# leejaeyong7/nerfacc

Measured on AMD Instinct MI355X. Metric: rays/sec (fwd+bwd) through 128^3 occ-grid, 1M-ray batch, higher is better.
Workload: dtype f32; 1 GPU; cfg2: 1048576 image rays/GPU, 128^3 shell10 occ grid (G=1), step 2*sqrt(3)/1024, sampling+rendering fwd+bwd; rays_per_gpu=1048576, resolution=128, grid=shell10, samples_after_compaction=32244949, parallelism=ray-sharded x1, field=synthetic analytic field, native callbacks (see bench.py NativeField/TorchField)

## Files before the change

### include/nerfacc_hip.h

```cpp
#ifndef NERFACC_HIP_H
#define NERFACC_HIP_H

#include <stdint.h>

#ifdef __cplusplus
extern "C" {
#endif

#define NFA_OK 0
#define NFA_EINVAL (-1)
#define NFA_EHIP (-2)

#define NFA_MAX_GRID_LEVELS 8

typedef void *nfa_stream_t;

const char *nfa_last_error(void);
#define NFA_VERSION 403
int nfa_version(void);
int nfa_set_tuning(const char *name, const char *value);
int nfa_device_arch(char *buf, int buflen);


int64_t nfa_cumsum_scratch_bytes(int64_t n);
// ... 78 lines not shown
                       uint8_t *mask, int32_t *alive, int64_t *count, int32_t count_samples, nfa_stream_t stream);
int nfa_bin_rays_levels(const float *rays_o, const float *rays_d, int64_t n_rays, const float *aabbs, int32_t n_grids,
                        const int32_t *res, float near_plane, int32_t *order, void *scratch,
                        uint64_t *coherence , nfa_stream_t stream);
int nfa_expand_runs(int64_t n_rays, float step_size, const int32_t *run_cnts, const uint64_t *runs,
                    int32_t max_runs, const int64_t *packed_info , float *t_starts,
                    float *t_ends, float *t_mids, int64_t *ray_indices, int64_t capacity, nfa_stream_t stream);
int nfa_fill_ray_indices(int64_t n_rays, const int64_t *packed_info , int64_t *ray_indices,
                         nfa_stream_t stream);
int nfa_traverse_cone_runs(const nfa_traverse_args *args, int32_t *run_cnts, uint64_t *runs, int32_t max_runs,
                           int32_t *overflow_count, const int32_t *ray_order ,
                           int64_t n_order, nfa_stream_t stream);
int nfa_traverse_cone_walk(const nfa_traverse_args *args, const uint32_t *bits, int32_t *run_cnts, uint64_t *runs,
                           int32_t max_runs, int32_t *overflow_count, uint32_t *arena, int32_t arena_capacity,
                           const int32_t *ray_order, int64_t n_order, nfa_stream_t stream);
int nfa_expand_cone_arena(const uint32_t *arena, int32_t n_entries, float step_size, float cone_angle,
                          const int64_t *packed_info , float *t_starts, float *t_ends, int64_t *ray_indices,
                          nfa_stream_t stream);
int nfa_expand_cone_runs(int64_t n_rays, float step_size, float cone_angle, const int32_t *run_cnts,
                         const uint64_t *runs, int32_t max_runs, const int64_t *packed_info, float *t_starts,
                         float *t_ends, int64_t *ray_indices, nfa_stream_t stream);
int nfa_expand_intervals(int64_t n_rays, float step_size, const int32_t *run_cnts, const uint64_t *runs,
                         int32_t max_runs, const int64_t *iv_packed_info , float *vals,
                         int64_t *ray_indices, uint8_t *is_left, uint8_t *is_right, nfa_stream_t stream);


int nfa_grid_cell_points(const int64_t *indices, const float *jitter , int64_t n, const int32_t *res,
                         const float *aabb , float *x , nfa_stream_t stream);
int nfa_grid_ema_update(float *occs, int64_t cell_base, const int64_t *indices, int64_t n, const float *occ,
                        float ema_decay, float *scratch , nfa_stream_t stream);
int64_t nfa_grid_rebinarize_scratch_bytes(void);
int nfa_grid_rebinarize(const float *occs, int32_t n_grids, const int32_t *res, float occ_thre, uint8_t *binaries,
                        uint32_t *walk_bits, void *scratch, nfa_stream_t stream);


void nfa_seg_plan(int64_t n_elems, int64_t n_rays, int64_t *tile_elems, int64_t *n_tiles);
int64_t nfa_seg_table_rows(int64_t n_tiles);
int nfa_seg_build_tiles(const int64_t *packed_info , int64_t n_rays, int64_t n_elems,
                        int64_t tile_elems, int64_t n_tiles, int64_t *tiles ,
                        int32_t *flags, nfa_stream_t stream);

int nfa_packed_scan(int kind, int reverse, const int64_t *packed_info, const int64_t *tiles, int64_t n_tiles,
                    int64_t n_rays, int64_t n_elems, const float *inputs, float *outputs,
                    nfa_stream_t stream);
int nfa_packed_scan_generic(int kind, int reverse, int normalize, const int64_t *packed_info,
                            int64_t n_rays, int64_t n_elems, const float *inputs, float *outputs,
                            nfa_stream_t stream);
int nfa_packed_prod_backward(int kind, const int64_t *packed_info, const int64_t *tiles, int64_t n_tiles,
                             int64_t n_rays, int64_t n_elems, const float *inputs,
                             const float *outputs, const float *grad_outputs, float *grad_inputs,
                             nfa_stream_t stream);

int nfa_render_from_density_fwd(const float *t_starts, const float *t_ends, const float *sigmas,
                                const float *prefix_trans , const int64_t *packed_info,
                                const int64_t *tiles, int64_t n_tiles, int64_t n_rays, int64_t n_elems,
                                float *weights, float *trans, float *alphas, nfa_stream_t stream);
int nfa_render_from_alpha_fwd(const float *alphas, const float *prefix_trans, const int64_t *packed_info,
                              const int64_t *tiles, int64_t n_tiles, int64_t n_rays, int64_t n_elems,
                              float *weights, float *trans, nfa_stream_t stream);
int nfa_render_from_density_bwd(const float *t_starts, const float *t_ends, const float *trans,
                                const float *alphas, const float *g_weights, const float *g_trans,
                                const float *g_alphas, const int64_t *packed_info, const int64_t *tiles, int64_t n_tiles,
                                int64_t n_rays, int64_t n_elems, float *grad_sigmas, float *grad_x,
                                nfa_stream_t stream);
int nfa_density_cdf_rows_fwd(const float *t_starts, const float *t_ends, const float *sigmas, const int64_t *packed_info,
                             const int64_t *tiles, int64_t n_tiles, int64_t n_rays, int64_t n_elems, int32_t row_len,
                             float *trans, float *alphas, float *cdfs , nfa_stream_t stream);
int nfa_density_cdf_rows_bwd(const float *t_starts, const float *t_ends, const float *trans, const float *alphas,
                             const float *g_cdfs , const int64_t *packed_info, const int64_t *tiles,
                             int64_t n_tiles, int64_t n_rays, int64_t n_elems, int32_t row_len, float *grad_sigmas,
                             nfa_stream_t stream);
int nfa_render_from_alpha_bwd(const float *alphas, const float *trans, const float *g_weights,
                              const float *g_trans, const int64_t *packed_info, const int64_t *tiles, int64_t n_tiles,
                              int64_t n_rays, int64_t n_elems, float *grad_alphas, nfa_stream_t stream);

int nfa_render_visibility(const float *t_starts, const float *t_ends, const float *sigmas_or_alphas,
                          const float *prefix_trans, float early_stop_eps, float alpha_thre,
                          const int64_t *packed_info, const int64_t *tiles, int64_t n_tiles, int64_t n_rays,
                          int64_t n_elems, uint8_t *vis, int64_t *vis_cnts, nfa_stream_t stream);
int nfa_compact_samples(const uint8_t *vis, const float *t_starts, const float *t_ends,
                        const int64_t *packed_info, const int64_t *tiles, int64_t n_tiles, const int64_t *out_starts,
                        int64_t n_rays, int64_t n_elems, int64_t *out_ray_indices,
                        float *out_t_starts, float *out_t_ends, int64_t capacity, nfa_stream_t stream);

int nfa_accumulate_along_rays(const float *weights, const float *values, int32_t D,
                              const int64_t *packed_info, const int64_t *tiles, int64_t n_tiles, int64_t n_rays,
                              int64_t n_elems, int accumulate, float *out, nfa_stream_t stream);
int nfa_accumulate_along_rays_atomic(const float *weights, const float *values, int32_t D,
                                     const int64_t *ray_indices, int64_t n_rays, int64_t n_elems,
                                     float *out, nfa_stream_t stream);
int nfa_accumulate_along_rays_bwd(const float *weights, const float *values, int32_t D,
                                  const float *g_out, const int64_t *packed_info, const int64_t *tiles, int64_t n_tiles,
                                  int64_t n_rays, int64_t n_elems, float *g_weights, float *g_values,
                                  nfa_stream_t stream);
int nfa_render_accumulate_fwd(const float *weights, const float *rgbs, const float *t_starts,
                              const float *t_ends, const int64_t *packed_info, const int64_t *tiles, int64_t n_tiles,
                              int64_t n_rays, int64_t n_elems, float *colors, float *opacities,
                              float *depths, nfa_stream_t stream);
int nfa_render_accumulate_bwd(const float *weights, const float *rgbs, const float *t_starts,
                              const float *t_ends, const float *g_colors, const float *g_opacities,
                              const float *g_depths, const int64_t *packed_info, const int64_t *tiles, int64_t n_tiles,
                              int64_t n_rays, int64_t n_elems, float *g_weights, float *g_rgbs,
                              nfa_stream_t stream);

int nfa_render_fused_fwd(const float *t_starts, const float *t_ends, const float *sigmas, const float *rgbs,
                         const int64_t *packed_info, const int64_t *tiles, int64_t n_tiles, int64_t n_rays,
                         int64_t n_elems, float *weights, float *trans, float *alphas, float *colors,
                         float *opacities, float *depths, nfa_stream_t stream);
int nfa_render_fused_bwd(const float *t_starts, const float *t_ends, const float *rgbs, const float *trans,
                         const float *alphas, const float *g_colors, const float *g_opacities,
                         const float *g_depths, const float *g_weights, const float *g_trans,
                         const float *g_alphas, const int64_t *packed_info, const int64_t *tiles, int64_t n_tiles,
                         int64_t n_rays, int64_t n_elems, float *grad_sigmas, float *grad_rgbs,
                         nfa_stream_t stream);

int nfa_distortion_fwd(const float *weights, const float *t_starts, const float *t_ends, const int64_t *packed_info,
                       const int64_t *tiles, int64_t n_tiles, int64_t n_rays, int64_t n_elems, float *loss, float *w_tot,
                       float *s_tot, nfa_stream_t stream);
int nfa_distortion_bwd(const float *weights, const float *t_starts, const float *t_ends, const float *w_tot,
                       const float *s_tot, const float *g_loss, const int64_t *packed_info, const int64_t *tiles,
                       int64_t n_tiles, int64_t n_rays, int64_t n_elems, float *grad_weights, float *grad_t_starts,
                       float *grad_t_ends, nfa_stream_t stream);

#define NFA_VISIBLE_SLOTS 1024
int nfa_render_step_accumulate(const float *t_starts, const float *t_ends, const float *sigmas, const float *rgbs,
                               const int64_t *packed_info, const int64_t *tiles, int64_t n_tiles, int64_t n_rays,
                               int64_t n_elems, float alpha_thre, float *colors, float *opacities, float *depths,
                               int64_t *n_visible, nfa_stream_t stream);


int nfa_importance_sampling(const float *in_vals, const float *cdfs, const int64_t *in_packed_info,
                            int64_t n_rays, int64_t n_edges_per_ray, int64_t n_samples,
                            int stratified, uint64_t seed, uint64_t offset,
                            float *out_intervals , float *out_samples ,
                            nfa_stream_t stream);
int nfa_importance_sampling_t(const float *in_vals, const float *cdfs, const int64_t *in_packed_info, int64_t n_rays,
                              int64_t n_edges_per_ray, int64_t n_samples, int stratified, uint64_t seed,
                              uint64_t offset, float *out_intervals, float *out_samples, int transform, float t_a,
                              float t_b, float *out_t_starts, float *out_t_ends, nfa_stream_t stream);
int nfa_importance_sampling_packed(const float *in_vals, const float *cdfs, const int64_t *in_packed_info, int64_t n_rays,
                                   int64_t n_edges_per_ray, const int64_t *sm_packed_info, const int64_t *iv_packed_info,
                                   int stratified, uint64_t seed, uint64_t offset, float *sm_vals, int64_t *sm_ray_indices,
                                   float *iv_vals, int64_t *iv_ray_indices, uint8_t *iv_is_left, uint8_t *iv_is_right,
                                   nfa_stream_t stream);
int nfa_searchsorted(const float *q_vals, const int64_t *q_packed_info, const int64_t *q_ray_indices,
                     int64_t q_n_rays, int64_t q_per_ray, int64_t q_total,
                     const float *k_vals, const int64_t *k_packed_info, int64_t k_per_ray,
                     int64_t *ids_left, int64_t *ids_right, nfa_stream_t stream);

int nfa_pdf_loss_fwd(const float *q_vals, const float *q_cdfs, const float *k_vals, const float *k_cdfs,
                     int64_t n_rays, int32_t n_query_edges, int32_t n_key_edges, float eps, float *loss,
                     uint32_t *key_ids, nfa_stream_t stream);
int nfa_pdf_loss_bwd(const float *q_cdfs, const float *k_cdfs, const uint32_t *key_ids, int64_t n_rays,
                     int32_t n_query_edges, int32_t n_key_edges, float eps, const float *g_loss, float *g_k_cdfs,
                     float *g_q_cdfs, nfa_stream_t stream);
int64_t nfa_pdf_loss_partials(int64_t n_rays, int32_t n_query_edges, int32_t n_key_edges);
int nfa_pdf_loss_sum_fwd(const float *q_vals, const float *q_cdfs, const float *k_vals, const float *k_cdfs,
                         int64_t n_rays, int32_t n_query_edges, int32_t n_key_edges, float eps, float *partials,
                         uint32_t *key_ids, nfa_stream_t stream);
int nfa_pdf_loss_mean_bwd(const float *q_cdfs, const float *k_cdfs, const uint32_t *key_ids, int64_t n_rays,
                          int32_t n_query_edges, int32_t n_key_edges, float eps, const float *g_mean, float *g_k_cdfs,
                          float *g_q_cdfs, nfa_stream_t stream);


int nfa_opencv_lens_undistortion(const float *uv, const float *params, int64_t n_points, int32_t n_params,
                                 int64_t param_stride, float eps, int32_t iters, float *uv_out, nfa_stream_t stream);
int nfa_opencv_lens_undistortion_fisheye(const float *uv, const float *params, int64_t n_points, int32_t n_params,
                                         int64_t param_stride, float eps, int32_t iters, float *uv_out,
                                         nfa_stream_t stream);


int nfa_hashgrid_fwd(const float *x, const float *params, int64_t n_points, int32_t n_levels, int32_t n_features,
                     int32_t log2_hashmap_size, const float *scales_host, const int32_t *resolutions_host,
                     const int32_t *sizes_host, int64_t n_params, float *y, nfa_stream_t stream);
int nfa_hashgrid_bwd(const float *x, const float *params, const float *grad_y, int64_t n_points, int32_t n_levels,
                     int32_t n_features, int32_t log2_hashmap_size, const float *scales_host,
                     const int32_t *resolutions_host, const int32_t *sizes_host, int64_t n_params, float *grad_params,
                     float *grad_x, nfa_stream_t stream);
int nfa_sh_fwd(const float *dirs, int64_t n_points, int32_t degree, float *out, nfa_stream_t stream);
int nfa_sh_bwd(const float *dirs, const float *grad_out, int64_t n_points, int32_t degree, float *grad_dirs,
               nfa_stream_t stream);


int nfa_sample_positions_fwd(const float *rays_o, const float *rays_d, const float *t_starts, const float *t_ends,
                             const int64_t *ray_indices, int64_t n_rays, int64_t n_elems, int64_t samples_per_ray,
                             const float *aabb_host, const float *aabb, int32_t contraction, int32_t dirs_mode,
                             float *positions, float *dirs, uint8_t *selector, nfa_stream_t stream);
int nfa_sample_positions_bwd(const float *rays_o, const float *rays_d, const float *t_starts, const float *t_ends,
                             const int64_t *ray_indices, const float *g_positions, const float *g_dirs,
                             const int64_t *packed_info, const int64_t *tiles, int64_t n_tiles, int64_t n_rays,
                             int64_t n_elems, int64_t samples_per_ray, const float *aabb_host, const float *aabb,
                             int32_t contraction, int32_t dirs_mode, float *grad_rays_o, float *grad_rays_d,
                             float *grad_t_starts, float *grad_t_ends, float *grad_p, nfa_stream_t stream);

#ifdef __cplusplus
}
#endif
// ... 2 lines not shown
```

### nerfacc_amd/_backend.py

```python
from __future__ import annotations

import ctypes as C
import os
import threading
from typing import Optional

import torch

from . import _build

_lock = threading.Lock()
_lib: Optional[C.CDLL] = None

_vp, _i64, _i32, _f32, _u64, _int = C.c_void_p, C.c_int64, C.c_int32, C.c_float, C.c_uint64, C.c_int


class TraverseArgs(C.Structure):
    _fields_ = [
        ("n_rays", _i64), ("rays_o", _vp), ("rays_d", _vp), ("rays_mask", _vp),
        ("n_grids", _i32), ("res", _i32 * 3), ("binaries", _vp), ("aabbs", _vp),
        ("hits", _vp), ("t_sorted", _vp), ("t_indices", _vp),
        ("near_planes", _vp), ("far_planes", _vp),
        ("step_size", _f32), ("cone_angle", _f32), ("traverse_steps_limit", _i32), ("mode", _i32),
        ("iv_vals", _vp), ("iv_ray_indices", _vp), ("iv_is_left", _vp), ("iv_is_right", _vp),
        ("iv_starts", _vp), ("iv_cnts", _vp),
        ("sm_vals", _vp), ("sm_ray_indices", _vp), ("sm_is_valid", _vp),
        ("sm_t_starts", _vp), ("sm_t_ends", _vp), ("sm_starts", _vp), ("sm_cnts", _vp),
        ("terminate_planes", _vp),
        ("ray_filter", _vp), ("ray_filter_min", _i32),
        ("bricks", _vp), ("coarse", _vp),
        ("steps_limit_dev", _vp), ("n_listed_dev", _vp), ("run_if_nonzero", _vp),
    ]


_SIGS = {
    "nfa_exclusive_cumsum_i64": [_vp, _i64, _vp, _vp, _vp, _vp],
    "nfa_exclusive_cumsum_pairs_i64": [_vp, _i64, _vp, _vp, _vp, _vp],
    "nfa_exclusive_cumsum_pairs_stats_i64": [_vp, _i64, _vp, _vp, _vp, _vp],
    "nfa_pack_info": [_vp, _i64, _i64, _vp, _vp, _vp, _vp],
    "nfa_pdf_loss_fwd": [_vp, _vp, _vp, _vp, _i64, _i32, _i32, _f32, _vp, _vp, _vp],
    "nfa_pdf_loss_bwd": [_vp, _vp, _vp, _i64, _i32, _i32, _f32, _vp, _vp, _vp, _vp],
    "nfa_pdf_loss_partials": [_i64, _i32, _i32],
    "nfa_pdf_loss_sum_fwd": [_vp, _vp, _vp, _vp, _i64, _i32, _i32, _f32, _vp, _vp, _vp],
    "nfa_pdf_loss_mean_bwd": [_vp, _vp, _vp, _i64, _i32, _i32, _f32, _vp, _vp, _vp, _vp],
    "nfa_pack_bits": [_vp, _i64, _vp, _vp],
    "nfa_unpack_rows": [_vp, _vp, _vp, _i64, _i64, _i64, _i64, _vp, _i32, _vp, _vp],
    "nfa_pack_rows": [_vp, _vp, _vp, _i64, _i64, _i64, _i64, _vp, _vp],
    "nfa_mask_row_counts": [_vp, _i64, _i64, _vp, _vp],
    "nfa_ray_aabb_intersect": [_vp, _vp, _i64, _vp, _i32, _f32, _f32, _f32, _vp, _vp, _vp, _vp],
    "nfa_ray_events": [_vp, _vp, _i64, _vp, _i32, _vp, _vp, _vp, _vp],
    "nfa_traverse_grids": [C.POINTER(TraverseArgs), _vp],
    "nfa_bricks_words": [_i32, C.POINTER(_i32)],
    "nfa_pack_bricks": [_vp, _i32, C.POINTER(_i32), _vp, _vp, _vp],
    "nfa_walk_bits_words": [_i32, C.POINTER(_i32)],
    "nfa_pack_walk_bits": [_vp, _i32, C.POINTER(_i32), _vp, _vp],
    "nfa_traverse_runs": [C.POINTER(TraverseArgs), _vp, _vp, _vp, _i32, _vp, _f32, _vp, _i64, _vp],
    "nfa_bin_rays": [_vp, _vp, _i64, _vp, _vp, _vp, _vp],
    "nfa_grid_cell_points": [_vp, _vp, _i64, C.POINTER(_i32), _vp, _vp, _vp],
    "nfa_grid_ema_update": [_vp, _i64, _vp, _i64, _vp, _f32, _vp, _vp],
    "nfa_grid_rebinarize_scratch_bytes": [],
    "nfa_grid_rebinarize": [_vp, _i32, C.POINTER(_i32), _f32, _vp, _vp, _vp, _vp],
    "nfa_expand_runs": [_i64, _f32, _vp, _vp, _i32, _vp, _vp, _vp, _vp, _vp, _i64, _vp],
    "nfa_fill_ray_indices": [_i64, _vp, _vp, _vp],
    "nfa_traverse_cone_runs": [C.POINTER(TraverseArgs), _vp, _vp, _i32, _vp, _vp, _i64, _vp],
    "nfa_alive_rays": [_vp, _vp, _i64, _f32, _i64, _vp, _vp, _vp, _vp],
    "nfa_testmode_begin": [_vp, _vp, _i64, _i32, _i32, _vp, _vp, _vp, _i32, _vp],
    "nfa_testmode_alive": [_vp, _vp, _vp, _f32, _i64, _vp, _vp, _vp, _i32, _vp],
    "nfa_traverse_cone_walk": [C.POINTER(TraverseArgs), _vp, _vp, _vp, _i32, _vp, _vp, _i32, _vp, _i64, _vp],
    "nfa_expand_cone_arena": [_vp, _i32, _f32, _f32, _vp, _vp, _vp, _vp, _vp],
    "nfa_bin_rays_levels": [_vp, _vp, _i64, _vp, _i32, C.POINTER(_i32), _f32, _vp, _vp, _vp, _vp],
    "nfa_expand_cone_runs": [_i64, _f32, _f32, _vp, _vp, _i32, _vp, _vp, _vp, _vp, _vp],
    "nfa_expand_intervals": [_i64, _f32, _vp, _vp, _i32, _vp, _vp, _vp, _vp, _vp, _vp],
    "nfa_seg_plan": [_i64, _i64, C.POINTER(_i64), C.POINTER(_i64)],
    "nfa_seg_table_rows": [_i64],
    "nfa_seg_build_tiles": [_vp, _i64, _i64, _i64, _i64, _vp, _vp, _vp],
    "nfa_packed_scan": [_int, _int, _vp, _vp, _i64, _i64, _i64, _vp, _vp, _vp],
    "nfa_packed_scan_generic": [_int, _int, _int, _vp, _i64, _i64, _vp, _vp, _vp],
    "nfa_packed_prod_backward": [_int, _vp, _vp, _i64, _i64, _i64, _vp, _vp, _vp, _vp, _vp],
    "nfa_render_from_density_fwd": [_vp, _vp, _vp, _vp, _vp, _vp, _i64, _i64, _i64, _vp, _vp, _vp, _vp],
    "nfa_render_from_alpha_fwd": [_vp, _vp, _vp, _vp, _i64, _i64, _i64, _vp, _vp, _vp],
    "nfa_render_from_density_bwd": [_vp, _vp, _vp, _vp, _vp, _vp, _vp, _vp, _vp, _i64, _i64, _i64, _vp, _vp, _vp],
    "nfa_density_cdf_rows_fwd": [_vp, _vp, _vp, _vp, _vp, _i64, _i64, _i64, _i32, _vp, _vp, _vp, _vp],
    "nfa_density_cdf_rows_bwd": [_vp, _vp, _vp, _vp, _vp, _vp, _vp, _i64, _i64, _i64, _i32, _vp, _vp],
    "nfa_render_from_alpha_bwd": [_vp, _vp, _vp, _vp, _vp, _vp, _i64, _i64, _i64, _vp, _vp],
    "nfa_render_visibility": [_vp, _vp, _vp, _vp, _f32, _f32, _vp, _vp, _i64, _i64, _i64, _vp, _vp, _vp],
    "nfa_compact_samples": [_vp, _vp, _vp, _vp, _vp, _i64, _vp, _i64, _i64, _vp, _vp, _vp, _i64, _vp],
    "nfa_accumulate_along_rays": [_vp, _vp, _i32, _vp, _vp, _i64, _i64, _i64, _int, _vp, _vp],
    "nfa_accumulate_along_rays_atomic": [_vp, _vp, _i32, _vp, _i64, _i64, _vp, _vp],
    "nfa_accumulate_along_rays_bwd": [_vp, _vp, _i32, _vp, _vp, _vp, _i64, _i64, _i64, _vp, _vp, _vp],
    "nfa_render_accumulate_fwd": [_vp, _vp, _vp, _vp, _vp, _vp, _i64, _i64, _i64, _vp, _vp, _vp, _vp],
    "nfa_render_accumulate_bwd": [_vp, _vp, _vp, _vp, _vp, _vp, _vp, _vp, _vp, _i64, _i64, _i64, _vp, _vp, _vp],
    "nfa_render_fused_fwd": [_vp, _vp, _vp, _vp, _vp, _vp, _i64, _i64, _i64, _vp, _vp, _vp, _vp, _vp, _vp, _vp],
    "nfa_render_fused_bwd": [_vp] * 13 + [_i64, _i64, _i64, _vp, _vp, _vp],
    "nfa_render_step_accumulate": [_vp, _vp, _vp, _vp, _vp, _vp, _i64, _i64, _i64, _f32, _vp, _vp, _vp, _vp, _vp],
    "nfa_distortion_fwd": [_vp, _vp, _vp, _vp, _vp, _i64, _i64, _i64, _vp, _vp, _vp, _vp],
    "nfa_distortion_bwd": [_vp] * 8 + [_i64, _i64, _i64, _vp, _vp, _vp, _vp],
    "nfa_importance_sampling": [_vp, _vp, _vp, _i64, _i64, _i64, _int, _u64, _u64, _vp, _vp, _vp],
    "nfa_importance_sampling_t": [_vp, _vp, _vp, _i64, _i64, _i64, _int, _u64, _u64, _vp, _vp, _int, _f32, _f32, _vp, _vp, _vp],
    "nfa_importance_sampling_packed": [_vp, _vp, _vp, _i64, _i64, _vp, _vp, _int, _u64, _u64, _vp, _vp, _vp, _vp, _vp, _vp, _vp],
    "nfa_searchsorted": [_vp, _vp, _vp, _i64, _i64, _i64, _vp, _vp, _i64, _vp, _vp, _vp],
    "nfa_opencv_lens_undistortion": [_vp, _vp, _i64, _i32, _i64, _f32, _i32, _vp, _vp],
    "nfa_opencv_lens_undistortion_fisheye": [_vp, _vp, _i64, _i32, _i64, _f32, _i32, _vp, _vp],
    "nfa_hashgrid_fwd": [_vp, _vp, _i64, _i32, _i32, _i32, _vp, _vp, _vp, _i64, _vp, _vp],
    "nfa_hashgrid_bwd": [_vp, _vp, _vp, _i64, _i32, _i32, _i32, _vp, _vp, _vp, _i64, _vp, _vp, _vp],
    "nfa_sh_fwd": [_vp, _i64, _i32, _vp, _vp],
    "nfa_sh_bwd": [_vp, _vp, _i64, _i32, _vp, _vp],
    "nfa_sample_positions_fwd": [_vp, _vp, _vp, _vp, _vp, _i64, _i64, _i64, _vp, _vp, _i32, _i32, _vp, _vp, _vp, _vp],
    "nfa_sample_positions_bwd": [_vp] * 9 + [_i64, _i64, _i64, _i64, _vp, _vp, _i32, _i32, _vp, _vp, _vp, _vp, _vp, _vp],
    "nfa_cumsum_scratch_bytes": [_i64],
    "nfa_last_error": [],
    "nfa_version": [],
    "nfa_set_tuning": [C.c_char_p, C.c_char_p],
    "nfa_device_arch": [C.c_char_p, _int],
}
_RESTYPES = {"nfa_grid_rebinarize_scratch_bytes": _i64, "nfa_bricks_words": _i64, "nfa_walk_bits_words": _i64, "nfa_pdf_loss_partials": _i64, "nfa_cumsum_scratch_bytes": _i64, "nfa_seg_table_rows": _i64, "nfa_seg_plan": None, "nfa_last_error": C.c_char_p}

EXPORTED_SYMBOLS = tuple(_SIGS)


def library_path() -> str:
    return _build.LIB_PATH


def load() -> C.CDLL:
    global _lib
    if _lib is not None:
        return _lib
    with _lock:
        if _lib is not None:
            return _lib
        path = _build.LIB_PATH
        if _build.is_stale() and _build.hipcc() is not None:
            path = _build.build()
        if not os.path.exists(path):
            raise RuntimeError(
                "nerfacc_amd: libnerfacc_hip.so is missing and hipcc is not available to build it. "
                "There is no CPU fallback for the native ops.")
        lib = C.CDLL(path)
        for name, argtypes in _SIGS.items():
            fn = getattr(lib, name)
            fn.argtypes = argtypes
            fn.restype = _RESTYPES[name] if name in _RESTYPES else _int
        if lib.nfa_version() != ABI_VERSION:
            raise RuntimeError(f"nerfacc_amd: {path} was built from include/nerfacc_hip.h version {lib.nfa_version()}, these "
                               f"bindings are written for {ABI_VERSION}: rebuild the library (nerfacc_amd._build.build(force=True))")
        _lib = lib
    return _lib


ABI_VERSION = 403


def set_tuning(name: str, value: Optional[str]) -> None:
    call("nfa_set_tuning", name.encode(), None if value is None else str(value).encode())


class NativeError(RuntimeError):
    """Counterpart of the RuntimeError TORCH_CHECK raises in the reference."""


def call(name: str, *args) -> None:
    lib = load()
    rc = getattr(lib, name)(*args)
    if rc != 0:
        msg = lib.nfa_last_error()
        raise NativeError(f"{name}: {msg.decode() if msg else rc}")


def call_group(name: str, fn) -> None:
    fn()


def ptr(t: Optional[torch.Tensor]):
    return None if t is None else t.data_ptr()


_RAW_STREAM = getattr(torch._C, "_cuda_getCurrentRawStream", None)
_CUR_DEVICE = getattr(torch._C, "_cuda_getDevice", None)


def stream() -> int:
    if _RAW_STREAM is not None and _CUR_DEVICE is not None:
        return _RAW_STREAM(_CUR_DEVICE())
    return torch.cuda.current_stream().cuda_stream


def require_device(*tensors: Optional[torch.Tensor]) -> torch.device:
    dev = None
    for t in tensors:
        if t is None:
            continue
        if not t.is_cuda:
            raise NotImplementedError(
                "nerfacc_amd: this op runs only on a ROCm device (the reference has no CPU "
                "implementation of its native ops either); got a tensor on " + str(t.device))
        if dev is None:
            dev = t.device
        elif t.device != dev:
            raise RuntimeError(f"nerfacc_amd: tensors on different devices ({dev} vs {t.device})")
    if dev is None:
        raise RuntimeError("nerfacc_amd: no tensor argument")
    return dev


def seg_plan(n_elems: int, n_rays: int = 0):
    t, n = _i64(0), _i64(0)
    load().nfa_seg_plan(n_elems, n_rays, C.byref(t), C.byref(n))
    return int(t.value), int(n.value)


def cumsum_scratch(n: int, device) -> torch.Tensor:
    nbytes = ((max(n, 1) + 2047) // 2048 + 1) * 8
    return torch.empty(nbytes // 8, dtype=torch.int64, device=device)
```

### nerfacc_amd/_segments.py

```python
from __future__ import annotations

from dataclasses import dataclass
from typing import Optional

import torch
from torch import Tensor

from . import _backend as B


@dataclass
class SegInfo:
    packed_info: Tensor
    n_rays: int
    n_elems: int
    tiles: Optional[Tensor]
    contiguous: bool
    sorted_indices: bool = True
    n_tiles: int = 0
    trusted: bool = False


_ATTR = "_nfa_seg"
_ATTR_RI = "_nfa_seg_from_ray_indices"


def _build_tiles(packed_info: Tensor, n_elems: int, trusted: bool) -> SegInfo:
    dev = B.require_device(packed_info)
    n_rays = packed_info.shape[0]
    with torch.cuda.device(dev):
        tile_elems, n_tiles = B.seg_plan(n_elems, n_rays)
        tiles = torch.empty((int(B.load().nfa_seg_table_rows(n_tiles)), 2), dtype=torch.int64, device=dev)
        flag = None if trusted else torch.empty(1, dtype=torch.int32, device=dev)
        B.call("nfa_seg_build_tiles", B.ptr(packed_info), n_rays, n_elems, tile_elems, n_tiles, B.ptr(tiles), B.ptr(flag),
               B.stream())
        ok = True if trusted else (int(flag.item()) == 0)
    return SegInfo(packed_info, n_rays, n_elems, tiles if ok else None, ok, n_tiles=n_tiles, trusted=trusted)


def seginfo_from_packed(packed_info: Tensor, n_elems: int, trusted: bool = False) -> SegInfo:
    assert packed_info.dim() == 2 and packed_info.shape[-1] == 2, "packed_info must be 2-D with shape (B, 2)."
    cached = getattr(packed_info, _ATTR, None)
    if cached is not None and cached[0] == packed_info._version and cached[1] == n_elems:
        return cached[2]
    pi = packed_info
    if pi.dtype != torch.int64 or not pi.is_contiguous():
        pi = pi.to(torch.int64).contiguous()
    info = _build_tiles(pi, n_elems, trusted)
    try:
        setattr(packed_info, _ATTR, (packed_info._version, n_elems, info))
    except Exception:
        pass
    return info


def tag_trusted(packed_info: Tensor, n_elems: int) -> SegInfo:
    return seginfo_from_packed(packed_info, n_elems, trusted=True)


def pack_info_native(ray_indices: Tensor, n_rays: int):
    dev = B.require_device(ray_indices)
    ri = ray_indices if (ray_indices.dtype == torch.int64 and ray_indices.is_contiguous()) else \
        ray_indices.to(torch.int64).contiguous()
    with torch.cuda.device(dev):
        packed = torch.empty((n_rays, 2), dtype=torch.int64, device=dev)
        flag = torch.empty(1, dtype=torch.int32, device=dev)
        scratch = B.cumsum_scratch(n_rays, dev)
        B.call("nfa_pack_info", B.ptr(ri), ri.numel(), n_rays, B.ptr(packed), B.ptr(flag), B.ptr(scratch), B.stream())
    return packed, flag


def seginfo_from_ray_indices(ray_indices: Tensor, n_rays: int) -> SegInfo:
    assert ray_indices.dim() == 1, "ray_indices must be a 1D tensor with shape (n_samples)."
    assert n_rays is not None, "n_rays must be provided"
    cached = getattr(ray_indices, _ATTR_RI, None)
    if cached is not None and cached[0] == ray_indices._version and cached[1] == n_rays:
        return cached[2]
    packed, flag = pack_info_native(ray_indices, n_rays)
    info = _build_tiles(packed, ray_indices.numel(), trusted=True)
    info.sorted_indices = int(flag.item()) == 0
    try:
        setattr(ray_indices, _ATTR_RI, (ray_indices._version, n_rays, info))
    except Exception:
        pass
    return info


def tag_ray_indices(ray_indices: Tensor, n_rays: int, info: SegInfo) -> None:
    setattr(ray_indices, _ATTR_RI, (ray_indices._version, n_rays, info))


def resolve(n_elems: int, packed_info: Optional[Tensor], ray_indices: Optional[Tensor],
            n_rays: Optional[int]) -> Optional[SegInfo]:
    if packed_info is not None:
        return seginfo_from_packed(packed_info, n_elems)
    if ray_indices is not None:
        if n_rays is None:
            n_rays = int(ray_indices.max().item()) + 1 if ray_indices.numel() else 0
        return seginfo_from_ray_indices(ray_indices, n_rays)
    return None


_UNIFORM: "dict[tuple, SegInfo]" = {}


def uniform_seginfo(n_rows: int, row_len: int, device: torch.device) -> SegInfo:
    key = (int(n_rows), int(row_len), device.type, device.index)
    info = _UNIFORM.get(key)
    if info is None:
        starts = torch.arange(n_rows, dtype=torch.int64, device=device) * row_len
        packed = torch.stack([starts, torch.full_like(starts, row_len)], dim=-1)
        info = _build_tiles(packed, n_rows * row_len, trusted=True)
        setattr(packed, _ATTR, (packed._version, n_rows * row_len, info))
        if len(_UNIFORM) >= 6:
            _UNIFORM.pop(next(iter(_UNIFORM)))
        _UNIFORM[key] = info
    return info


def batched_native(*tensors: Optional[Tensor]) -> Optional[SegInfo]:
    ref = None
    for t in tensors:
        if t is None:
            continue
        if not t.is_cuda or t.dtype != torch.float32 or t.dim() < 1:
            return None
        if ref is None:
            ref = t
        elif t.shape != ref.shape:
            return None
    if ref is None or ref.numel() == 0:
        return None
    return uniform_seginfo(ref.numel() // ref.shape[-1], ref.shape[-1], ref.device)
```

### nerfacc_amd/csrc/segscan.hip

```cpp
#include <stdlib.h>

#include "common.hip.h"
#include "samples.h"

namespace nfa {

constexpr int SE = 4;
constexpr int SQ = SE / 4;
constexpr int SEG_CHUNK = 64 * SE;
#ifndef NFA_SEG_TILE_ROWS
#define NFA_SEG_TILE_ROWS 256
#endif
constexpr int64_t SEG_TILE_ROWS = NFA_SEG_TILE_ROWS;
#ifndef NFA_VIS_EXP_FREE
#define NFA_VIS_EXP_FREE 1
#endif
#ifndef NFA_SEG_WAVES_PER_BLOCK
#define NFA_SEG_WAVES_PER_BLOCK 4
#endif
constexpr int SEG_WAVES_PER_BLOCK = NFA_SEG_WAVES_PER_BLOCK;

__global__ __launch_bounds__(256) void seg_build_tiles_kernel(const int64_t *__restrict__ packed_info, int64_t n_rays,
                                                              int64_t n_elems, int64_t tile_elems, int64_t n_tiles,
                                                              longlong2 *__restrict__ tiles, int32_t *__restrict__ flags)
{
    for (int64_t r = (int64_t)blockIdx.x * blockDim.x + threadIdx.x; r <= n_rays;
         r += (int64_t)blockDim.x * gridDim.x) {
        int64_t b_lo, b_hi, e_first;
        bool bad = false;
        if (r < n_rays) {
            const int64_t s = packed_info[2 * r], n = packed_info[2 * r + 1];
            int64_t s_prev = -1;
            if (r > 0) {
                const int64_t ps = packed_info[2 * r - 2], pn = packed_info[2 * r - 1];
                s_prev = ps;
                bad |= (ps + pn != s);
            }
            bad |= (n < 0) || (s < 0) || (s + n > n_elems);
            if (bad) { if (flags) atomicOr(flags, 1); continue; }
            b_lo = (s_prev < 0) ? 0 : s_prev / tile_elems + (r - 1) / SEG_TILE_ROWS + 1;
            b_hi = s / tile_elems + r / SEG_TILE_ROWS;
            e_first = s;
        } else {
            const int64_t s_prev = n_rays > 0 ? packed_info[2 * n_rays - 2] : -1;
            const int64_t n_prev = n_rays > 0 ? packed_info[2 * n_rays - 1] : 0;
            b_lo = (s_prev < 0) ? 0 : s_prev / tile_elems + (n_rays - 1) / SEG_TILE_ROWS + 1;
            b_hi = n_tiles;
            e_first = (s_prev < 0) ? 0 : s_prev + n_prev;
            if (s_prev > n_elems) { if (flags) atomicOr(flags, 1); continue; }
        }
        for (int64_t b = b_lo; b <= b_hi && b <= n_tiles; ++b) tiles[b] = make_longlong2(r, e_first);
    }
}

__host__ __device__ inline int64_t seg_table_rows(int64_t n_tiles) { return n_tiles + 1; }

struct F4 { float v[SE]; };

struct Pos {
    int64_t c;
    int32_t off;
    int32_t safe;
    bool valid[SE];
    bool any, all;
    int32_t d_lo, d_hi;
    bool qany[SQ], qall[SQ];
    __device__ __forceinline__ int64_t p0() const { return c + off; }
};

template <bool VEC>
__device__ __forceinline__ void ld4(const float *__restrict__ p, const Pos &q, F4 &out)
{
    const float *b = p + q.c;
    if (VEC) {
#pragma unroll
        for (int h = 0; h < SQ; ++h) {
            const nfa_v4f v = *reinterpret_cast<const nfa_v4f *>(b + (q.qany[h] ? q.off + 4 * h : q.safe));
            out.v[4 * h] = v.x; out.v[4 * h + 1] = v.y; out.v[4 * h + 2] = v.z; out.v[4 * h + 3] = v.w;
        }
    } else {
#pragma unroll
        for (int j = 0; j < SE; ++j) out.v[j] = b[q.valid[j] ? q.off + j : q.safe];
    }
}
__device__ __forceinline__ float sel(const F4 &r, int j, const bool valid[SE], float fill) { return valid[j] ? r.v[j] : fill; }

#define NFA_ELEMENTWISE_PATH() asm volatile("; element-wise path" ::: "memory")
template <bool VEC>
__device__ __forceinline__ void store4(float *__restrict__ p, const Pos &q, const float v[SE])
{
    float *b = p + q.c;
#pragma unroll
    for (int h = 0; h < SQ; ++h) {
        if (VEC && q.qall[h]) {
            store_f4(b + q.off + 4 * h, v[4 * h], v[4 * h + 1], v[4 * h + 2], v[4 * h + 3]);
        } else {
            NFA_ELEMENTWISE_PATH();
#pragma unroll
            for (int j = 4 * h; j < 4 * h + 4; ++j)
                if (q.valid[j]) b[q.off + j] = v[j];
        }
    }
}

struct StepHeads {
    int32_t lh[SE];
    uint32_t acc;
    bool open_prefix;
    bool carry_on_lane_end;
    int32_t carry_lane;
    int32_t ph;
    int32_t rid[SE], prev_rid[SE];
    bool is_head[SE];
};

template <int S>
__device__ __forceinline__ void heads_step(int32_t &ah, uint32_t &acc)
{
    const int32_t uh = dpp_step<S>(-1, ah);
    if (ah < 0) { acc |= 1u << S; ah = uh; }
}

template <int DIR>
__device__ __forceinline__ void resolve_heads(const int32_t hj[SE], const bool valid[SE], int32_t carry_rid, StepHeads &hd)
{
#pragma unroll
    for (int k = 0; k < SE; ++k) {
        const int j = DIR > 0 ? k : SE - 1 - k;
        const int32_t h = valid[j] ? hj[j] : -1;
        hd.is_head[k] = h >= 0;
        hd.lh[k] = (k == 0 || h >= 0) ? h : hd.lh[k - 1 < 0 ? 0 : k - 1];
    }
    int32_t ah = hd.lh[SE - 1];
    uint32_t acc = 0;
    heads_step<0>(ah, acc); heads_step<1>(ah, acc); heads_step<2>(ah, acc);
    heads_step<3>(ah, acc); heads_step<4>(ah, acc); heads_step<5>(ah, acc);
    const int lane = lane_id(), r = lane & 15;
    const uint32_t has_src = (r >= 1 ? 1u : 0u) | (r >= 2 ? 2u : 0u) | (r >= 4 ? 4u : 0u) | (r >= 8 ? 8u : 0u) |
                             ((lane & 16) ? 16u : 0u) | (lane >= 32 ? 32u : 0u);
    hd.acc = acc & has_src;
    int32_t ph = dpp_prev_lane(-1, ah);
    hd.open_prefix = ph < 0;
    if (ph < 0) ph = carry_rid;
    hd.ph = ph;
    int32_t pr = ph;
#pragma unroll
    for (int k = 0; k < SE; ++k) {
        hd.prev_rid[k] = pr;
        hd.rid[k] = hd.lh[k] >= 0 ? hd.lh[k] : ph;
        pr = hd.rid[k];
    }
}

template <int S, int N, class FI, class FC>
__device__ __forceinline__ void values_step(const StepHeads &hd, float av[N], FI identity, FC comb)
{
    const bool take = (hd.acc >> S) & 1u;
#pragma unroll
    for (int ch = 0; ch < N; ++ch) {
        const float uv = dpp_step<S>(identity(ch), av[ch]);
        if (take) av[ch] = comb(ch, uv, av[ch]);
    }
}

template <int N, class FI, class FC>
__device__ __forceinline__ void scan_values(const StepHeads &hd, const float x[SE][N], float carry[N], float incl[SE][N],
                                            float prev[SE][N], FI identity, FC comb)
{
    float li[SE][N];
#pragma unroll
    for (int k = 0; k < SE; ++k)
#pragma unroll
        for (int ch = 0; ch < N; ++ch)
            li[k][ch] = (k == 0 || hd.is_head[k]) ? x[k][ch] : comb(ch, li[k - 1 < 0 ? 0 : k - 1][ch], x[k][ch]);
    float av[N];
#pragma unroll
    for (int ch = 0; ch < N; ++ch) av[ch] = li[SE - 1][ch];
    values_step<0, N>(hd, av, identity, comb); values_step<1, N>(hd, av, identity, comb);
    values_step<2, N>(hd, av, identity, comb); values_step<3, N>(hd, av, identity, comb);
    values_step<4, N>(hd, av, identity, comb); values_step<5, N>(hd, av, identity, comb);
    float pv[N];
#pragma unroll
    for (int ch = 0; ch < N; ++ch) {
        pv[ch] = dpp_prev_lane(identity(ch), av[ch]);
        if (hd.open_prefix) pv[ch] = comb(ch, carry[ch], pv[ch]);
    }
#pragma unroll
// ... 462 lines not shown
#pragma unroll
                for (int j = 0; j < 4; ++j)
                    if (pq.valid[4 * h + j]) g4[j] = b[pq.off + 4 * h + j + crid[4 * h + j]];
            }
#pragma unroll
            for (int j = 0; j < 4; ++j) {
                const float GT = -g4[j];
                q[4 * h + j] = GW[4 * h + j] * (T[4 * h + j] * A[4 * h + j]) + GT * T[4 * h + j];
            }
        }
    }
    __device__ __forceinline__ void fetch(const Pos &q, Raw &r) const
    {
        ld4<VEC>(ts, q, r.a);
        ld4<VEC>(te, q, r.b);
        ld4<VEC>(tr, q, r.T);
        if (!CDF) ld4<VEC>(al, q, r.A);
        if (gw) ld4<VEC>(gw, q, r.gw);
        if (gt) ld4<VEC>(gt, q, r.gt);
        if (ga) ld4<VEC>(ga, q, r.ga);
    }
    __device__ __forceinline__ void load(const Raw &r, const Pos &pos)
    {
        const bool *valid = pos.valid;
#pragma unroll
        for (int j = 0; j < SE; ++j) {
            T[j] = sel(r.T, j, valid, 0.0f); A[j] = CDF ? 0.0f : sel(r.A, j, valid, 0.0f);
            GW[j] = (gw && valid[j]) ? r.gw.v[j] : 0.0f;
            const float GT = (gt && valid[j]) ? r.gt.v[j] : 0.0f;
            GA[j] = (ga && valid[j]) ? r.ga.v[j] : 0.0f;
            dlt[j] = r.b.v[j] - r.a.v[j];
            q[j] = GW[j] * (T[j] * A[j]) + GT * T[j];
        }
    }
    __device__ __forceinline__ float x(int j, int) const { return q[j]; }
    __device__ __forceinline__ void emit(int j, int64_t, bool, bool is_head, int, int, const float *, const float prev[1])
    {
        const float E = is_head ? 0.0f : prev[0];
        const float om = 1.0f - A[j];
        const float B = GW[j] * T[j] * om + GA[j] * om - E;
        rx[j] = B; rs[j] = dlt[j] * B;
    }
    __device__ __forceinline__ void store(const Pos &q)
    {
        (void)q.p0();
        if (gsig) store4<VEC>(gsig, q, rs);
        if (gx) store4<VEC>(gx, q, rx);
    }
};

template <bool VEC>
struct AlphaBwdOp : OpBase {
    struct Raw { F4 T, A, gw, gt; };
    const float *al, *tr, *gw, *gt;
    float *galpha;
    float T[SE], A[SE], GW[SE], q[SE], res[SE];
    __device__ __forceinline__ void fetch(const Pos &q, Raw &r) const
    {
        ld4<VEC>(tr, q, r.T);
        ld4<VEC>(al, q, r.A);
        if (gw) ld4<VEC>(gw, q, r.gw);
        if (gt) ld4<VEC>(gt, q, r.gt);
    }
    __device__ __forceinline__ void load(const Raw &r, const Pos &pos)
    {
        const bool *valid = pos.valid;
#pragma unroll
        for (int j = 0; j < SE; ++j) {
            T[j] = sel(r.T, j, valid, 0.0f); A[j] = sel(r.A, j, valid, 0.0f);
            GW[j] = (gw && valid[j]) ? r.gw.v[j] : 0.0f;
            const float GT = (gt && valid[j]) ? r.gt.v[j] : 0.0f;
            q[j] = (GW[j] * A[j] + GT) * T[j];
        }
    }
    __device__ __forceinline__ float x(int j, int) const { return q[j]; }
    __device__ __forceinline__ void emit(int j, int64_t, bool, bool is_head, int, int, const float *, const float prev[1])
    {
        const float E = is_head ? 0.0f : prev[0];
        res[j] = GW[j] * T[j] - E / fmaxf(1.0f - A[j], 1e-10f);
    }
    __device__ __forceinline__ void store(const Pos &q) { store4<VEC>(galpha, q, res); }
};

template <bool DENSITY, bool VEC, bool COUNT>
struct VisibilityOp : OpBase {
    static constexpr int NCHB = COUNT ? 1 : 0;
    struct Raw { F4 s, pf, a, b; };
    const float *ts, *te, *val, *prefix;
    float eps, thre;
    float s_lo, s_hi;
    uint8_t *vis;
    int64_t *cnts;
    float x0[SE], a4[SE], pf[SE];
    uint8_t m[SE];
    __device__ __forceinline__ float identity(int) const { return DENSITY ? 0.0f : 1.0f; }
    __device__ __forceinline__ float comb(int, float a, float b) const { return DENSITY ? a + b : a * b; }
    __device__ __forceinline__ void fetch(const Pos &q, Raw &r) const
    {
        ld4<VEC>(val, q, r.s);
        if (prefix) ld4<VEC>(prefix, q, r.pf);
        if (DENSITY) {
            ld4<VEC>(ts, q, r.a);
            ld4<VEC>(te, q, r.b);
        }
    }
    __device__ __forceinline__ void load(const Raw &r, const Pos &pos)
    {
        const bool *valid = pos.valid;
#pragma unroll
        for (int j = 0; j < SE; ++j) {
            pf[j] = prefix ? r.pf.v[j] : 1.0f;
            const float sv = sel(r.s, j, valid, 0.0f);
            if (DENSITY) { x0[j] = valid[j] ? sv * (r.b.v[j] - r.a.v[j]) : 0.0f; a4[j] = (thre > 0.0f) ? 1.0f - expf(-x0[j]) : 1.0f; }
            else { a4[j] = sv; x0[j] = 1.0f - sv; }
        }
    }
    __device__ __forceinline__ float x(int j, int) const { return x0[j]; }
    __device__ __forceinline__ void emit(int j, int64_t, bool valid, bool is_head, int, int, const float *, const float prev[1])
    {
        bool v;
        if (DENSITY && NFA_VIS_EXP_FREE && !prefix) {
            const float S = is_head ? 0.0f : prev[0];
            v = S <= s_lo;
            const bool band = S > s_lo && S < s_hi;
            if (__ballot(band) != 0ull) {
                asm volatile("; transmittance near the threshold" ::: "memory");
                if (band) v = expf(-S) >= eps;
            }
        } else {
            float T = DENSITY ? expf(-(is_head ? 0.0f : prev[0])) : (is_head ? 1.0f : prev[0]);
            if (prefix) T *= pf[j];
            v = T >= eps;
        }
        if (thre > 0.0f) v = v && (a4[j] >= thre);
        m[j] = (valid && v) ? 1 : 0;
    }
    __device__ __forceinline__ float xb(int j, int) const { return (float)m[j]; }
    __device__ __forceinline__ void ray_done_b(int rid, int, float tot) const { cnts[rid] = (int64_t)tot; }
    __device__ __forceinline__ void store(const Pos &q)
    {
        uint8_t *b = vis + q.c;
#pragma unroll
        for (int h = 0; h < SQ; ++h) {
            if (VEC && q.qall[h]) {
                *reinterpret_cast<uchar4 *>(b + q.off + 4 * h) = make_uchar4(m[4 * h], m[4 * h + 1], m[4 * h + 2], m[4 * h + 3]);
            } else {
                NFA_ELEMENTWISE_PATH();
#pragma unroll
                for (int j = 4 * h; j < 4 * h + 4; ++j)
                    if (q.valid[j]) b[q.off + j] = m[j];
            }
        }
    }
    __device__ __forceinline__ void empty_ray(int rid) const
    {
        if (COUNT) cnts[rid] = 0;
    }
};

struct U4 { uint32_t w[SQ]; };
__device__ __forceinline__ void load_mask4(const uint8_t *vis, bool vec, const Pos &q, U4 &m)
{
    const uint8_t *b = vis + q.c;
#pragma unroll
    for (int h = 0; h < SQ; ++h) {
        if (vec) {
            const int32_t o = q.safe + (q.qany[h] ? 1 : 0) * (q.off + 4 * h - q.safe);
            m.w[h] = *reinterpret_cast<const uint32_t *>(b + o);
        } else {
            uint32_t w = 0;
#pragma unroll
            for (int j = 0; j < 4; ++j) w |= (uint32_t)b[q.valid[4 * h + j] ? q.off + 4 * h + j : q.safe] << (8 * j);
            m.w[h] = w;
        }
    }
}
__device__ __forceinline__ float mask_sel(const U4 &m, int j, const bool valid[SE])
{
    return (valid[j] && ((m.w[j / 4] >> (8 * (j % 4))) & 0xFFu)) ? 1.0f : 0.0f;
}

template <bool VEC>
struct CompactOp : OpBase {
    static constexpr int RAY_CAP = 192;
    static constexpr int RAY_LDS_FLOATS = 3 * SEG_CHUNK + 2 * RAY_CAP;
    struct Raw { U4 m; F4 a, b; };
    const uint8_t *vis;
    int vis_vec;
    const float *ts, *te;
    const int64_t *out_starts;
    int64_t *o_ri;
    float *o_ts, *o_te;
    int64_t cap = (int64_t)1 << 62;
    float *stage = nullptr;
    const int64_t *s_start = nullptr;
    int32_t g_lo = 0, g_n = 0;
    float m[SE], a[SE], b[SE];
    int64_t dst[SE];
    int32_t er[SE];
    float rank[SE];
    __device__ __forceinline__ void tile_begin(int32_t r_lo, int32_t r_hi, float *lds)
    {
        stage = lds;
        int64_t *st = reinterpret_cast<int64_t *>(lds + 3 * SEG_CHUNK);
        s_start = st; g_lo = r_lo; g_n = min(r_hi - r_lo, RAY_CAP);
        __builtin_amdgcn_wave_barrier();
        for (int32_t i = lane_id(); i < g_n; i += 64) st[i] = out_starts[(int64_t)r_lo + i];
        __builtin_amdgcn_wave_barrier();
    }
    __device__ __forceinline__ void fetch(const Pos &q, Raw &r) const
    {
        load_mask4(vis, vis_vec != 0, q, r.m);
        ld4<VEC>(ts, q, r.a);
        ld4<VEC>(te, q, r.b);
    }
    __device__ __forceinline__ void load(const Raw &r, const Pos &pos)
    {
        const bool *valid = pos.valid;
#pragma unroll
        for (int j = 0; j < SE; ++j) { m[j] = mask_sel(r.m, j, valid); a[j] = r.a.v[j]; b[j] = r.b.v[j]; }
    }
    __device__ __forceinline__ float x(int j, int) const { return m[j]; }
    __device__ __forceinline__ void emit(int j, int64_t, bool, bool is_head, int rid, int, const float *, const float prev[1])
    {
        er[j] = rid;
        rank[j] = is_head ? 0.0f : prev[0];
    }
    __device__ __forceinline__ void store(const Pos &)
    {
        struct __attribute__((packed, aligned(4))) Q4 { float x, y, z, w; };
        struct __attribute__((packed, aligned(8))) L2 { int64_t x, y; };
        bool keep[SE];
        bool any = false;
        int n_mine = 0;
#pragma unroll
        for (int j = 0; j < SE; ++j) { keep[j] = m[j] != 0.0f; any = any || keep[j]; n_mine += keep[j] ? 1 : 0; }
        const unsigned long long lanes = __ballot(any);
        if (lanes == 0ull) return;
        bool far = false;
#pragma unroll
        for (int j = 0; j < SE; ++j) {
            const uint32_t slot = (uint32_t)(er[j] - g_lo);
            const bool staged = slot < (uint32_t)g_n;
            dst[j] = s_start[staged ? slot : 0u];
            far = far || (keep[j] && !staged);
        }
        if (__ballot(far) != 0ull) {
            asm volatile("; output offsets beyond the staged rays" ::: "memory");
#pragma unroll
            for (int j = 0; j < SE; ++j)
                if (keep[j] && (uint32_t)(er[j] - g_lo) >= (uint32_t)g_n) dst[j] = out_starts[er[j]];
        }
#pragma unroll
        for (int j = 0; j < SE; ++j) dst[j] = keep[j] ? dst[j] + (int64_t)rank[j] : 0;
        const int lane = lane_id();
        const int first = __builtin_ctzll(lanes), last = 63 - __builtin_clzll(lanes);
        int64_t my_first = dst[SE - 1], my_last = dst[0];
#pragma unroll
        for (int j = SE - 2; j >= 0; --j) if (keep[j]) my_first = dst[j];
#pragma unroll
        for (int j = 1; j < SE; ++j) if (keep[j]) my_last = dst[j];
        const int64_t base = uniform64(__shfl(my_first, first, 64));
        const int64_t span = uniform64(__shfl(my_last, last, 64)) - base + 1;
        int cnt = n_mine;
#pragma unroll
        for (int off = 32; off >= 1; off >>= 1) cnt += __shfl_xor(cnt, off, 64);
        if (span == (int64_t)cnt && span <= SEG_CHUNK) {
            float *s_ts = stage, *s_te = stage + SEG_CHUNK;
            int32_t *s_ri = reinterpret_cast<int32_t *>(stage + 2 * SEG_CHUNK);
            __builtin_amdgcn_wave_barrier();
#pragma unroll
            for (int j = 0; j < SE; ++j)
                if (keep[j]) {
                    const uint32_t o = (uint32_t)(dst[j] - base);
                    if (o < (uint32_t)SEG_CHUNK) { s_ts[o] = a[j]; s_te[o] = b[j]; s_ri[o] = er[j]; }
                }
            __builtin_amdgcn_wave_barrier();
            const int n = (int)max((int64_t)0, min(span, cap - base));
            float *g_ts = o_ts + base, *g_te = o_te + base;
            int64_t *g_ri = o_ri + base;
            for (int o = 4 * lane; o < n; o += 256) {
                if (o + 3 < n) {
                    const Q4 vt = {s_ts[o], s_ts[o + 1], s_ts[o + 2], s_ts[o + 3]};
                    const Q4 ve = {s_te[o], s_te[o + 1], s_te[o + 2], s_te[o + 3]};
                    *reinterpret_cast<Q4 *>(g_ts + o) = vt;
                    *reinterpret_cast<Q4 *>(g_te + o) = ve;
                    const L2 r0 = {(int64_t)s_ri[o], (int64_t)s_ri[o + 1]}, r1 = {(int64_t)s_ri[o + 2], (int64_t)s_ri[o + 3]};
                    *reinterpret_cast<L2 *>(g_ri + o) = r0;
                    *reinterpret_cast<L2 *>(g_ri + o + 2) = r1;
                } else {
                    for (int i = o; i < n; ++i) { g_ts[i] = s_ts[i]; g_te[i] = s_te[i]; g_ri[i] = (int64_t)s_ri[i]; }
                }
            }
            __builtin_amdgcn_wave_barrier();
        } else {
#pragma unroll
            for (int j = 0; j < SE; ++j)
                if (keep[j] && dst[j] < cap) { o_ri[dst[j]] = er[j]; o_ts[dst[j]] = a[j]; o_te[dst[j]] = b[j]; }
        }
    }
};

template <int C, bool VEC>
// ... 161 lines not shown
    const float *w, *rgb, *ts, *te;
    float *colors, *opac, *depth;
    float xv[SE][5];
    __device__ __forceinline__ void fetch(const Pos &q, Raw &r) const
    {
        ld4<VEC>(w, q, r.w);
        ld4<VEC>(ts, q, r.a);
        ld4<VEC>(te, q, r.b);
        load_rgb12(rgb, VEC, q, r.c);
    }
    __device__ __forceinline__ void load(const Raw &r, const Pos &pos)
    {
        const bool *valid = pos.valid;
        float c[3 * SE];
        fix_rgb12(rgb, VEC, pos, r.c, c);
#pragma unroll
        for (int j = 0; j < SE; ++j) {
            const float ww = sel(r.w, j, valid, 0.0f);
            xv[j][0] = ww * c[3 * j]; xv[j][1] = ww * c[3 * j + 1]; xv[j][2] = ww * c[3 * j + 2];
            xv[j][3] = ww;
            xv[j][4] = ww * ((r.a.v[j] + r.b.v[j]) / 2.0f);
        }
    }
    __device__ __forceinline__ float x(int j, int ch) const { return xv[j][ch]; }
    __device__ __forceinline__ void put(int rid, const float *t) const
    {
        colors[3 * (int64_t)rid] = t[0]; colors[3 * (int64_t)rid + 1] = t[1]; colors[3 * (int64_t)rid + 2] = t[2];
        opac[rid] = t[3]; depth[rid] = t[4];
    }
    __device__ __forceinline__ void emit(int, int64_t, bool, bool, int, int, const float *, const float *) const {}
    __device__ __forceinline__ void store(const Pos &) const {}
    __device__ __forceinline__ void ray_done(int rid, const float t[5]) const { put(rid, t); }
    __device__ __forceinline__ void empty_ray(int rid) const
    {
        const float z[5] = {0, 0, 0, 0, 0};
        put(rid, z);
    }
};

template <bool VEC>
struct RenderAccumBwdOp : OpBase {
    struct Raw { F4 w, a, b; float c[3 * SE]; };
    const float *w, *rgb, *ts, *te, *gc, *go, *gd;
    float *gw, *grgb;
    float ww[SE], mid[SE], res[SE], c[3 * SE], gr[3 * SE];
    __device__ __forceinline__ void fetch(const Pos &q, Raw &r) const
    {
        ld4<VEC>(w, q, r.w);
        ld4<VEC>(ts, q, r.a);
        ld4<VEC>(te, q, r.b);
        load_rgb12(rgb, VEC, q, r.c);
    }
    __device__ __forceinline__ void load(const Raw &r, const Pos &pos)
    {
        const bool *valid = pos.valid;
        (void)valid;
#pragma unroll
        for (int j = 0; j < SE; ++j) { ww[j] = r.w.v[j]; mid[j] = (r.a.v[j] + r.b.v[j]) / 2.0f; }
        fix_rgb12(rgb, VEC, pos, r.c, c);
    }
    __device__ __forceinline__ float x(int, int) const { return 0.0f; }
    __device__ __forceinline__ void emit(int j, int64_t, bool valid, bool, int rid, int, const float *, const float *)
    {
        float g = 0.0f;
        gr[3 * j] = gr[3 * j + 1] = gr[3 * j + 2] = 0.0f;
        if (valid) {
            if (gc) {
                const float g0 = gc[3 * (int64_t)rid], g1 = gc[3 * (int64_t)rid + 1], g2 = gc[3 * (int64_t)rid + 2];
                g += g0 * c[3 * j] + g1 * c[3 * j + 1] + g2 * c[3 * j + 2];
                gr[3 * j] = g0 * ww[j]; gr[3 * j + 1] = g1 * ww[j]; gr[3 * j + 2] = g2 * ww[j];
            }
            if (go) g += go[rid];
            if (gd) g += gd[rid] * mid[j];
        }
        res[j] = g;
    }
    __device__ __forceinline__ void store(const Pos &q)
    {
        if (gw) store4<VEC>(gw, q, res);
        if (grgb) store_rgb12(grgb, VEC, q, gr);
    }
};

template <bool VEC>
struct RenderFusedFwdOp : OpBase {
    static constexpr int NCHB = 5;
    struct Raw { F4 a, b, s; float c[3 * SE]; };
    const float *ts, *te, *sig, *rgb;
    float *w, *tr, *al, *colors, *opac, *depth;
    float xs[SE], mid[SE], rw[SE], rt[SE], ra[SE], c[3 * SE];
    __device__ __forceinline__ void fetch(const Pos &q, Raw &r) const
    {
        ld4<VEC>(ts, q, r.a);
        ld4<VEC>(te, q, r.b);
        ld4<VEC>(sig, q, r.s);
        load_rgb12(rgb, VEC, q, r.c);
    }
    __device__ __forceinline__ void load(const Raw &r, const Pos &pos)
    {
        const bool *valid = pos.valid;
        fix_rgb12(rgb, VEC, pos, r.c, c);
#pragma unroll
        for (int j = 0; j < SE; ++j) {
            xs[j] = valid[j] ? r.s.v[j] * (r.b.v[j] - r.a.v[j]) : 0.0f;
            mid[j] = (r.a.v[j] + r.b.v[j]) / 2.0f;
        }
    }
    __device__ __forceinline__ float x(int j, int) const { return xs[j]; }
    __device__ __forceinline__ void emit(int j, int64_t, bool, bool is_head, int, int, const float *, const float prev[1])
    {
        const float S = is_head ? 0.0f : prev[0];
        const float T = expf(-S);
        const float a = 1.0f - expf(-xs[j]);
        rt[j] = T; ra[j] = a; rw[j] = T * a;
    }
    __device__ __forceinline__ float xb(int j, int ch) const
    {
        return ch < 3 ? rw[j] * c[3 * j + ch] : (ch == 3 ? rw[j] : rw[j] * mid[j]);
    }
    __device__ __forceinline__ void put(int rid, const float *t) const
    {
        colors[3 * (int64_t)rid] = t[0]; colors[3 * (int64_t)rid + 1] = t[1]; colors[3 * (int64_t)rid + 2] = t[2];
        opac[rid] = t[3]; depth[rid] = t[4];
    }
    __device__ __forceinline__ void ray_done_b(int rid, int ch, float t) const
    {
        if (ch < 3) colors[3 * (int64_t)rid + ch] = t;
        else if (ch == 3) opac[rid] = t;
        else depth[rid] = t;
    }
    __device__ __forceinline__ void empty_ray(int rid) const
    {
        const float z[5] = {0, 0, 0, 0, 0};
        put(rid, z);
    }
    __device__ __forceinline__ void store(const Pos &q)
    {
        if (w) store4<VEC>(w, q, rw);
        if (tr) store4<VEC>(tr, q, rt);
        if (al) store4<VEC>(al, q, ra);
    }
};

template <bool VEC>
struct RenderStepOp : OpBase {
    static constexpr int NCHB = 5;
    static constexpr bool NEEDS_RID = true;
    struct Raw { F4 a, b, s; float c[3 * SE]; };
    const float *ts, *te, *sig, *rgb;
    float thre;
    float *colors, *opac, *depth;
    unsigned long long *n_visible;
    float xs[SE], mid[SE], pf[SE], rw[SE], c[3 * SE];
    bool keep[SE];
    __device__ __forceinline__ void fetch(const Pos &q, Raw &r) const
    {
        ld4<VEC>(ts, q, r.a);
        ld4<VEC>(te, q, r.b);
        ld4<VEC>(sig, q, r.s);
        load_rgb12(rgb, VEC, q, r.c);
    }
    __device__ __forceinline__ void load(const Raw &r, const Pos &pos)
    {
        const bool *valid = pos.valid;
        fix_rgb12(rgb, VEC, pos, r.c, c);
#pragma unroll
        for (int j = 0; j < SE; ++j) {
            xs[j] = valid[j] ? r.s.v[j] * (r.b.v[j] - r.a.v[j]) : 0.0f;
            mid[j] = (r.a.v[j] + r.b.v[j]) / 2.0f;
        }
    }
    __device__ __forceinline__ void pre(int j, int64_t, bool valid, int rid) { pf[j] = valid ? 1.0f - opac[rid] : 1.0f; }
    __device__ __forceinline__ void store_pre(const Pos &) const {}
    __device__ __forceinline__ float x(int j, int) const { return xs[j]; }
    __device__ __forceinline__ void emit(int j, int64_t, bool valid, bool is_head, int, int, const float *, const float prev[1])
    {
        const float S = is_head ? 0.0f : prev[0];
        const float T = expf(-S) * pf[j];
        const float a = 1.0f - expf(-xs[j]);
        keep[j] = valid && !(thre > 0.0f && !(a >= thre));
        rw[j] = keep[j] ? T * a : 0.0f;
    }
    __device__ __forceinline__ float xb(int j, int ch) const
    {
        return ch < 3 ? rw[j] * c[3 * j + ch] : (ch == 3 ? rw[j] : rw[j] * mid[j]);
    }
    __device__ __forceinline__ void ray_done_b(int rid, int ch, float t) const
    {
        if (ch < 3) colors[3 * (int64_t)rid + ch] += t;
        else if (ch == 3) opac[rid] += t;
        else depth[rid] += t;
    }
    __device__ __forceinline__ void store(const Pos &) const
    {
        if (n_visible) {
            int c = 0;
#pragma unroll
            for (int j = 0; j < SE; ++j) c += __builtin_popcountll(__ballot(keep[j]));
            if (c > 0 && lane_id() == 0)
                atomicAdd(n_visible + ((blockIdx.x * SEG_WAVES_PER_BLOCK + (threadIdx.x >> 6)) & (NFA_VISIBLE_SLOTS - 1)), (unsigned long long)c);
        }
    }
};

template <bool VEC, bool EXTRA >
struct RenderFusedBwdOp : OpBase {
    static constexpr bool NEEDS_RID = true;
    static constexpr int RAY_CAP = 192;
    static constexpr int RAY_LDS_FLOATS = 8 * RAY_CAP;
    static constexpr bool PIPE = true;
    struct Raw { F4 a, b, T, A, gw, gt, ga; float c[3 * SE]; };
    const float *ts, *te, *rgb, *tr, *al, *gc, *go, *gd, *gw, *gt, *ga;
    float *gsig, *grgb;
    const float *g_lds = nullptr;
    int32_t g_lo = 0, g_n = 0;
    __device__ __forceinline__ void tile_begin(int32_t r_lo, int32_t r_hi, float *lds)
    {
        g_lds = lds; g_n = min(r_hi - r_lo, RAY_CAP); g_lo = r_hi - g_n;
        __builtin_amdgcn_wave_barrier();
        for (int32_t i = lane_id(); i < g_n; i += 64) {
            const int64_t r = (int64_t)g_lo + i;
            float4 v = make_float4(0.f, 0.f, 0.f, 0.f);
            if (gc) { v.x = gc[3 * r]; v.y = gc[3 * r + 1]; v.z = gc[3 * r + 2]; }
            if (go) v.w = go[r];
            *reinterpret_cast<float4 *>(lds + 8 * i) = v;
            lds[8 * i + 4] = gd ? gd[r] : 0.0f;
        }
        __builtin_amdgcn_wave_barrier();
    }
    float T[SE], A[SE], GW[SE], GT[SE], GA[SE], dlt[SE], mid[SE], q[SE], rs[SE], c[3 * SE], gr[3 * SE];
    __device__ __forceinline__ void fetch(const Pos &q, Raw &r) const
    {
        ld4<VEC>(ts, q, r.a);
        ld4<VEC>(te, q, r.b);
        ld4<VEC>(tr, q, r.T);
        ld4<VEC>(al, q, r.A);
        if (EXTRA) {
            if (gw) ld4<VEC>(gw, q, r.gw);
            if (gt) ld4<VEC>(gt, q, r.gt);
            if (ga) ld4<VEC>(ga, q, r.ga);
        }
        load_rgb12(rgb, VEC, q, r.c);
    }
    __device__ __forceinline__ void load(const Raw &r, const Pos &pos)
    {
        const bool *valid = pos.valid;
        fix_rgb12(rgb, VEC, pos, r.c, c);
#pragma unroll
        for (int j = 0; j < SE; ++j) {
            T[j] = sel(r.T, j, valid, 0.0f); A[j] = sel(r.A, j, valid, 0.0f);
            GW[j] = (EXTRA && gw && valid[j]) ? r.gw.v[j] : 0.0f;
            GT[j] = (EXTRA && gt && valid[j]) ? r.gt.v[j] : 0.0f;
            GA[j] = (EXTRA && ga && valid[j]) ? r.ga.v[j] : 0.0f;
            dlt[j] = r.b.v[j] - r.a.v[j];
            mid[j] = (r.a.v[j] + r.b.v[j]) / 2.0f;
        }
    }
    __device__ __forceinline__ void pre(int j, int64_t, bool valid, int rid)
    {
        float g = 0.0f;
        gr[3 * j] = gr[3 * j + 1] = gr[3 * j + 2] = 0.0f;
        const float wj = T[j] * A[j];
        if (valid) {
            const uint32_t slot = (uint32_t)(rid - g_lo);
            float g0, g1, g2, g3, g4;
            if (slot < (uint32_t)g_n) {
                const float4 v = *reinterpret_cast<const float4 *>(g_lds + 8 * slot);
                g0 = v.x; g1 = v.y; g2 = v.z; g3 = v.w; g4 = g_lds[8 * slot + 4];
            } else {
                g0 = gc ? gc[3 * (int64_t)rid] : 0.0f; g1 = gc ? gc[3 * (int64_t)rid + 1] : 0.0f; g2 = gc ? gc[3 * (int64_t)rid + 2] : 0.0f;
                g3 = go ? go[rid] : 0.0f; g4 = gd ? gd[rid] : 0.0f;
            }
            if (gc) {
                g += g0 * c[3 * j] + g1 * c[3 * j + 1] + g2 * c[3 * j + 2];
                gr[3 * j] = g0 * wj; gr[3 * j + 1] = g1 * wj; gr[3 * j + 2] = g2 * wj;
            }
            if (go) g += g3;
            if (gd) g += g4 * mid[j];
        }
        GW[j] = g + GW[j];
        q[j] = GW[j] * wj + GT[j] * T[j];
    }
    __device__ __forceinline__ void store_pre(const Pos &pq)
    {
        if (grgb) store_rgb12(grgb, VEC, pq, gr);
    }
    __device__ __forceinline__ float x(int j, int) const { return q[j]; }
    __device__ __forceinline__ void emit(int j, int64_t, bool, bool is_head, int, int, const float *, const float prev[1])
    {
        const float E = is_head ? 0.0f : prev[0];
        const float om = 1.0f - A[j];
        const float Bv = GW[j] * T[j] * om + GA[j] * om - E;
        rs[j] = dlt[j] * Bv;
    }
    __device__ __forceinline__ void store(const Pos &pq)
    {
        if (gsig) store4<VEC>(gsig, pq, rs);
    }
};

constexpr int DIST_RAY_CAP = SEG_TILE_ROWS < 256 ? (int)SEG_TILE_ROWS : 256;
__device__ __forceinline__ float dist_mid(float a, float b) { return (a + b) / 2.0f; }
__device__ __forceinline__ float dist_first_mid(const int64_t *packed_info, const float *ts, const float *te, int64_t r)
{
    const longlong2 pr = *reinterpret_cast<const longlong2 *>(packed_info + 2 * r);
    return pr.y > 0 ? dist_mid(ts[pr.x], te[pr.x]) : 0.0f;
}

template <bool VEC>
struct DistortionFwdOp : OpBase {
    static constexpr int NCH = 2;
    static constexpr int NCHB = 1;
    static constexpr bool NEEDS_RID = true;
    static constexpr bool TOTALS = true;
    static constexpr int RAY_LDS_FLOATS = DIST_RAY_CAP;
    struct Raw { F4 a, b, w; };
    const int64_t *pinfo;
    const float *ts, *te, *w;
    float *loss, *wtot, *stot;
    const float *m_lds = nullptr;
    int32_t g_lo = 0, g_n = 0;
    float ww[SE], mid[SE], sw[SE], d[SE], term[SE];
    __device__ __forceinline__ void tile_begin(int32_t r_lo, int32_t r_hi, float *lds)
    {
        m_lds = lds; g_lo = r_lo; g_n = min(r_hi - r_lo, DIST_RAY_CAP);
        __builtin_amdgcn_wave_barrier();
        for (int32_t i = lane_id(); i < g_n; i += 64) lds[i] = dist_first_mid(pinfo, ts, te, (int64_t)g_lo + i);
        __builtin_amdgcn_wave_barrier();
    }
    __device__ __forceinline__ void fetch(const Pos &q, Raw &r) const
    {
        ld4<VEC>(ts, q, r.a);
        ld4<VEC>(te, q, r.b);
        ld4<VEC>(w, q, r.w);
    }
    __device__ __forceinline__ void load(const Raw &r, const Pos &pos)
    {
        const bool *valid = pos.valid;
// ... 157 lines not shown
    }
    __device__ __forceinline__ void put(int rid, const float *t) const
    {
        if (go) { go[3 * (int64_t)rid] = t[0]; go[3 * (int64_t)rid + 1] = t[1]; go[3 * (int64_t)rid + 2] = t[2]; }
        if (gd) { gd[3 * (int64_t)rid] = t[3]; gd[3 * (int64_t)rid + 1] = t[4]; gd[3 * (int64_t)rid + 2] = t[5]; }
    }
    __device__ __forceinline__ void ray_done(int rid, const float t[6]) const { put(rid, t); }
    __device__ __forceinline__ void empty_ray(int rid) const
    {
        const float z[6] = {0, 0, 0, 0, 0, 0};
        put(rid, z);
    }
};

template <bool EXCL, bool PROD>
__global__ __launch_bounds__(256) void generic_scan_kernel(const int64_t *__restrict__ packed_info, int64_t n_rays,
                                                           const float *__restrict__ in, float *__restrict__ out,
                                                           int reverse, int normalize)
{
    const int lane = lane_id();
    const float init = PROD ? 1.0f : 0.0f;
    for (int64_t r = ((int64_t)blockIdx.x * blockDim.x + threadIdx.x) >> 6; r < n_rays;
         r += ((int64_t)blockDim.x * gridDim.x) >> 6) {
        const int64_t s = packed_info[2 * r], n = packed_info[2 * r + 1];
        if (n <= 0) continue;
        float den = 1.0f;
        if (normalize) {
            float tot = init;
            for (int64_t k = lane; k < n; k += 64) tot = PROD ? tot * in[s + k] : tot + in[s + k];
#pragma unroll
            for (int off = 32; off >= 1; off >>= 1) {
                const float u = __shfl_xor(tot, off, 64);
                tot = PROD ? tot * u : tot + u;
            }
            den = fmaxf(tot, 1e-10f);
        }
        float carry = init;
        for (int64_t c = 0; c < n; c += 64) {
            const int64_t k = c + lane;
            const int64_t pos = reverse ? s + n - 1 - k : s + k;
            float v = k < n ? in[pos] : init;
#pragma unroll
            for (int off = 1; off < 64; off <<= 1) {
                const float u = __shfl_up(v, off, 64);
                if (lane >= off) v = PROD ? u * v : u + v;
            }
            v = PROD ? carry * v : carry + v;
            float prevv = __shfl_up(v, 1, 64);
            if (lane == 0) prevv = carry;
            if (k < n) {
                float o = EXCL ? prevv : v;
                if (normalize && !(EXCL && k == 0)) o /= den;
                out[pos] = o;
            }
            carry = __shfl(v, 63, 64);
        }
    }
}

__global__ __launch_bounds__(256) void accumulate_atomic_kernel(const float *__restrict__ w, const float *__restrict__ vals,
                                                                int32_t D, const int64_t *__restrict__ ri, int64_t n_rays,
                                                                int64_t n, float *__restrict__ out)
{
    for (int64_t i = (int64_t)blockIdx.x * blockDim.x + threadIdx.x; i < n * D; i += (int64_t)blockDim.x * gridDim.x) {
        const int64_t e = i / D;
        const int32_t ch = (int32_t)(i - e * D);
        const int64_t r = ri[e];
        if (r < 0 || r >= n_rays) continue;
        const float v = vals ? w[e] * vals[i] : w[e];
        atomicAdd(out + r * D + ch, v);
    }
}

}

using namespace nfa;

#define SEG_COMMON_CHECKS(name)                                                                         \
    NFA_REQUIRE(n_rays >= 0 && n_elems >= 0, name ": negative size");                                   \
    NFA_REQUIRE(n_rays < ((int64_t)1 << 31) - 64, name ": too many rays");                              \
    if (n_elems == 0 && n_rays == 0) return NFA_OK;                                                      \
    NFA_REQUIRE(packed_info && tiles && n_tiles >= 1, name ": packed_info/tiles is null")

extern "C" {

void nfa_seg_plan(int64_t n_elems, int64_t n_rays, int64_t *tile_elems, int64_t *n_tiles)
{
    const int64_t t_env = tuning_env("NFA_SEG_TILE") ? atoll(tuning_env("NFA_SEG_TILE")) : 0;
    const int64_t t = t_env > 0 ? t_env : 1024;
    *tile_elems = t;
    *n_tiles = n_elems / t + (n_rays > 0 ? n_rays : 0) / SEG_TILE_ROWS + 1;
}

int64_t nfa_seg_table_rows(int64_t n_tiles) { return seg_table_rows(n_tiles); }

int nfa_seg_build_tiles(const int64_t *packed_info, int64_t n_rays, int64_t n_elems, int64_t tile_elems, int64_t n_tiles,
                        int64_t *tiles, int32_t *flags, nfa_stream_t stream)
{
    NFA_REQUIRE(n_rays >= 0 && n_elems >= 0 && tiles, "seg_build_tiles: bad arguments");
    NFA_REQUIRE(n_rays == 0 || packed_info, "seg_build_tiles: packed_info is null");
    NFA_REQUIRE(n_rays < ((int64_t)1 << 31) - 64, "seg_build_tiles: too many rays");
    NFA_REQUIRE(tile_elems >= 64 && tile_elems % 4 == 0 && n_tiles == n_elems / tile_elems + n_rays / SEG_TILE_ROWS + 1,
                "seg_build_tiles: tile_elems must be a multiple of 4 (>= 64) and n_tiles what nfa_seg_plan returns for (n_elems, n_rays)");
    hipStream_t s = as_stream(stream);
    if (flags && hipMemsetAsync(flags, 0, sizeof(int32_t), s) != hipSuccess) { set_error("seg_build_tiles: memset failed"); return NFA_EHIP; }
    hipLaunchKernelGGL(seg_build_tiles_kernel, dim3(grid_1d(n_rays + 1, 256)), dim3(256), 0, s, packed_info, n_rays,
                       n_elems, tile_elems, n_tiles, reinterpret_cast<longlong2 *>(tiles), flags);
    NFA_CHECK_LAUNCH("seg_build_tiles");
    return NFA_OK;
}

int nfa_packed_scan(int kind, int reverse, const int64_t *packed_info, const int64_t *tiles, int64_t n_tiles, int64_t n_rays,
                    int64_t n_elems, const float *inputs, float *outputs, nfa_stream_t stream)
{
    SEG_COMMON_CHECKS("packed_scan");
    NFA_REQUIRE(kind >= 0 && kind <= 3, "packed_scan: kind must be 0..3");
    if (n_elems == 0) return NFA_OK;
    NFA_REQUIRE(inputs && outputs, "packed_scan: null data pointer");
    hipStream_t s = as_stream(stream);
    const bool vec = all_aligned16(inputs, outputs);
    dispatch_bool(kind & 1, [&](auto EX) {
        dispatch_bool(kind >= 2, [&](auto PR) {
            dispatch_bool(vec, [&](auto V) {
                ScanOp<EX, PR, V> op;
                op.in = inputs; op.out = outputs;
                dispatch_bool(reverse != 0, [&](auto REV) { launch_seg<REV ? -1 : 1>(op, packed_info, tiles, n_rays, n_tiles, s); });
            });
        });
    });
    NFA_CHECK_LAUNCH("packed_scan");
    return NFA_OK;
}

int nfa_packed_scan_generic(int kind, int reverse, int normalize, const int64_t *packed_info, int64_t n_rays,
                            int64_t n_elems, const float *inputs, float *outputs, nfa_stream_t stream)
{
    NFA_REQUIRE(kind >= 0 && kind <= 3 && n_rays >= 0 && n_elems >= 0, "packed_scan_generic: bad arguments");
    if (n_elems == 0 || n_rays == 0) return NFA_OK;
    NFA_REQUIRE(packed_info && inputs && outputs, "packed_scan_generic: null pointer");
    hipStream_t s = as_stream(stream);
    const unsigned grid = grid_1d(n_rays * 64, 256, 1 << 16);
    switch (kind) {
        case 0: hipLaunchKernelGGL((generic_scan_kernel<false, false>), dim3(grid), dim3(256), 0, s, packed_info, n_rays, inputs, outputs, reverse, normalize); break;
        case 1: hipLaunchKernelGGL((generic_scan_kernel<true, false>), dim3(grid), dim3(256), 0, s, packed_info, n_rays, inputs, outputs, reverse, normalize); break;
        case 2: hipLaunchKernelGGL((generic_scan_kernel<false, true>), dim3(grid), dim3(256), 0, s, packed_info, n_rays, inputs, outputs, reverse, normalize); break;
        default: hipLaunchKernelGGL((generic_scan_kernel<true, true>), dim3(grid), dim3(256), 0, s, packed_info, n_rays, inputs, outputs, reverse, normalize); break;
    }
    NFA_CHECK_LAUNCH("packed_scan_generic");
    return NFA_OK;
}

int nfa_packed_prod_backward(int kind, const int64_t *packed_info, const int64_t *tiles, int64_t n_tiles, int64_t n_rays,
                             int64_t n_elems, const float *inputs, const float *outputs, const float *grad_outputs,
                             float *grad_inputs, nfa_stream_t stream)
{
    SEG_COMMON_CHECKS("packed_prod_backward");
    NFA_REQUIRE(kind == 2 || kind == 3, "packed_prod_backward: kind must be 2 or 3");
    if (n_elems == 0) return NFA_OK;
    NFA_REQUIRE(inputs && outputs && grad_outputs && grad_inputs, "packed_prod_backward: null data pointer");
    hipStream_t s = as_stream(stream);
    const bool vec = all_aligned16(inputs, outputs, grad_outputs, grad_inputs);
    dispatch_bool(kind == 3, [&](auto EX) {
        dispatch_bool(vec, [&](auto V) {
            ProdBwdOp<EX, V> op;
            op.in = inputs; op.outv = outputs; op.g = grad_outputs; op.gin = grad_inputs;
            launch_seg<-1>(op, packed_info, tiles, n_rays, n_tiles, s);
// ... 51 lines not shown
    NFA_REQUIRE(t_starts && t_ends && trans && alphas && (grad_sigmas || grad_x), "render_from_density_bwd: null pointer");
    hipStream_t s = as_stream(stream);
    const bool vec = all_aligned16(t_starts, t_ends, trans, alphas, g_weights, g_trans, g_alphas, grad_sigmas, grad_x);
    dispatch_bool(vec, [&](auto V) {
        DensityBwdOp<V> op;
        op.ts = t_starts; op.te = t_ends; op.tr = trans; op.al = alphas;
        op.gw = g_weights; op.gt = g_trans; op.ga = g_alphas; op.gsig = grad_sigmas; op.gx = grad_x;
        launch_seg<-1>(op, packed_info, tiles, n_rays, n_tiles, s);
    });
    NFA_CHECK_LAUNCH("render_from_density_bwd");
    return NFA_OK;
}

int nfa_density_cdf_rows_fwd(const float *t_starts, const float *t_ends, const float *sigmas, const int64_t *packed_info,
                             const int64_t *tiles, int64_t n_tiles, int64_t n_rays, int64_t n_elems, int32_t row_len,
                             float *trans, float *alphas, float *cdfs, nfa_stream_t stream)
{
    SEG_COMMON_CHECKS("density_cdf_rows_fwd");
    if (n_elems == 0) return NFA_OK;
    NFA_REQUIRE(t_starts && t_ends && sigmas && cdfs, "density_cdf_rows_fwd: null pointer");
    NFA_REQUIRE(row_len >= 1 && n_rays * (int64_t)row_len == n_elems, "density_cdf_rows_fwd: n_elems must be n_rays * row_len");
    hipStream_t s = as_stream(stream);
    const bool vec = all_aligned16(t_starts, t_ends, sigmas, trans, alphas);
    dispatch_bool(vec, [&](auto V) {
        DensityFwdOp<V> op;
        op.ts = t_starts; op.te = t_ends; op.sig = sigmas; op.prefix = nullptr;
        op.w = nullptr; op.tr = trans; op.al = alphas; op.cdf = cdfs; op.row_len = row_len;
        launch_seg<1>(op, packed_info, tiles, n_rays, n_tiles, s);
    });
    NFA_CHECK_LAUNCH("density_cdf_rows_fwd");
    return NFA_OK;
}

int nfa_density_cdf_rows_bwd(const float *t_starts, const float *t_ends, const float *trans, const float *alphas,
                             const float *g_cdfs, const int64_t *packed_info, const int64_t *tiles, int64_t n_tiles,
                             int64_t n_rays, int64_t n_elems, int32_t row_len, float *grad_sigmas, nfa_stream_t stream)
{
    SEG_COMMON_CHECKS("density_cdf_rows_bwd");
    if (n_elems == 0) return NFA_OK;
    NFA_REQUIRE(t_starts && t_ends && trans && g_cdfs && grad_sigmas, "density_cdf_rows_bwd: null pointer");
    (void)alphas;
    NFA_REQUIRE(row_len >= 1 && n_rays * (int64_t)row_len == n_elems, "density_cdf_rows_bwd: n_elems must be n_rays * row_len");
    hipStream_t s = as_stream(stream);
    const bool vec = all_aligned16(t_starts, t_ends, trans, alphas, grad_sigmas);
    dispatch_bool(vec, [&](auto V) {
        DensityBwdOp<V, true> op;
        op.ts = t_starts; op.te = t_ends; op.tr = trans; op.al = alphas;
        op.gw = nullptr; op.gt = nullptr; op.ga = nullptr; op.gcdf = g_cdfs; op.gsig = grad_sigmas; op.gx = nullptr;
        launch_seg<-1>(op, packed_info, tiles, n_rays, n_tiles, s);
    });
    NFA_CHECK_LAUNCH("density_cdf_rows_bwd");
    return NFA_OK;
}

int nfa_render_from_alpha_bwd(const float *alphas, const float *trans, const float *g_weights, const float *g_trans,
                              const int64_t *packed_info, const int64_t *tiles, int64_t n_tiles, int64_t n_rays, int64_t n_elems,
                              float *grad_alphas, nfa_stream_t stream)
{
    SEG_COMMON_CHECKS("render_from_alpha_bwd");
    if (n_elems == 0) return NFA_OK;
    NFA_REQUIRE(alphas && trans && grad_alphas, "render_from_alpha_bwd: null pointer");
    hipStream_t s = as_stream(stream);
    const bool vec = all_aligned16(alphas, trans, g_weights, g_trans, grad_alphas);
    dispatch_bool(vec, [&](auto V) {
        AlphaBwdOp<V> op;
        op.al = alphas; op.tr = trans; op.gw = g_weights; op.gt = g_trans; op.galpha = grad_alphas;
        launch_seg<-1>(op, packed_info, tiles, n_rays, n_tiles, s);
    });
    NFA_CHECK_LAUNCH("render_from_alpha_bwd");
    return NFA_OK;
}

int nfa_render_visibility(const float *t_starts, const float *t_ends, const float *sigmas_or_alphas,
                          const float *prefix_trans, float early_stop_eps, float alpha_thre,
                          const int64_t *packed_info, const int64_t *tiles, int64_t n_tiles, int64_t n_rays, int64_t n_elems,
                          uint8_t *vis, int64_t *vis_cnts, nfa_stream_t stream)
{
    SEG_COMMON_CHECKS("render_visibility");
    hipStream_t s = as_stream(stream);
    if (n_elems > 0) {
        NFA_REQUIRE(sigmas_or_alphas && vis, "render_visibility: null pointer");
        const bool density = t_starts != nullptr;
        NFA_REQUIRE(!density || t_ends, "render_visibility: t_ends is null");
        float s_lo, s_hi;
        if (early_stop_eps > 0.0f) {
            const double L = -log((double)early_stop_eps);
            const double w = 2e-5 * (L > 1.0 ? L : 1.0);
            s_lo = (float)(L - w); s_hi = (float)(L + w);
        } else {
            s_lo = INFINITY; s_hi = INFINITY;
        }
        const bool vec = all_aligned16(t_starts, t_ends, sigmas_or_alphas, prefix_trans) &&
                         (reinterpret_cast<uintptr_t>(vis) & 3) == 0;
        dispatch_bool(density, [&](auto DN) {
            dispatch_bool(vec, [&](auto V) {
                dispatch_bool(vis_cnts != nullptr, [&](auto CN) {
                    VisibilityOp<DN, V, CN> op;
                    op.ts = t_starts; op.te = t_ends; op.val = sigmas_or_alphas; op.prefix = prefix_trans;
                    op.eps = early_stop_eps; op.thre = alpha_thre; op.vis = vis; op.cnts = vis_cnts; op.s_lo = s_lo; op.s_hi = s_hi;
                    launch_seg<1>(op, packed_info, tiles, n_rays, n_tiles, s);
                });
            });
        });
    } else if (vis_cnts && n_rays > 0) {
        if (hipMemsetAsync(vis_cnts, 0, sizeof(int64_t) * n_rays, s) != hipSuccess) { set_error("render_visibility: memset failed"); return NFA_EHIP; }
    }
    NFA_CHECK_LAUNCH("render_visibility");
    return NFA_OK;
}

int nfa_compact_samples(const uint8_t *vis, const float *t_starts, const float *t_ends, const int64_t *packed_info,
                        const int64_t *tiles, int64_t n_tiles, const int64_t *out_starts, int64_t n_rays, int64_t n_elems,
                        int64_t *out_ray_indices, float *out_t_starts, float *out_t_ends, int64_t capacity, nfa_stream_t stream)
{
    SEG_COMMON_CHECKS("compact_samples");
    if (n_elems == 0) return NFA_OK;
    NFA_REQUIRE(vis && t_starts && t_ends && out_starts, "compact_samples: null input");
    NFA_REQUIRE(capacity >= 0, "compact_samples: negative capacity");
    hipStream_t s = as_stream(stream);
    const bool vec = all_aligned16(t_starts, t_ends);
    dispatch_bool(vec, [&](auto V) {
        CompactOp<V> op;
        op.vis = vis; op.vis_vec = (reinterpret_cast<uintptr_t>(vis) & 3) == 0; op.ts = t_starts; op.te = t_ends;
        op.out_starts = out_starts; op.o_ri = out_ray_indices; op.o_ts = out_t_starts; op.o_te = out_t_ends; op.cap = capacity;
        launch_seg<1>(op, packed_info, tiles, n_rays, n_tiles, s);
    });
    NFA_CHECK_LAUNCH("compact_samples");
    return NFA_OK;
}

int nfa_accumulate_along_rays(const float *weights, const float *values, int32_t D, const int64_t *packed_info,
                              const int64_t *tiles, int64_t n_tiles, int64_t n_rays, int64_t n_elems, int accumulate, float *out,
                              nfa_stream_t stream)
{
    SEG_COMMON_CHECKS("accumulate_along_rays");
    NFA_REQUIRE(D >= 1 && (values || D == 1), "accumulate_along_rays: bad D");
    if (n_rays == 0) return NFA_OK;
    NFA_REQUIRE(out && (n_elems == 0 || weights), "accumulate_along_rays: null pointer");
    hipStream_t s = as_stream(stream);
    const bool vec = all_aligned16(weights);
    for (int32_t d0 = 0; d0 < D;) {
        const int32_t c = (D - d0 >= 4) ? 4 : (D - d0);
        dispatch_channels(c, [&](auto C) {
            dispatch_bool(vec, [&](auto V) {
                AccumOp<C, V> op;
                op.w = weights; op.vals = values; op.D = D; op.d0 = d0; op.out = out; op.accumulate = accumulate;
                launch_seg<1>(op, packed_info, tiles, n_rays, n_tiles, s);
            });
        });
        d0 += c;
    }
    NFA_CHECK_LAUNCH("accumulate_along_rays");
    return NFA_OK;
}

int nfa_accumulate_along_rays_atomic(const float *weights, const float *values, int32_t D, const int64_t *ray_indices,
                                     int64_t n_rays, int64_t n_elems, float *out, nfa_stream_t stream)
{
    NFA_REQUIRE(D >= 1 && (values || D == 1) && n_rays >= 0 && n_elems >= 0, "accumulate_along_rays_atomic: bad arguments");
    if (n_elems == 0 || n_rays == 0) return NFA_OK;
    NFA_REQUIRE(weights && ray_indices && out, "accumulate_along_rays_atomic: null pointer");
    hipLaunchKernelGGL(accumulate_atomic_kernel, dim3(grid_1d(n_elems * D, 256)), dim3(256), 0, as_stream(stream), weights,
                       values, D, ray_indices, n_rays, n_elems, out);
    NFA_CHECK_LAUNCH("accumulate_along_rays_atomic");
    return NFA_OK;
}

int nfa_accumulate_along_rays_bwd(const float *weights, const float *values, int32_t D, const float *g_out,
                                  const int64_t *packed_info, const int64_t *tiles, int64_t n_tiles, int64_t n_rays, int64_t n_elems,
                                  float *g_weights, float *g_values, nfa_stream_t stream)
{
    SEG_COMMON_CHECKS("accumulate_along_rays_bwd");
    NFA_REQUIRE(D >= 1 && (values || D == 1), "accumulate_along_rays_bwd: bad D");
    if (n_elems == 0) return NFA_OK;
    NFA_REQUIRE(weights && g_out && (g_weights || g_values), "accumulate_along_rays_bwd: null pointer");
    hipStream_t s = as_stream(stream);
    const bool vec = all_aligned16(weights, g_weights);
    for (int32_t d0 = 0; d0 < D;) {
        const int32_t c = (D - d0 >= 4) ? 4 : (D - d0);
        dispatch_channels(c, [&](auto C) {
            dispatch_bool(vec, [&](auto V) {
                AccumBwdOp<C, V> op;
                op.w = weights; op.vals = values; op.gout = g_out; op.D = D; op.d0 = d0;
                op.first = (d0 == 0); op.gw = g_weights; op.gv = g_values;
                launch_seg<1>(op, packed_info, tiles, n_rays, n_tiles, s);
            });
        });
        d0 += c;
    }
    NFA_CHECK_LAUNCH("accumulate_along_rays_bwd");
    return NFA_OK;
}

int nfa_render_accumulate_fwd(const float *weights, const float *rgbs, const float *t_starts, const float *t_ends,
                              const int64_t *packed_info, const int64_t *tiles, int64_t n_tiles, int64_t n_rays, int64_t n_elems,
                              float *colors, float *opacities, float *depths, nfa_stream_t stream)
{
    SEG_COMMON_CHECKS("render_accumulate_fwd");
    if (n_rays == 0) return NFA_OK;
    NFA_REQUIRE(colors && opacities && depths && (n_elems == 0 || (weights && rgbs && t_starts && t_ends)),
                "render_accumulate_fwd: null pointer");
    hipStream_t s = as_stream(stream);
    const bool vec = all_aligned16(weights, rgbs, t_starts, t_ends);
    dispatch_bool(vec, [&](auto V) {
        RenderAccumOp<V> op;
        op.w = weights; op.rgb = rgbs; op.ts = t_starts; op.te = t_ends;
        op.colors = colors; op.opac = opacities; op.depth = depths;
        launch_seg<1>(op, packed_info, tiles, n_rays, n_tiles, s);
    });
    NFA_CHECK_LAUNCH("render_accumulate_fwd");
    return NFA_OK;
}

int nfa_render_accumulate_bwd(const float *weights, const float *rgbs, const float *t_starts, const float *t_ends,
                              const float *g_colors, const float *g_opacities, const float *g_depths,
                              const int64_t *packed_info, const int64_t *tiles, int64_t n_tiles, int64_t n_rays, int64_t n_elems,
                              float *g_weights, float *g_rgbs, nfa_stream_t stream)
{
    SEG_COMMON_CHECKS("render_accumulate_bwd");
    if (n_elems == 0) return NFA_OK;
    NFA_REQUIRE(weights && rgbs && t_starts && t_ends && (g_weights || g_rgbs), "render_accumulate_bwd: null pointer");
    hipStream_t s = as_stream(stream);
    const bool vec = all_aligned16(weights, rgbs, t_starts, t_ends, g_weights, g_rgbs);
    dispatch_bool(vec, [&](auto V) {
        RenderAccumBwdOp<V> op;
        op.w = weights; op.rgb = rgbs; op.ts = t_starts; op.te = t_ends;
        op.gc = g_colors; op.go = g_opacities; op.gd = g_depths; op.gw = g_weights; op.grgb = g_rgbs;
        launch_seg<1>(op, packed_info, tiles, n_rays, n_tiles, s);
    });
    NFA_CHECK_LAUNCH("render_accumulate_bwd");
    return NFA_OK;
}

int nfa_render_fused_fwd(const float *t_starts, const float *t_ends, const float *sigmas, const float *rgbs,
                         const int64_t *packed_info, const int64_t *tiles, int64_t n_tiles, int64_t n_rays, int64_t n_elems,
                         float *weights, float *trans, float *alphas, float *colors, float *opacities, float *depths,
                         nfa_stream_t stream)
{
    SEG_COMMON_CHECKS("render_fused_fwd");
    if (n_rays == 0) return NFA_OK;
    NFA_REQUIRE(colors && opacities && depths && (n_elems == 0 || (t_starts && t_ends && sigmas && rgbs)),
                "render_fused_fwd: null pointer");
    hipStream_t s = as_stream(stream);
    const bool vec = all_aligned16(t_starts, t_ends, sigmas, rgbs, weights, trans, alphas);
    dispatch_bool(vec, [&](auto V) {
        RenderFusedFwdOp<V> op;
        op.ts = t_starts; op.te = t_ends; op.sig = sigmas; op.rgb = rgbs; op.w = weights; op.tr = trans; op.al = alphas;
        op.colors = colors; op.opac = opacities; op.depth = depths;
        launch_seg<1>(op, packed_info, tiles, n_rays, n_tiles, s);
    });
    NFA_CHECK_LAUNCH("render_fused_fwd");
    return NFA_OK;
}

int nfa_render_fused_bwd(const float *t_starts, const float *t_ends, const float *rgbs, const float *trans, const float *alphas,
                         const float *g_colors, const float *g_opacities, const float *g_depths, const float *g_weights,
                         const float *g_trans, const float *g_alphas, const int64_t *packed_info, const int64_t *tiles,
                         int64_t n_tiles, int64_t n_rays, int64_t n_elems, float *grad_sigmas, float *grad_rgbs,
                         nfa_stream_t stream)
{
    SEG_COMMON_CHECKS("render_fused_bwd");
    if (n_elems == 0) return NFA_OK;
    NFA_REQUIRE(t_starts && t_ends && rgbs && trans && alphas && (grad_sigmas || grad_rgbs), "render_fused_bwd: null pointer");
    hipStream_t s = as_stream(stream);
    const bool vec = all_aligned16(t_starts, t_ends, rgbs, trans, alphas, g_weights, g_trans, g_alphas, grad_sigmas, grad_rgbs);
    const bool extra = g_weights || g_trans || g_alphas;
    dispatch_bool(vec, [&](auto V) {
        dispatch_bool(extra, [&](auto X) {
            RenderFusedBwdOp<V, X> op;
            op.ts = t_starts; op.te = t_ends; op.rgb = rgbs; op.tr = trans; op.al = alphas;
            op.gc = g_colors; op.go = g_opacities; op.gd = g_depths; op.gw = g_weights; op.gt = g_trans; op.ga = g_alphas;
            op.gsig = grad_sigmas; op.grgb = grad_rgbs;
            launch_seg<-1>(op, packed_info, tiles, n_rays, n_tiles, s);
        });
    });
    NFA_CHECK_LAUNCH("render_fused_bwd");
    return NFA_OK;
}

int nfa_distortion_fwd(const float *weights, const float *t_starts, const float *t_ends, const int64_t *packed_info,
                       const int64_t *tiles, int64_t n_tiles, int64_t n_rays, int64_t n_elems, float *loss, float *w_tot,
                       float *s_tot, nfa_stream_t stream)
{
    SEG_COMMON_CHECKS("distortion_fwd");
    if (n_rays == 0) return NFA_OK;
    NFA_REQUIRE(loss && w_tot && s_tot && (n_elems == 0 || (weights && t_starts && t_ends)), "distortion_fwd: null pointer");
    hipStream_t s = as_stream(stream);
    const bool vec = all_aligned16(weights, t_starts, t_ends);
    dispatch_bool(vec, [&](auto V) {
        DistortionFwdOp<V> op;
        op.pinfo = packed_info; op.ts = t_starts; op.te = t_ends; op.w = weights;
        op.loss = loss; op.wtot = w_tot; op.stot = s_tot;
        launch_seg<1>(op, packed_info, tiles, n_rays, n_tiles, s);
    });
    NFA_CHECK_LAUNCH("distortion_fwd");
    return NFA_OK;
}

int nfa_distortion_bwd(const float *weights, const float *t_starts, const float *t_ends, const float *w_tot, const float *s_tot,
                       const float *g_loss, const int64_t *packed_info, const int64_t *tiles, int64_t n_tiles, int64_t n_rays,
                       int64_t n_elems, float *grad_weights, float *grad_t_starts, float *grad_t_ends, nfa_stream_t stream)
{
    SEG_COMMON_CHECKS("distortion_bwd");
    if (n_elems == 0) return NFA_OK;
    NFA_REQUIRE(weights && t_starts && t_ends && w_tot && s_tot && g_loss && (grad_weights || grad_t_starts || grad_t_ends),
                "distortion_bwd: null pointer");
    hipStream_t s = as_stream(stream);
    const bool vec = all_aligned16(weights, t_starts, t_ends, grad_weights, grad_t_starts, grad_t_ends);
    dispatch_bool(vec, [&](auto V) {
        DistortionBwdOp<V> op;
        op.pinfo = packed_info; op.ts = t_starts; op.te = t_ends; op.w = weights;
        op.wtot = w_tot; op.stot = s_tot; op.gl = g_loss;
        op.gw = grad_weights; op.gts = grad_t_starts; op.gte = grad_t_ends;
        launch_seg<-1>(op, packed_info, tiles, n_rays, n_tiles, s);
    });
    NFA_CHECK_LAUNCH("distortion_bwd");
    return NFA_OK;
}

int nfa_render_step_accumulate(const float *t_starts, const float *t_ends, const float *sigmas, const float *rgbs,
                               const int64_t *packed_info, const int64_t *tiles, int64_t n_tiles, int64_t n_rays,
                               int64_t n_elems, float alpha_thre, float *colors, float *opacities, float *depths,
                               int64_t *n_visible, nfa_stream_t stream)
{
    SEG_COMMON_CHECKS("render_step_accumulate");
    if (n_elems == 0) return NFA_OK;
    NFA_REQUIRE(t_starts && t_ends && sigmas && rgbs && colors && opacities && depths, "render_step_accumulate: null pointer");
    hipStream_t s = as_stream(stream);
    const bool vec = all_aligned16(t_starts, t_ends, sigmas, rgbs);
    dispatch_bool(vec, [&](auto V) {
        RenderStepOp<V> op;
        op.ts = t_starts; op.te = t_ends; op.sig = sigmas; op.rgb = rgbs; op.thre = alpha_thre;
        op.colors = colors; op.opac = opacities; op.depth = depths;
        op.n_visible = reinterpret_cast<unsigned long long *>(n_visible);
        launch_seg<1>(op, packed_info, tiles, n_rays, n_tiles, s);
    });
    NFA_CHECK_LAUNCH("render_step_accumulate");
    return NFA_OK;
}

int nfa_sample_positions_bwd(const float *rays_o, const float *rays_d, const float *t_starts, const float *t_ends,
                             const int64_t *ray_indices, const float *g_positions, const float *g_dirs,
                             const int64_t *packed_info, const int64_t *tiles, int64_t n_tiles, int64_t n_rays, int64_t n_elems,
                             int64_t samples_per_ray, const float *aabb_host, const float *aabb, int32_t contraction,
                             int32_t dirs_mode, float *grad_rays_o, float *grad_rays_d, float *grad_t_starts,
                             float *grad_t_ends, float *grad_p, nfa_stream_t stream)
{
    NFA_REQUIRE(n_rays >= 0 && n_elems >= 0 && samples_per_ray >= 0, "sample_positions_bwd: negative size");
    NFA_REQUIRE(n_rays < ((int64_t)1 << 31) - 64, "sample_positions_bwd: too many rays");
    NFA_REQUIRE(contraction >= 0 && contraction <= 2 && dirs_mode >= 0 && dirs_mode <= 2,
                "sample_positions_bwd: contraction and dirs_mode must be 0, 1 or 2");
    const bool has_box = aabb_host || aabb;
    NFA_REQUIRE(has_box || contraction == 0, "sample_positions_bwd: contraction needs an aabb");
    NFA_REQUIRE(!(aabb_host && aabb), "sample_positions_bwd: aabb given twice");
    const bool per_ray = grad_rays_o || grad_rays_d;
    if (n_elems == 0 && (n_rays == 0 || !per_ray)) return NFA_OK;
    NFA_REQUIRE(rays_o && rays_d && t_starts && t_ends, "sample_positions_bwd: null pointer");
    NFA_REQUIRE(!g_dirs || dirs_mode != 0, "sample_positions_bwd: g_dirs needs dirs_mode");
    SampleBox box;
// ... 31 lines not shown
```

### nerfacc_amd/estimators/occ_grid.py

```python
from __future__ import annotations

import ctypes as C
from typing import Callable, List, Optional, Tuple, Union

import torch
from torch import Tensor

from .. import _backend as B
from .._segments import SegInfo, tag_ray_indices, tag_trusted
from ..grid import _enlarge_aabb, _exclusive_cumsum, _traverse_samples
from ..volrend import _visibility_native
from .base import AbstractEstimator


class TraversalHandle:

    def __init__(self, tensors, event, key):
        self._tensors, self._event, self.key = tensors, event, key

    def consume(self, stream):
        assert self._tensors is not None, "a TraversalHandle can be consumed once"
        stream.wait_event(self._event)
        tensors, self._tensors = self._tensors, None
        for t in tensors:
            t.record_stream(stream)
        seg = getattr(tensors[3], "_nfa_seg", None)
        if seg is not None and seg[2].tiles is not None:
            seg[2].tiles.record_stream(stream)
        return tensors


class OccGridEstimator(AbstractEstimator):

    DIM: int = 3

    def __init__(self, roi_aabb: Union[List[int], Tensor], resolution: Union[int, List[int], Tensor] = 128,
                 levels: int = 1, **kwargs) -> None:
        super().__init__()
        if "contraction_type" in kwargs:
            raise ValueError("`contraction_type` is not supported anymore for nerfacc >= 0.4.0.")
        if isinstance(resolution, int):
            resolution = [resolution] * self.DIM
        if isinstance(resolution, (list, tuple)):
            resolution = torch.tensor(resolution, dtype=torch.int32)
        assert isinstance(resolution, Tensor), f"Invalid type: {resolution}!"
        assert resolution.shape[0] == self.DIM, f"Invalid shape: {resolution}!"
        if isinstance(roi_aabb, (list, tuple)):
            roi_aabb = torch.tensor(roi_aabb, dtype=torch.float32)
        assert isinstance(roi_aabb, Tensor), f"Invalid type: {roi_aabb}!"
        assert roi_aabb.shape[0] == self.DIM * 2, f"Invalid shape: {roi_aabb}!"

        self.levels = levels
        self.cells_per_lvl = int(resolution.prod().item())
        aabbs = torch.stack([_enlarge_aabb(roi_aabb, 2 ** i) for i in range(levels)], dim=0)
        self.register_buffer("resolution", resolution)
        self.register_buffer("aabbs", aabbs)
        self.register_buffer("occs", torch.zeros(levels * self.cells_per_lvl))
        self.register_buffer("binaries", torch.zeros([levels] + resolution.tolist(), dtype=torch.bool))
        self.register_buffer("grid_coords", _meshgrid3d(resolution).reshape(self.cells_per_lvl, self.DIM),
                             persistent=False)
        self.register_buffer("grid_indices", torch.arange(self.cells_per_lvl), persistent=False)
        self._occs_mean_cache = None
        self._prefetch_stream = None
        self._walk_stats = {}

    def _planes(self, rays_o: Tensor, near_plane: float, far_plane: float):
        key = (rays_o.shape[0], float(near_plane), float(far_plane), rays_o.device, rays_o.dtype)
        cached = getattr(self, "_planes_cache", None)
        if cached is None or cached[0] != key:
            cached = (key, torch.full_like(rays_o[..., 0], fill_value=near_plane),
                      torch.full_like(rays_o[..., 0], fill_value=far_plane))
            self._planes_cache = cached
        return cached[1], cached[2]

    bin_rays: Optional[bool] = None

    def _occs_mean(self) -> float:
        key = (id(self.occs), self.occs.data_ptr(), self.occs._version)
        if self._occs_mean_cache is None or self._occs_mean_cache[0] != key:
            self._occs_mean_cache = (key, float(self.occs.mean().item()))
        return self._occs_mean_cache[1]

    def _traverse(self, rays_o, rays_d, near_plane, far_plane, t_min, t_max, render_step_size, stratified, cone_angle,
                  speculate=True):
        near_planes, far_planes = self._planes(rays_o, near_plane, far_plane)
        if t_min is not None:
            near_planes = torch.clamp(near_planes, min=t_min)
        if t_max is not None:
            far_planes = torch.clamp(far_planes, max=t_max)
        if stratified:
            near_planes = near_planes + torch.rand_like(near_planes) * render_step_size
        use_bins = self.bin_rays
        if use_bins is None and not cone_angle > 0.0:
            use_bins = self._walk_stats.get("max_over_mean", 1.0) > 5.0 and rays_o.shape[0] >= 65536
        return _traverse_samples(rays_o, rays_d, self.binaries, self.aabbs, near_planes, far_planes, render_step_size,
                                 cone_angle, near_hint=near_plane, bin_rays=None if use_bins is None else bool(use_bins),
                                 stats_sink=self._walk_stats, speculate=speculate)

    def _traversal_key(self, rays_o, rays_d, near_plane, far_plane, t_min, t_max, render_step_size, stratified, cone_angle):
        def tid(t):
            return None if t is None else (t.data_ptr(), tuple(t.shape), t._version)
        return (tid(rays_o), tid(rays_d), tid(t_min), tid(t_max), float(near_plane), float(far_plane),
                float(render_step_size), bool(stratified), float(cone_angle), tid(self.binaries), id(self.binaries))

    @torch.no_grad()
    def prefetch_traversal(
        self,
        rays_o: Tensor,
        rays_d: Tensor,
        near_plane: float = 0.0,
        far_plane: float = 1e10,
        t_min: Optional[Tensor] = None,
        t_max: Optional[Tensor] = None,
        render_step_size: float = 1e-3,
        stratified: bool = False,
        cone_angle: float = 0.0,
        wait_for_inputs: bool = True,
    ) -> "TraversalHandle":
        if self._prefetch_stream is None:
            try:
                self._prefetch_stream = torch.cuda.Stream(device=rays_o.device, priority=-1)
            except Exception:
                self._prefetch_stream = torch.cuda.Stream(device=rays_o.device)
        side = self._prefetch_stream
        if wait_for_inputs:
            side.wait_stream(torch.cuda.current_stream(rays_o.device))
        with torch.cuda.stream(side):
            out = self._traverse(rays_o, rays_d, near_plane, far_plane, t_min, t_max, render_step_size, stratified,
                                 cone_angle, speculate=False)
            event = torch.cuda.Event()
            event.record(side)
        key = self._traversal_key(rays_o, rays_d, near_plane, far_plane, t_min, t_max, render_step_size, stratified, cone_angle)
        return TraversalHandle(out, event, key)

    @torch.no_grad()
    def sampling(
        self,
        rays_o: Tensor,
        rays_d: Tensor,
        sigma_fn: Optional[Callable] = None,
        alpha_fn: Optional[Callable] = None,
        near_plane: float = 0.0,
        far_plane: float = 1e10,
        t_min: Optional[Tensor] = None,
        t_max: Optional[Tensor] = None,
        render_step_size: float = 1e-3,
        early_stop_eps: float = 1e-4,
        alpha_thre: float = 0.0,
        stratified: bool = False,
        cone_angle: float = 0.0,
        traversal: Optional["TraversalHandle"] = None,
    ) -> Tuple[Tensor, Tensor, Tensor]:
        if traversal is not None:
            key = self._traversal_key(rays_o, rays_d, near_plane, far_plane, t_min, t_max, render_step_size, stratified, cone_angle)
            if traversal.key != key:
                raise ValueError("nerfacc_amd: the prefetched traversal was made for other rays / planes / step / grid "
                                 "(or the ray / plane tensors were modified in place since)")
            ray_indices, t_starts, t_ends, packed_info = traversal.consume(torch.cuda.current_stream(rays_o.device))
        else:
            ray_indices, t_starts, t_ends, packed_info = self._traverse(
                rays_o, rays_d, near_plane, far_plane, t_min, t_max, render_step_size, stratified, cone_angle)

        if (alpha_thre > 0.0 or early_stop_eps > 0.0) and (sigma_fn is not None or alpha_fn is not None):
            alpha_thre = min(alpha_thre, self._occs_mean())
            seg: SegInfo = tag_trusted(packed_info, t_starts.numel())
            if sigma_fn is not None:
                if t_starts.shape[0] != 0:
                    sigmas = sigma_fn(t_starts, t_ends, ray_indices)
                else:
                    sigmas = torch.empty((0,), device=t_starts.device)
                assert sigmas.shape == t_starts.shape, "sigmas must have shape of (N,)! Got {}".format(sigmas.shape)
                vis, cnts = _visibility_native(seg, t_starts, t_ends, sigmas, None, early_stop_eps, alpha_thre, True)
            else:
                if t_starts.shape[0] != 0:
                    alphas = alpha_fn(t_starts, t_ends, ray_indices)
                else:
                    alphas = torch.empty((0,), device=t_starts.device)
                assert alphas.shape == t_starts.shape, "alphas must have shape of (N,)! Got {}".format(alphas.shape)
                vis, cnts = _visibility_native(seg, None, None, alphas, None, early_stop_eps, alpha_thre, True)
            compacted = _compact(seg, vis, cnts, t_starts, t_ends)
            if compacted is not None:
                ray_indices, t_starts, t_ends = compacted
        return ray_indices, t_starts, t_ends

    @torch.no_grad()
    def update_every_n_steps(self, step: int, occ_eval_fn: Callable, occ_thre: float = 1e-2,
                             ema_decay: float = 0.95, warmup_steps: int = 256, n: int = 16) -> None:
        if not self.training:
            raise RuntimeError(
                "You should only call this function only during training. "
                "Please call _update() directly if you want to update the field during inference.")
        if step % n == 0:
            self._update(step=step, occ_eval_fn=occ_eval_fn, occ_thre=occ_thre, ema_decay=ema_decay,
                         warmup_steps=warmup_steps)

    @torch.no_grad()
    def mark_invisible_cells(self, K: Tensor, c2w: Tensor, width: int, height: int, near_plane: float = 0.0,
                             chunk: int = 32 ** 3) -> None:
        assert K.dim() == 3 and K.shape[1:] == (3, 3)
        assert c2w.dim() == 3 and (c2w.shape[1:] == (3, 4) or c2w.shape[1:] == (4, 4))
        assert K.shape[0] == c2w.shape[0] or K.shape[0] == 1
        n_cams = c2w.shape[0]
        rot = c2w[:, :3, :3].transpose(2, 1)
        trans = -rot @ c2w[:, :3, 3:]
        for lvl, indices in enumerate(self._get_all_cells()):
            coords = self.grid_coords[indices]
            lo, hi = self.aabbs[lvl, :3], self.aabbs[lvl, 3:]
            for i in range(0, len(indices), chunk):
                ids = indices[i:i + chunk]
                world = (lo + coords[i:i + chunk] / (self.resolution - 1) * (hi - lo)).T
                uvd = K @ (rot @ world + trans)
                depth = uvd[:, 2]
                uv = uvd[:, :2] / uvd[:, 2:]
                in_image = (depth >= 0) & (uv[:, 0] >= 0) & (uv[:, 0] < width) & (uv[:, 1] >= 0) & (uv[:, 1] < height)
                seen = ((depth >= near_plane) & in_image).sum(0) / n_cams > 0
                too_near = ((depth < near_plane) & in_image).any(0)
                self.occs[lvl * self.cells_per_lvl + ids] = torch.where(seen & ~too_near, 0.0, -1.0)

    @torch.no_grad()
    def _get_all_cells(self) -> List[Tensor]:
        out = []
        for lvl in range(self.levels):
            keep = self.occs[lvl * self.cells_per_lvl + self.grid_indices] >= 0.0
            out.append(self.grid_indices[keep])
        return out

    @torch.no_grad()
    def _sample_uniform_and_occupied_cells(self, n: int) -> List[Tensor]:
        if self.occs.is_cuda and self.levels * self.cells_per_lvl <= self.ONE_READ_MAX_CELLS:
            return self._sample_cells_one_read(n)
        dev, L, cells = self.occs.device, self.levels, self.cells_per_lvl
        out = []
        for lvl in range(L):
            uni = torch.randint(cells, (n,), device=dev)
            uni = uni[self.occs[lvl * cells + uni] >= 0.0]
            occ = torch.nonzero(self.binaries[lvl].flatten())[:, 0]
            if n < len(occ):
                occ = occ[torch.randint(len(occ), (n,), device=dev)]
            out.append(torch.cat([uni, occ], dim=0))
        return out

    ONE_READ_MAX_CELLS = 1 << 27

    @torch.no_grad()
    def _sample_cells_one_read(self, n: int) -> List[Tensor]:
        dev, L, cells = self.occs.device, self.levels, self.cells_per_lvl
        uni = torch.randint(cells, (L, n), device=dev)
        uni_ok = self.occs.view(L, cells).gather(1, uni) >= 0.0
        uni_pos = torch.cumsum(uni_ok, dim=1, dtype=torch.int32)
        occ_flag = self.binaries.view(L, cells)
        occ_pos = torch.cumsum(occ_flag, dim=1, dtype=torch.int32)
        sizes = torch.stack([uni_pos[:, -1], occ_pos[:, -1]], dim=1).tolist()
        out = []
        cell_ids = torch.arange(cells, device=dev)
        for lvl, (n_uni, n_occ) in enumerate(sizes):
# ... 38 lines not shown
            for lvl, indices in enumerate(lvl_indices):
                jitter = torch.rand((indices.shape[0], self.DIM), dtype=torch.float32, device=indices.device)
                x = self._cell_points(lvl, indices, jitter)
                occ = occ_eval_fn(x).squeeze(-1)
                self._ema_update(lvl, indices, occ, ema_decay)
        self._rebinarize(occ_thre)

    def _cell_points(self, lvl: int, indices: Tensor, jitter: Tensor) -> Tensor:
        if not indices.is_cuda:
            unit = (self.grid_coords[indices] + jitter) / self.resolution
            return self.aabbs[lvl, :3] + unit * (self.aabbs[lvl, 3:] - self.aabbs[lvl, :3])
        n = indices.shape[0]
        x = torch.empty((n, self.DIM), dtype=torch.float32, device=indices.device)
        res = (C.c_int32 * 3)(*[int(v) for v in self.binaries.shape[1:]])
        with torch.cuda.device(indices.device):
            B.call("nfa_grid_cell_points", B.ptr(indices.contiguous()), B.ptr(jitter.contiguous()), n, res,
                   self.aabbs.data_ptr() + 24 * lvl, B.ptr(x), B.stream())
        return x

    def _ema_update(self, lvl: int, indices: Tensor, occ: Tensor, ema_decay: float) -> None:
        if not self.occs.is_cuda:
            cell_ids = lvl * self.cells_per_lvl + indices
            self.occs[cell_ids] = torch.maximum(self.occs[cell_ids] * ema_decay, occ)
            return
        n = indices.shape[0]
        occ = occ.to(torch.float32).contiguous()
        assert occ.shape == (n,), "occ_eval_fn must return one value per position"
        scratch = torch.empty(n, dtype=torch.float32, device=self.occs.device)
        with torch.cuda.device(self.occs.device):
            B.call("nfa_grid_ema_update", B.ptr(self.occs), lvl * self.cells_per_lvl, B.ptr(indices.contiguous()), n, B.ptr(occ),
                   float(ema_decay), B.ptr(scratch), B.stream())
        self._occs_mean_cache = None

    def _rebinarize(self, occ_thre: float) -> None:
        if not self.occs.is_cuda:
            thre = torch.clamp(self.occs[self.occs >= 0].mean(), max=occ_thre)
            self.binaries = (self.occs > thre).view(self.binaries.shape)
            return
        from ..grid import _walk_supported
        dev = self.occs.device
        shape = tuple(self.binaries.shape)
        if not _walk_supported(self.binaries):
            thre = torch.clamp(self.occs[self.occs >= 0].mean(), max=occ_thre)
            self.binaries = (self.occs > thre).view(self.binaries.shape)
            return
        res = (C.c_int32 * 3)(*shape[1:])
        binaries = torch.empty(shape, dtype=torch.bool, device=dev)
        bits = torch.empty(int(B.load().nfa_walk_bits_words(shape[0], res)), dtype=torch.int32, device=dev)
        scratch = torch.empty(int(B.load().nfa_grid_rebinarize_scratch_bytes()) // 8 + 1, dtype=torch.float64, device=dev)
        with torch.cuda.device(dev):
            B.call("nfa_grid_rebinarize", B.ptr(self.occs), shape[0], res, float(occ_thre), B.ptr(binaries), B.ptr(bits),
                   B.ptr(scratch), B.stream())
        binaries._nfa_walk_bits = (binaries._version, bits)
        self.binaries = binaries
        self._occs_mean_cache = None


_PINNED_READ = __import__("os").environ.get("NERFACC_AMD_PINNED_READ", "1") != "0"
_PINNED_TOTALS: dict = {}


def _pinned_total(dev) -> Tensor:
    buf = _PINNED_TOTALS.get(dev.index)
    if buf is None:
        buf = _PINNED_TOTALS[dev.index] = torch.empty(1, dtype=torch.int64, pin_memory=True)
    return buf


_KEPT_FRACTION: dict = {}
_SPECULATE_COMPACTION = __import__("os").environ.get("NERFACC_AMD_SPECULATE_COMPACTION", "1") != "0"


def _compact(seg: SegInfo, vis: Tensor, cnts: Tensor, t_starts: Tensor, t_ends: Tensor):
    dev = t_starts.device
    n = t_starts.numel()
    key = (seg.n_rays, dev.index)
    with torch.cuda.device(dev):
        total = torch.empty(1, dtype=torch.int64, device=dev)
        out_starts = _exclusive_cumsum(cnts, total)
        frac = _KEPT_FRACTION.get(key, 1.0) if _SPECULATE_COMPACTION else 1.0
        host = _pinned_total(dev)
        ri = ts = te = None
        cap = 0

        def run(ri, ts, te, capacity):
            B.call("nfa_compact_samples", B.ptr(vis), B.ptr(t_starts), B.ptr(t_ends), B.ptr(seg.packed_info),
                   B.ptr(seg.tiles), seg.n_tiles, B.ptr(out_starts), seg.n_rays, n, B.ptr(ri), B.ptr(ts), B.ptr(te), capacity, B.stream())

        if frac < 1.0 and n > 0:
            cap = min(n, ((int(n * min(1.0, frac * 1.03)) + 8192) // 4096) * 4096)
            main = torch.cuda.current_stream()
            ready = torch.cuda.Event(); ready.record(main)
            from ..grid import _side_stream
            side = _side_stream(dev)
            with torch.cuda.stream(side):
                side.wait_event(ready)
                host.copy_(total, non_blocking=True)
                done = torch.cuda.Event(); done.record(side)
            ri = torch.empty(cap, dtype=torch.int64, device=dev)
            ts = torch.empty(cap, dtype=torch.float32, device=dev)
            te = torch.empty(cap, dtype=torch.float32, device=dev)
            run(ri, ts, te, cap)
            done.synchronize()
            m = int(host[0])
        elif _PINNED_READ:
            host.copy_(total, non_blocking=True)
            done = torch.cuda.Event(); done.record()
            done.synchronize()
            m = int(host[0])
        else:
            m = int(total.item())
        if n > 0:
            _KEPT_FRACTION[key] = m / n
        if m == n:
            return None
        if cap > 0 and m <= cap:
            ri, ts, te = ri[:m], ts[:m], te[:m]
        else:
            ri = torch.empty(m, dtype=torch.int64, device=dev)
            ts = torch.empty(m, dtype=torch.float32, device=dev)
            te = torch.empty(m, dtype=torch.float32, device=dev)
            if m > 0:
                run(ri, ts, te, m)
        packed = torch.stack([out_starts, cnts], dim=-1)
    info = tag_trusted(packed, m)
    tag_ray_indices(ri, seg.n_rays, info)
    return ri, ts, te


def _meshgrid3d(res: Tensor, device: Union[torch.device, str] = "cpu") -> Tensor:
    assert len(res) == 3
    axes = [torch.arange(int(r), dtype=torch.long) for r in res.tolist()]
    return torch.stack(torch.meshgrid(axes, indexing="ij"), dim=-1).to(device)
```

### nerfacc_amd/grid.py

```python
from __future__ import annotations

import ctypes as C
import os
from typing import Optional, Tuple

import torch
from torch import Tensor

from . import _backend as B
from ._segments import tag_ray_indices, tag_trusted
from .data_specs import RayIntervals, RaySamples


@torch.no_grad()
def ray_aabb_intersect(
    rays_o: Tensor,
    rays_d: Tensor,
    aabbs: Tensor,
    near_plane: float = -float("inf"),
    far_plane: float = float("inf"),
    miss_value: float = float("inf"),
) -> Tuple[Tensor, Tensor, Tensor]:
    assert rays_o.ndim == 2 and rays_o.shape[-1] == 3
    assert rays_d.ndim == 2 and rays_d.shape[-1] == 3
    assert aabbs.ndim == 2 and aabbs.shape[-1] == 6
    dev = B.require_device(rays_o, rays_d, aabbs)
    rays_o, rays_d, aabbs = rays_o.float().contiguous(), rays_d.float().contiguous(), aabbs.float().contiguous()
    n, m = rays_o.shape[0], aabbs.shape[0]
    t_mins = torch.empty((n, m), dtype=torch.float32, device=dev)
    t_maxs = torch.empty((n, m), dtype=torch.float32, device=dev)
    hits = torch.empty((n, m), dtype=torch.bool, device=dev)
    with torch.cuda.device(dev):
        B.call("nfa_ray_aabb_intersect", B.ptr(rays_o), B.ptr(rays_d), n, B.ptr(aabbs), m, float(near_plane),
               float(far_plane), float(miss_value), B.ptr(t_mins), B.ptr(t_maxs), B.ptr(hits), B.stream())
    return t_mins, t_maxs, hits


def _traverse_args(rays_o, rays_d, rays_mask, binaries, aabbs, t_sorted, t_indices, hits, near_planes, far_planes,
                   step_size, cone_angle, limit, mode) -> B.TraverseArgs:
    a = B.TraverseArgs()
    a.n_rays = rays_o.shape[0]
    a.rays_o, a.rays_d, a.rays_mask = B.ptr(rays_o), B.ptr(rays_d), B.ptr(rays_mask)
    a.n_grids = binaries.shape[0]
    a.res[0], a.res[1], a.res[2] = binaries.shape[1], binaries.shape[2], binaries.shape[3]
    a.binaries, a.aabbs = B.ptr(binaries), B.ptr(aabbs)
    a.hits, a.t_sorted, a.t_indices = B.ptr(hits), B.ptr(t_sorted), B.ptr(t_indices)
    a.near_planes, a.far_planes = B.ptr(near_planes), B.ptr(far_planes)
    a.step_size, a.cone_angle = float(step_size), float(cone_angle)
    a.traverse_steps_limit, a.mode = int(limit), int(mode)
    bricks, coarse = _get_bricks(binaries)
    a._keepalive = (bricks, coarse)
    a.bricks, a.coarse = B.ptr(bricks), B.ptr(coarse)
    return a


def _launch(a: B.TraverseArgs) -> None:
    B.call("nfa_traverse_grids", C.byref(a), B.stream())


def _exclusive_cumsum(cnts: Tensor, total_out: Tensor):
    starts = torch.empty_like(cnts)
    scratch = B.cumsum_scratch(cnts.numel(), cnts.device)
    B.call("nfa_exclusive_cumsum_i64", B.ptr(cnts), cnts.numel(), B.ptr(starts), B.ptr(total_out), B.ptr(scratch),
           B.stream())
    return starts


def _cumsum_packed(cnts: Tensor, total_out: Tensor, stats: bool = False) -> Tensor:
    packed = torch.empty((cnts.numel(), 2), dtype=torch.int64, device=cnts.device)
    scratch = B.cumsum_scratch(cnts.numel(), cnts.device)
    B.call("nfa_exclusive_cumsum_pairs_stats_i64" if stats else "nfa_exclusive_cumsum_pairs_i64", B.ptr(cnts), cnts.numel(),
           B.ptr(packed), B.ptr(total_out), B.ptr(scratch), B.stream())
    return packed


MAX_EVENT_LEVELS = 8


def ray_events(rays_o: Tensor, rays_d: Tensor, aabbs: Tensor):
    G = aabbs.shape[0]
    if G > MAX_EVENT_LEVELS or not rays_o.is_cuda:
        t_mins, t_maxs, hits = ray_aabb_intersect(rays_o, rays_d, aabbs)
        t_sorted, t_indices = torch.sort(torch.cat([t_mins, t_maxs], dim=-1), dim=-1)
        return t_sorted, t_indices, hits
    dev = B.require_device(rays_o, rays_d, aabbs)
    rays_o, rays_d, aabbs = rays_o.float().contiguous(), rays_d.float().contiguous(), aabbs.float().contiguous()
    n = rays_o.shape[0]
    t_sorted = torch.empty((n, 2 * G), dtype=torch.float32, device=dev)
    t_indices = torch.empty((n, 2 * G), dtype=torch.int64, device=dev)
    hits = torch.empty((n, G), dtype=torch.bool, device=dev)
    with torch.cuda.device(dev):
        B.call("nfa_ray_events", B.ptr(rays_o), B.ptr(rays_d), n, B.ptr(aabbs), G, B.ptr(t_sorted), B.ptr(t_indices),
               B.ptr(hits), B.stream())
# ... 320 lines not shown
            _launch(a)
        packed_info = _cumsum_packed(sm_cnts, meta[0:3], stats=True)
        cap = _SPEC_CAPACITY.get(spec_key, 0) if (SPECULATE and speculate and use_runs) else 0
        t_starts = t_ends = ray_indices = None
        if cap > 0:
            host = _pinned_meta(dev)
            main = torch.cuda.current_stream()
            ready = torch.cuda.Event(); ready.record(main)
            side = _side_stream(dev)
            with torch.cuda.stream(side):
                side.wait_event(ready)
                host[:6].copy_(meta, non_blocking=True)
                done = torch.cuda.Event(); done.record(side)
            t_starts = torch.empty(cap, dtype=torch.float32, device=dev)
            t_ends = torch.empty(cap, dtype=torch.float32, device=dev)
            ray_indices = torch.empty(cap, dtype=torch.int64, device=dev)
            B.call("nfa_expand_runs", n_rays, float(step_size), B.ptr(run_cnts), B.ptr(runs), MAX_RUNS,
                   B.ptr(packed_info), B.ptr(t_starts), B.ptr(t_ends), None, B.ptr(ray_indices), cap, B.stream())
            done.synchronize()
            n_sm, s_max, s_sum, n_overflow, c_max, c_sum = (int(v) for v in host[:6].tolist())
        else:
            n_sm, s_max, s_sum, n_overflow, c_max, c_sum = (int(v) for v in meta.tolist())
        n_overflow, off_lattice = n_overflow & 0xFFFFFFFF, n_overflow >> 32
        n_arena = 0
        if use_cone_runs and arena is not None:
            n_arena, off_lattice = min(off_lattice, arena_cap), 0
        if off_lattice and use_runs and near_hint is not None:
            return _traverse_samples(rays_o, rays_d, binaries, aabbs, near_planes, far_planes, step_size, cone_angle,
                                     rays_mask=rays_mask, traverse_steps_limit=traverse_steps_limit, t_sorted=t_sorted,
                                     t_indices=t_indices, hits=hits, return_terminate=return_terminate, near_hint=None,
                                     bin_rays=bin_rays, stats_sink=stats_sink, speculate=speculate, n_alive=n_alive,
                                     alive_list=alive_list)
        if stats_sink is not None and c_sum > 0:
            stats_sink["cells_max_over_mean"] = 64.0 * c_max / c_sum
        if SPECULATE and use_runs:
            _SPEC_CAPACITY[spec_key] = ((int(n_sm * 1.03) + 4096) // 4096) * 4096
        if stats_sink is not None and s_sum > 0:
            stats_sink["max_over_mean"] = 64.0 * s_max / s_sum
        expanded = cap > 0 and n_sm <= cap
        if expanded:
            t_starts, t_ends, ray_indices = t_starts[:n_sm], t_ends[:n_sm], ray_indices[:n_sm]
        else:
            t_starts = torch.empty(n_sm, dtype=torch.float32, device=dev)
            t_ends = torch.empty(n_sm, dtype=torch.float32, device=dev)
            ray_indices = torch.empty(n_sm, dtype=torch.int64, device=dev)
        if n_sm > 0:
            main = torch.cuda.current_stream()
            joined = None
            if (use_runs or use_cone_runs) and n_overflow > 0:
                sm_starts = packed_info[:, 0].contiguous()
                side = _side_stream(dev)
                side.wait_stream(main)
                with torch.cuda.stream(side):
                    a.mode = 1
                    a.terminate_planes = None
                    a.sm_starts = B.ptr(sm_starts)
                    a.sm_t_starts, a.sm_t_ends, a.sm_ray_indices = B.ptr(t_starts), B.ptr(t_ends), B.ptr(ray_indices)
                    a.ray_filter, a.ray_filter_min = B.ptr(run_cnts), MAX_RUNS
                    _launch(a)
                    joined = torch.cuda.Event()
                    joined.record(side)
            if use_runs and not expanded:
                B.call("nfa_expand_runs", n_rays, float(step_size), B.ptr(run_cnts), B.ptr(runs), MAX_RUNS,
                       B.ptr(packed_info), B.ptr(t_starts), B.ptr(t_ends), None, B.ptr(ray_indices), n_sm, B.stream())
            elif use_cone_runs:
                B.call("nfa_expand_cone_runs", n_rays, float(step_size), float(cone_angle), B.ptr(run_cnts), B.ptr(runs),
                       MAX_RUNS, B.ptr(packed_info), B.ptr(t_starts), B.ptr(t_ends), B.ptr(ray_indices), B.stream())
                if n_arena > 0:
                    B.call("nfa_expand_cone_arena", B.ptr(arena), n_arena, float(step_size), float(cone_angle), B.ptr(packed_info),
                           B.ptr(t_starts), B.ptr(t_ends), B.ptr(ray_indices), B.stream())
            if joined is not None:
                main.wait_event(joined)
            if not (use_runs or use_cone_runs):
                a.mode = 1
                a.terminate_planes = None
                sm_starts = packed_info[:, 0].contiguous()
                a.sm_starts = B.ptr(sm_starts)
                a.sm_t_starts, a.sm_t_ends = B.ptr(t_starts), B.ptr(t_ends)
                a.sm_ray_indices = None
                _launch(a)
                B.call("nfa_fill_ray_indices", n_rays, B.ptr(packed_info), B.ptr(ray_indices), B.stream())
    info = tag_trusted(packed_info, n_sm)
    tag_ray_indices(ray_indices, n_rays, info)
    out = (ray_indices, t_starts, t_ends, packed_info)
    return (*out, terminate) if return_terminate else out


def _enlarge_aabb(aabb: Tensor, factor: float) -> Tensor:
    center = (aabb[:3] + aabb[3:]) / 2
    extent = (aabb[3:] - aabb[:3]) / 2
    return torch.cat([center - extent * factor, center + extent * factor])


def _query(x: Tensor, data: Tensor, base_aabb: Tensor) -> Tuple[Tensor, Tensor]:
    lo, hi = base_aabb[:3], base_aabb[3:]
    u = (x - lo) / (hi - lo)
    r = (u - 0.5).abs().amax(dim=-1).clamp_min(0.1)
    mip = (torch.frexp(r)[1].long() + 1).clamp_min(0)
    inside = mip < data.shape[0]
    uu = (u - 0.5) / (2 ** mip)[:, None] + 0.5
    res = torch.tensor(data.shape[1:], device=x.device)
    ix = torch.minimum((uu * res).long(), res - 1)
    lvl = mip.clamp_max(data.shape[0] - 1)
    return data[lvl, ix[:, 0], ix[:, 1], ix[:, 2]] * inside, inside
```

### nerfacc_amd/volrend.py

```python
from __future__ import annotations

from typing import Callable, Dict, Optional, Tuple

import torch
from torch import Tensor
from torch.autograd.function import once_differentiable

from . import _backend as B
from ._segments import SegInfo, batched_native, resolve, seginfo_from_ray_indices
from .scan import exclusive_prod, exclusive_sum


FUSE_RENDERING = True


def _f32c(t: Optional[Tensor]) -> Optional[Tensor]:
    if t is None:
        return None
    if t.dtype != torch.float32:
        raise TypeError("nerfacc_amd: packed rendering ops support float32 only")
    return t.contiguous()


class _RenderFromDensity(torch.autograd.Function):

    @staticmethod
    def forward(ctx, t_starts, t_ends, sigmas, prefix_trans, seg: SegInfo, want_weights: bool):
        ctx.set_materialize_grads(False)
        ts, te, sg, pf = _f32c(t_starts), _f32c(t_ends), _f32c(sigmas), _f32c(prefix_trans)
        dev = B.require_device(ts, te, sg, pf)
        n = sg.numel()
        weights = torch.empty_like(sg) if want_weights else None
        trans, alphas = torch.empty_like(sg), torch.empty_like(sg)
        if n:
            with torch.cuda.device(dev):
                B.call("nfa_render_from_density_fwd", B.ptr(ts), B.ptr(te), B.ptr(sg), B.ptr(pf),
                       B.ptr(seg.packed_info), B.ptr(seg.tiles), seg.n_tiles, seg.n_rays, n, B.ptr(weights), B.ptr(trans),
                       B.ptr(alphas), B.stream())
        ctx.seg = seg
        ctx.want_weights = want_weights
        ctx.save_for_backward(ts, te, sg, trans, alphas)
        if not want_weights:
            weights = trans.new_empty(0)
            ctx.mark_non_differentiable(weights)
        return weights, trans, alphas

    @staticmethod
    @once_differentiable
    def backward(ctx, g_w, g_t, g_a):
        ts, te, sg, trans, alphas = ctx.saved_tensors
        seg = ctx.seg
        n = sg.numel()
        need_ts, need_te, need_sg = ctx.needs_input_grad[0], ctx.needs_input_grad[1], ctx.needs_input_grad[2]
        if ctx.needs_input_grad[3]:
            raise NotImplementedError("nerfacc_amd: gradient w.r.t. prefix_trans is not implemented")
        g_w = None if (g_w is None or not ctx.want_weights) else _f32c(g_w)
        g_t = None if g_t is None else _f32c(g_t)
        g_a = None if g_a is None else _f32c(g_a)
        need_x = need_ts or need_te
        g_sig = torch.empty_like(sg) if need_sg else None
        g_x = torch.empty_like(sg) if need_x else None
        if n and (need_sg or need_x):
            with torch.cuda.device(sg.device):
                B.call("nfa_render_from_density_bwd", B.ptr(ts), B.ptr(te), B.ptr(trans), B.ptr(alphas), B.ptr(g_w),
                       B.ptr(g_t), B.ptr(g_a), B.ptr(seg.packed_info), B.ptr(seg.tiles), seg.n_tiles, seg.n_rays, n,
                       B.ptr(g_sig), B.ptr(g_x), B.stream())
        g_ts = (-(g_x * sg)) if need_ts else None
        g_te = (g_x * sg) if need_te else None
        return g_ts, g_te, g_sig, None, None, None


class _RenderFromAlpha(torch.autograd.Function):

    @staticmethod
    def forward(ctx, alphas, prefix_trans, seg: SegInfo, want_weights: bool):
        ctx.set_materialize_grads(False)
        al, pf = _f32c(alphas), _f32c(prefix_trans)
        dev = B.require_device(al, pf)
        n = al.numel()
        weights = torch.empty_like(al) if want_weights else None
        trans = torch.empty_like(al)
        if n:
            with torch.cuda.device(dev):
                B.call("nfa_render_from_alpha_fwd", B.ptr(al), B.ptr(pf), B.ptr(seg.packed_info), B.ptr(seg.tiles), seg.n_tiles,
                       seg.n_rays, n, B.ptr(weights), B.ptr(trans), B.stream())
        ctx.seg, ctx.want_weights = seg, want_weights
        ctx.save_for_backward(al, trans)
        if not want_weights:
            weights = trans.new_empty(0)
            ctx.mark_non_differentiable(weights)
        return weights, trans

# ... 9 lines not shown
        g_w = None if (g_w is None or not ctx.want_weights) else _f32c(g_w)
        g_t = None if g_t is None else _f32c(g_t)
        g_al = torch.empty_like(al)
        if al.numel():
            with torch.cuda.device(al.device):
                B.call("nfa_render_from_alpha_bwd", B.ptr(al), B.ptr(trans), B.ptr(g_w), B.ptr(g_t),
                       B.ptr(seg.packed_info), B.ptr(seg.tiles), seg.n_tiles, seg.n_rays, al.numel(), B.ptr(g_al), B.stream())
        return g_al, None, None, None


class _Accumulate(torch.autograd.Function):

    @staticmethod
    def forward(ctx, weights, values, seg: SegInfo):
        ctx.set_materialize_grads(False)
        w, v = _f32c(weights), _f32c(values)
        dev = B.require_device(w, v)
        D = 1 if v is None else v.shape[-1]
        out = torch.empty((seg.n_rays, D), dtype=torch.float32, device=dev)
        if seg.n_rays and D:
            with torch.cuda.device(dev):
                B.call("nfa_accumulate_along_rays", B.ptr(w), B.ptr(v), D, B.ptr(seg.packed_info), B.ptr(seg.tiles), seg.n_tiles,
                       seg.n_rays, w.numel(), 0, B.ptr(out), B.stream())
        ctx.seg, ctx.D, ctx.has_values = seg, D, v is not None
        ctx.save_for_backward(w, v if v is not None else w.new_empty(0))
        return out

    @staticmethod
    @once_differentiable
    def backward(ctx, g_out):
        w, v = ctx.saved_tensors
        v = v if ctx.has_values else None
        seg = ctx.seg
        g_out = _f32c(g_out)
        need_w, need_v = ctx.needs_input_grad[0], ctx.needs_input_grad[1] and v is not None
        g_w = torch.empty_like(w) if need_w else None
        g_v = torch.empty_like(v) if need_v else None
        if w.numel() and (need_w or need_v):
            with torch.cuda.device(w.device):
                B.call("nfa_accumulate_along_rays_bwd", B.ptr(w), B.ptr(v), ctx.D, B.ptr(g_out),
                       B.ptr(seg.packed_info), B.ptr(seg.tiles), seg.n_tiles, seg.n_rays, w.numel(), B.ptr(g_w), B.ptr(g_v),
                       B.stream())
        return g_w, g_v, None


class _RenderAccumulate(torch.autograd.Function):

    @staticmethod
    def forward(ctx, weights, rgbs, t_starts, t_ends, seg: SegInfo):
        ctx.set_materialize_grads(False)
        w, c, ts, te = _f32c(weights), _f32c(rgbs), _f32c(t_starts), _f32c(t_ends)
        dev = B.require_device(w, c, ts, te)
        R = seg.n_rays
        colors = torch.empty((R, 3), dtype=torch.float32, device=dev)
        opac = torch.empty((R, 1), dtype=torch.float32, device=dev)
        depth = torch.empty((R, 1), dtype=torch.float32, device=dev)
        if R:
            with torch.cuda.device(dev):
                B.call("nfa_render_accumulate_fwd", B.ptr(w), B.ptr(c), B.ptr(ts), B.ptr(te), B.ptr(seg.packed_info),
                       B.ptr(seg.tiles), seg.n_tiles, R, w.numel(), B.ptr(colors), B.ptr(opac), B.ptr(depth), B.stream())
        ctx.seg = seg
        ctx.save_for_backward(w, c, ts, te)
        return colors, opac, depth

    @staticmethod
    @once_differentiable
    def backward(ctx, g_c, g_o, g_d):
        w, c, ts, te = ctx.saved_tensors
        seg = ctx.seg
        need_w, need_c = ctx.needs_input_grad[0], ctx.needs_input_grad[1]
        g_w = torch.empty_like(w) if need_w else None
        g_rgb = torch.empty_like(c) if need_c else None
        if w.numel() and (need_w or need_c):
            with torch.cuda.device(w.device):
                B.call("nfa_render_accumulate_bwd", B.ptr(w), B.ptr(c), B.ptr(ts), B.ptr(te), B.ptr(_f32c(g_c)),
                       B.ptr(_f32c(g_o)), B.ptr(_f32c(g_d)), B.ptr(seg.packed_info), B.ptr(seg.tiles), seg.n_tiles, seg.n_rays,
                       w.numel(), B.ptr(g_w), B.ptr(g_rgb), B.stream())
        return g_w, g_rgb, None, None, None


class _RenderFused(torch.autograd.Function):

    @staticmethod
    def forward(ctx, t_starts, t_ends, sigmas, rgbs, seg: SegInfo):
        ctx.set_materialize_grads(False)
        ts, te, sg, c = _f32c(t_starts), _f32c(t_ends), _f32c(sigmas), _f32c(rgbs)
        dev = B.require_device(ts, te, sg, c)
        R, n = seg.n_rays, sg.numel()
        weights, trans, alphas = torch.empty_like(sg), torch.empty_like(sg), torch.empty_like(sg)
        colors = torch.empty((R, 3), dtype=torch.float32, device=dev)
        opac = torch.empty((R, 1), dtype=torch.float32, device=dev)
        depth = torch.empty((R, 1), dtype=torch.float32, device=dev)
        if R:
            with torch.cuda.device(dev):
                B.call("nfa_render_fused_fwd", B.ptr(ts), B.ptr(te), B.ptr(sg), B.ptr(c), B.ptr(seg.packed_info),
                       B.ptr(seg.tiles), seg.n_tiles, R, n, B.ptr(weights), B.ptr(trans), B.ptr(alphas), B.ptr(colors),
                       B.ptr(opac), B.ptr(depth), B.stream())
        ctx.seg = seg
        ctx.save_for_backward(ts, te, c, trans, alphas)
        return colors, opac, depth, weights, trans, alphas

    @staticmethod
    @once_differentiable
    def backward(ctx, g_c, g_o, g_d, g_w, g_t, g_a):
        ts, te, c, trans, alphas = ctx.saved_tensors
        seg = ctx.seg
        if ctx.needs_input_grad[0] or ctx.needs_input_grad[1]:
            raise NotImplementedError("nerfacc_amd: rendering is not differentiable w.r.t. t_starts / t_ends "
                                      "(same contract as the reference, volrend.py:33-35)")
        need_sg, need_c = ctx.needs_input_grad[2], ctx.needs_input_grad[3]
        g_sig = torch.empty_like(trans) if need_sg else None
        g_rgb = torch.empty_like(c) if need_c else None
        if trans.numel() and (need_sg or need_c):
            with torch.cuda.device(trans.device):
                B.call("nfa_render_fused_bwd", B.ptr(ts), B.ptr(te), B.ptr(c), B.ptr(trans), B.ptr(alphas),
                       B.ptr(_f32c(g_c)), B.ptr(_f32c(g_o)), B.ptr(_f32c(g_d)), B.ptr(_f32c(g_w)), B.ptr(_f32c(g_t)),
                       B.ptr(_f32c(g_a)), B.ptr(seg.packed_info), B.ptr(seg.tiles), seg.n_tiles, seg.n_rays,
                       trans.numel(), B.ptr(g_sig), B.ptr(g_rgb), B.stream())
        return None, None, g_sig, g_rgb, None


def _use_fused(seg: Optional[SegInfo], *tensors: Optional[Tensor]) -> bool:
    if seg is None or not seg.contiguous:
        return False
    return all(t is None or (t.dim() == 1 and t.dtype == torch.float32) for t in tensors)


def _prefix_needs_grad(prefix_trans: Optional[Tensor]) -> bool:
    return prefix_trans is not None and prefix_trans.requires_grad and torch.is_grad_enabled()


def rendering(
    t_starts: Tensor,
    t_ends: Tensor,
    ray_indices: Optional[Tensor] = None,
    n_rays: Optional[int] = None,
    rgb_sigma_fn: Optional[Callable] = None,
    rgb_alpha_fn: Optional[Callable] = None,
    render_bkgd: Optional[Tensor] = None,
) -> Tuple[Tensor, Tensor, Tensor, Dict]:
    if ray_indices is not None:
        assert (
            t_starts.shape == t_ends.shape == ray_indices.shape
        ), "Since nerfacc 0.5.0, t_starts, t_ends and ray_indices must have the same shape (N,). "
    if rgb_sigma_fn is None and rgb_alpha_fn is None:
        raise ValueError("At least one of `rgb_sigma_fn` and `rgb_alpha_fn` should be specified.")

    seg = None
    if ray_indices is not None and ray_indices.is_cuda:
        assert n_rays is not None, "n_rays must be provided"
        seg = seginfo_from_ray_indices(ray_indices, n_rays)

    if rgb_sigma_fn is not None:
        if t_starts.shape[0] != 0:
            rgbs, sigmas = rgb_sigma_fn(t_starts, t_ends, ray_indices)
        else:
            rgbs = torch.empty((0, 3), device=t_starts.device)
            sigmas = torch.empty((0,), device=t_starts.device)
        assert rgbs.shape[-1] == 3, "rgbs must have 3 channels, got {}".format(rgbs.shape)
        assert sigmas.shape == t_starts.shape, "sigmas must have shape of (N,)! Got {}".format(sigmas.shape)
        if FUSE_RENDERING and seg is not None and seg.sorted_indices and _use_fused(seg, sigmas, t_starts, t_ends) \
                and rgbs.dtype == torch.float32 and rgbs.dim() == 2 \
                and not (t_starts.requires_grad or t_ends.requires_grad):
            colors, opacities, depths, weights, trans, alphas = _RenderFused.apply(t_starts, t_ends, sigmas, rgbs, seg)
            extras = {"weights": weights, "alphas": alphas, "trans": trans, "sigmas": sigmas, "rgbs": rgbs}
            return _finish_rendering(colors, opacities, depths, extras, rgbs, render_bkgd)
        weights, trans, alphas = render_weight_from_density(
            t_starts, t_ends, sigmas, ray_indices=ray_indices, n_rays=n_rays
        )
        extras = {"weights": weights, "alphas": alphas, "trans": trans, "sigmas": sigmas, "rgbs": rgbs}
    else:
        if t_starts.shape[0] != 0:
            rgbs, alphas = rgb_alpha_fn(t_starts, t_ends, ray_indices)
        else:
            rgbs = torch.empty((0, 3), device=t_starts.device)
            alphas = torch.empty((0,), device=t_starts.device)
        assert rgbs.shape[-1] == 3, "rgbs must have 3 channels, got {}".format(rgbs.shape)
        assert alphas.shape == t_starts.shape, "alphas must have shape of (N,)! Got {}".format(alphas.shape)
        weights, trans = render_weight_from_alpha(alphas, ray_indices=ray_indices, n_rays=n_rays)
        extras = {"weights": weights, "trans": trans, "rgbs": rgbs, "alphas": alphas}

    if seg is not None and seg.sorted_indices and _use_fused(seg, weights, t_starts, t_ends) \
            and rgbs.dtype == torch.float32:
        colors, opacities, depths = _RenderAccumulate.apply(weights, rgbs, t_starts, t_ends, seg)
    else:
        colors = accumulate_along_rays(weights, values=rgbs, ray_indices=ray_indices, n_rays=n_rays)
        opacities = accumulate_along_rays(weights, values=None, ray_indices=ray_indices, n_rays=n_rays)
        depths = accumulate_along_rays(
            weights, values=(t_starts + t_ends)[..., None] / 2.0, ray_indices=ray_indices, n_rays=n_rays
        )
    return _finish_rendering(colors, opacities, depths, extras, rgbs, render_bkgd)


def _finish_rendering(colors, opacities, depths, extras, rgbs, render_bkgd):
    depths = depths / opacities.clamp_min(torch.finfo(rgbs.dtype).eps)
    if render_bkgd is not None:
        colors = colors + render_bkgd * (1.0 - opacities)
    return colors, opacities, depths, extras


def _batched_as_packed(fn, tensors, packed_info, ray_indices, **kw):
    if packed_info is not None or ray_indices is not None:
        return None
    useg = batched_native(*tensors)
    if useg is None:
        return None
    shape = next(t for t in tensors if t is not None).shape
    flat = [None if t is None else t.contiguous().view(-1) for t in tensors]
    out = fn(*flat[:-1], packed_info=useg.packed_info, prefix_trans=flat[-1], **kw)
    return tuple(o.view(shape) for o in out) if isinstance(out, tuple) else out.view(shape)


def render_transmittance_from_alpha(
    alphas: Tensor,
    packed_info: Optional[Tensor] = None,
    ray_indices: Optional[Tensor] = None,
    n_rays: Optional[int] = None,
    prefix_trans: Optional[Tensor] = None,
) -> Tensor:
    out = _batched_as_packed(render_transmittance_from_alpha, (alphas, prefix_trans), packed_info, ray_indices)
    if out is not None:
        return out
    seg = resolve(alphas.numel(), packed_info, ray_indices, n_rays) if alphas.dim() == 1 else None
    if _use_fused(seg, alphas, prefix_trans) and not _prefix_needs_grad(prefix_trans):
        _, trans = _RenderFromAlpha.apply(alphas, prefix_trans, seg, False)
        return trans
    trans = exclusive_prod(1 - alphas, seg.packed_info if seg is not None else None)
    if prefix_trans is not None:
        trans = trans * prefix_trans
    return trans


def render_transmittance_from_density(
    t_starts: Tensor,
    t_ends: Tensor,
    sigmas: Tensor,
    packed_info: Optional[Tensor] = None,
    ray_indices: Optional[Tensor] = None,
    n_rays: Optional[int] = None,
    prefix_trans: Optional[Tensor] = None,
) -> Tuple[Tensor, Tensor]:
    out = _batched_as_packed(render_transmittance_from_density, (t_starts, t_ends, sigmas, prefix_trans), packed_info, ray_indices)
    if out is not None:
        return out
    seg = resolve(sigmas.numel(), packed_info, ray_indices, n_rays) if sigmas.dim() == 1 else None
    if _use_fused(seg, t_starts, t_ends, sigmas, prefix_trans) and not _prefix_needs_grad(prefix_trans):
        _, trans, alphas = _RenderFromDensity.apply(t_starts, t_ends, sigmas, prefix_trans, seg, False)
        return trans, alphas
    sigmas_dt = sigmas * (t_ends - t_starts)
    alphas = 1.0 - torch.exp(-sigmas_dt)
    trans = torch.exp(-exclusive_sum(sigmas_dt, seg.packed_info if seg is not None else None))
    if prefix_trans is not None:
        trans = trans * prefix_trans
    return trans, alphas


def render_weight_from_alpha(
    alphas: Tensor,
    packed_info: Optional[Tensor] = None,
    ray_indices: Optional[Tensor] = None,
    n_rays: Optional[int] = None,
    prefix_trans: Optional[Tensor] = None,
) -> Tuple[Tensor, Tensor]:
    out = _batched_as_packed(render_weight_from_alpha, (alphas, prefix_trans), packed_info, ray_indices)
    if out is not None:
        return out
    seg = resolve(alphas.numel(), packed_info, ray_indices, n_rays) if alphas.dim() == 1 else None
    if _use_fused(seg, alphas, prefix_trans) and not _prefix_needs_grad(prefix_trans):
        return _RenderFromAlpha.apply(alphas, prefix_trans, seg, True)
    trans = render_transmittance_from_alpha(alphas, seg.packed_info if seg is not None else None,
                                            None, None, prefix_trans)
    return trans * alphas, trans


def render_weight_from_density(
    t_starts: Tensor,
    t_ends: Tensor,
    sigmas: Tensor,
    packed_info: Optional[Tensor] = None,
    ray_indices: Optional[Tensor] = None,
    n_rays: Optional[int] = None,
    prefix_trans: Optional[Tensor] = None,
) -> Tuple[Tensor, Tensor, Tensor]:
    out = _batched_as_packed(render_weight_from_density, (t_starts, t_ends, sigmas, prefix_trans), packed_info, ray_indices)
    if out is not None:
        return out
    seg = resolve(sigmas.numel(), packed_info, ray_indices, n_rays) if sigmas.dim() == 1 else None
    if _use_fused(seg, t_starts, t_ends, sigmas, prefix_trans) and not _prefix_needs_grad(prefix_trans):
        return _RenderFromDensity.apply(t_starts, t_ends, sigmas, prefix_trans, seg, True)
    trans, alphas = render_transmittance_from_density(
        t_starts, t_ends, sigmas, seg.packed_info if seg is not None else None, None, None, prefix_trans)
    return trans * alphas, trans, alphas


def _visibility_native(seg: SegInfo, t_starts, t_ends, vals, prefix_trans, early_stop_eps, alpha_thre,
                       want_counts: bool = False):
    ts, te, v, pf = _f32c(t_starts), _f32c(t_ends), _f32c(vals), _f32c(prefix_trans)
    dev = B.require_device(v, ts, te, pf)
    n = v.numel()
    vis = torch.empty(n, dtype=torch.bool, device=dev)
    cnts = torch.empty(seg.n_rays, dtype=torch.int64, device=dev) if want_counts else None
    with torch.cuda.device(dev):
        B.call("nfa_render_visibility", B.ptr(ts), B.ptr(te), B.ptr(v), B.ptr(pf), float(early_stop_eps),
               float(alpha_thre), B.ptr(seg.packed_info), B.ptr(seg.tiles), seg.n_tiles, seg.n_rays, n, B.ptr(vis), B.ptr(cnts),
               B.stream())
    return (vis, cnts) if want_counts else vis


@torch.no_grad()
def render_visibility_from_alpha(
    alphas: Tensor,
    packed_info: Optional[Tensor] = None,
    ray_indices: Optional[Tensor] = None,
    n_rays: Optional[int] = None,
    early_stop_eps: float = 1e-4,
    alpha_thre: float = 0.0,
    prefix_trans: Optional[Tensor] = None,
) -> Tensor:
    out = _batched_as_packed(render_visibility_from_alpha, (alphas, prefix_trans), packed_info, ray_indices, early_stop_eps=early_stop_eps, alpha_thre=alpha_thre)
    if out is not None:
        return out
    seg = resolve(alphas.numel(), packed_info, ray_indices, n_rays) if alphas.dim() == 1 else None
    if _use_fused(seg, alphas, prefix_trans):
        return _visibility_native(seg, None, None, alphas, prefix_trans, early_stop_eps, alpha_thre)
    trans = render_transmittance_from_alpha(alphas, seg.packed_info if seg is not None else None, None, None,
                                            prefix_trans)
    vis = trans >= early_stop_eps
    if alpha_thre > 0:
        vis = vis & (alphas >= alpha_thre)
    return vis


@torch.no_grad()
def render_visibility_from_density(
    t_starts: Tensor,
    t_ends: Tensor,
    sigmas: Tensor,
    packed_info: Optional[Tensor] = None,
    ray_indices: Optional[Tensor] = None,
    n_rays: Optional[int] = None,
    early_stop_eps: float = 1e-4,
    alpha_thre: float = 0.0,
    prefix_trans: Optional[Tensor] = None,
) -> Tensor:
    out = _batched_as_packed(render_visibility_from_density, (t_starts, t_ends, sigmas, prefix_trans), packed_info, ray_indices, early_stop_eps=early_stop_eps, alpha_thre=alpha_thre)
    if out is not None:
        return out
    seg = resolve(sigmas.numel(), packed_info, ray_indices, n_rays) if sigmas.dim() == 1 else None
    if _use_fused(seg, t_starts, t_ends, sigmas, prefix_trans):
        return _visibility_native(seg, t_starts, t_ends, sigmas, prefix_trans, early_stop_eps, alpha_thre)
    trans, alphas = render_transmittance_from_density(
        t_starts, t_ends, sigmas, seg.packed_info if seg is not None else None, None, None, prefix_trans)
    vis = trans >= early_stop_eps
    if alpha_thre > 0:
        vis = vis & (alphas >= alpha_thre)
    return vis


def accumulate_along_rays(
    weights: Tensor,
    values: Optional[Tensor] = None,
    ray_indices: Optional[Tensor] = None,
    n_rays: Optional[int] = None,
) -> Tensor:
    if values is not None:
        assert values.dim() == weights.dim() + 1
        assert weights.shape == values.shape[:-1]
    if ray_indices is not None:
        assert n_rays is not None, "n_rays must be provided"
        assert weights.dim() == 1, "weights must be flattened"
        if weights.is_cuda and weights.dtype == torch.float32 and (values is None or values.dtype == torch.float32):
            seg = seginfo_from_ray_indices(ray_indices, n_rays)
            if seg.sorted_indices:
                return _Accumulate.apply(weights, values, seg)
        src = weights[..., None] if values is None else weights[..., None] * values
        outputs = torch.zeros((n_rays, src.shape[-1]), device=src.device, dtype=src.dtype)
        outputs.index_add_(0, ray_indices, src)
        return outputs
    src = weights[..., None] if values is None else weights[..., None] * values
    return torch.sum(src, dim=-2)


def accumulate_along_rays_(
    weights: Tensor,
    values: Optional[Tensor] = None,
    ray_indices: Optional[Tensor] = None,
# ... 32 lines not shown
```

Before: 740.8 million rays/s.

## Recompute t_ends from t_starts and step size instead of loading them in render kernels

Tags t_starts/t_ends produced by grid traversal and compaction with the step size and cone angle. Visibility, compaction and fused render fwd/bwd kernels then recompute t_end = t_start + calc_dt(t_start) instead of reading the t_ends array. This removes one float stream of global-memory reads per sample in several bandwidth-bound passes. It adds a small amount of arithmetic, and Python-side tag validation that could fall back to explicit ends if the tensors were modified.

```diff
diff --git a/include/nerfacc_hip.h b/include/nerfacc_hip.h
--- a/include/nerfacc_hip.h
+++ b/include/nerfacc_hip.h
@@ -184,6 +184,14 @@
                         const int64_t *packed_info, const int64_t *tiles, int64_t n_tiles, const int64_t *out_starts,
                         int64_t n_rays, int64_t n_elems, int64_t *out_ray_indices,
                         float *out_t_starts, float *out_t_ends, int64_t capacity, nfa_stream_t stream);
+int nfa_render_visibility_implied(const float *t_starts, float step_size, float cone_angle, const float *sigmas,
+                                  const float *prefix_trans, float early_stop_eps, float alpha_thre,
+                                  const int64_t *packed_info, const int64_t *tiles, int64_t n_tiles, int64_t n_rays,
+                                  int64_t n_elems, uint8_t *vis, int64_t *vis_cnts, nfa_stream_t stream);
+int nfa_compact_samples_implied(const uint8_t *vis, const float *t_starts, float step_size, float cone_angle,
+                                const int64_t *packed_info, const int64_t *tiles, int64_t n_tiles, const int64_t *out_starts,
+                                int64_t n_rays, int64_t n_elems, int64_t *out_ray_indices,
+                                float *out_t_starts, float *out_t_ends, int64_t capacity, nfa_stream_t stream);
 
 int nfa_accumulate_along_rays(const float *weights, const float *values, int32_t D,
                               const int64_t *packed_info, const int64_t *tiles, int64_t n_tiles, int64_t n_rays,
@@ -215,6 +223,16 @@
                          const float *g_alphas, const int64_t *packed_info, const int64_t *tiles, int64_t n_tiles,
                          int64_t n_rays, int64_t n_elems, float *grad_sigmas, float *grad_rgbs,
                          nfa_stream_t stream);
+int nfa_render_fused_fwd_implied(const float *t_starts, float step_size, float cone_angle, const float *sigmas,
+                                 const float *rgbs, const int64_t *packed_info, const int64_t *tiles, int64_t n_tiles,
+                                 int64_t n_rays, int64_t n_elems, float *weights, float *trans, float *alphas,
+                                 float *colors, float *opacities, float *depths, nfa_stream_t stream);
+int nfa_render_fused_bwd_implied(const float *t_starts, float step_size, float cone_angle, const float *rgbs,
+                                 const float *trans, const float *alphas, const float *g_colors,
+                                 const float *g_opacities, const float *g_depths, const float *g_weights,
+                                 const float *g_trans, const float *g_alphas, const int64_t *packed_info,
+                                 const int64_t *tiles, int64_t n_tiles, int64_t n_rays, int64_t n_elems,
+                                 float *grad_sigmas, float *grad_rgbs, nfa_stream_t stream);
 
 int nfa_distortion_fwd(const float *weights, const float *t_starts, const float *t_ends, const int64_t *packed_info,
                        const int64_t *tiles, int64_t n_tiles, int64_t n_rays, int64_t n_elems, float *loss, float *w_tot,
diff --git a/nerfacc_amd/_backend.py b/nerfacc_amd/_backend.py
--- a/nerfacc_amd/_backend.py
+++ b/nerfacc_amd/_backend.py
@@ -85,6 +85,8 @@
     "nfa_render_from_alpha_bwd": [_vp, _vp, _vp, _vp, _vp, _vp, _i64, _i64, _i64, _vp, _vp],
     "nfa_render_visibility": [_vp, _vp, _vp, _vp, _f32, _f32, _vp, _vp, _i64, _i64, _i64, _vp, _vp, _vp],
     "nfa_compact_samples": [_vp, _vp, _vp, _vp, _vp, _i64, _vp, _i64, _i64, _vp, _vp, _vp, _i64, _vp],
+    "nfa_render_visibility_implied": [_vp, _f32, _f32, _vp, _vp, _f32, _f32, _vp, _vp, _i64, _i64, _i64, _vp, _vp, _vp],
+    "nfa_compact_samples_implied": [_vp, _vp, _f32, _f32, _vp, _vp, _i64, _vp, _i64, _i64, _vp, _vp, _vp, _i64, _vp],
     "nfa_accumulate_along_rays": [_vp, _vp, _i32, _vp, _vp, _i64, _i64, _i64, _int, _vp, _vp],
     "nfa_accumulate_along_rays_atomic": [_vp, _vp, _i32, _vp, _i64, _i64, _vp, _vp],
     "nfa_accumulate_along_rays_bwd": [_vp, _vp, _i32, _vp, _vp, _vp, _i64, _i64, _i64, _vp, _vp, _vp],
@@ -92,6 +94,8 @@
     "nfa_render_accumulate_bwd": [_vp, _vp, _vp, _vp, _vp, _vp, _vp, _vp, _vp, _i64, _i64, _i64, _vp, _vp, _vp],
     "nfa_render_fused_fwd": [_vp, _vp, _vp, _vp, _vp, _vp, _i64, _i64, _i64, _vp, _vp, _vp, _vp, _vp, _vp, _vp],
     "nfa_render_fused_bwd": [_vp] * 13 + [_i64, _i64, _i64, _vp, _vp, _vp],
+    "nfa_render_fused_fwd_implied": [_vp, _f32, _f32, _vp, _vp, _vp, _vp, _i64, _i64, _i64, _vp, _vp, _vp, _vp, _vp, _vp, _vp],
+    "nfa_render_fused_bwd_implied": [_vp, _f32, _f32] + [_vp] * 11 + [_i64, _i64, _i64, _vp, _vp, _vp],
     "nfa_render_step_accumulate": [_vp, _vp, _vp, _vp, _vp, _vp, _i64, _i64, _i64, _f32, _vp, _vp, _vp, _vp, _vp],
     "nfa_distortion_fwd": [_vp, _vp, _vp, _vp, _vp, _i64, _i64, _i64, _vp, _vp, _vp, _vp],
     "nfa_distortion_bwd": [_vp] * 8 + [_i64, _i64, _i64, _vp, _vp, _vp, _vp],
@@ -159,8 +163,25 @@
     """Counterpart of the RuntimeError TORCH_CHECK raises in the reference."""
 
 
+class ImpliedEnds:
+    __slots__ = ("step", "cone")
+
+    def __init__(self, step: float, cone: float):
+        self.step, self.cone = float(step), float(cone)
+
+
+_ENDS_SLOT = {"nfa_render_visibility": 1, "nfa_compact_samples": 2, "nfa_render_fused_fwd": 1, "nfa_render_fused_bwd": 1}
+call_log: Optional[list] = None
+
+
 def call(name: str, *args) -> None:
     lib = load()
+    slot = _ENDS_SLOT.get(name)
+    if slot is not None and isinstance(args[slot], ImpliedEnds):
+        e = args[slot]
+        name, args = name + "_implied", args[:slot] + (e.step, e.cone) + args[slot + 1:]
+    if call_log is not None:
+        call_log.append(name)
     rc = getattr(lib, name)(*args)
     if rc != 0:
         msg = lib.nfa_last_error()
diff --git a/nerfacc_amd/_segments.py b/nerfacc_amd/_segments.py
--- a/nerfacc_amd/_segments.py
+++ b/nerfacc_amd/_segments.py
@@ -90,6 +90,26 @@
     setattr(ray_indices, _ATTR_RI, (ray_indices._version, n_rays, info))
 
 
+_ATTR_ENDS = "_nfa_implied_ends"
+
+
+def tag_implied_ends(t_starts: Tensor, t_ends: Tensor, step: float, cone: float) -> None:
+    if not float(step) > 0.0:
+        return
+    setattr(t_ends, _ATTR_ENDS, (t_ends._version, t_starts, t_starts.data_ptr(), t_starts._version, float(step), float(cone)))
+
+
+def implied_ends(t_starts: Optional[Tensor], t_ends: Optional[Tensor]) -> "Optional[B.ImpliedEnds]":
+    tag = getattr(t_ends, _ATTR_ENDS, None) if t_ends is not None else None
+    if tag is None:
+        return None
+    version, partner, ptr, partner_version, step, cone = tag
+    if (version != t_ends._version or partner is not t_starts or t_starts.data_ptr() != ptr
+            or t_starts._version != partner_version or t_starts.shape != t_ends.shape):
+        return None
+    return B.ImpliedEnds(step, cone)
+
+
 def resolve(n_elems: int, packed_info: Optional[Tensor], ray_indices: Optional[Tensor],
             n_rays: Optional[int]) -> Optional[SegInfo]:
     if packed_info is not None:
diff --git a/nerfacc_amd/csrc/segscan.hip b/nerfacc_amd/csrc/segscan.hip
--- a/nerfacc_amd/csrc/segscan.hip
+++ b/nerfacc_amd/csrc/segscan.hip
@@ -1,6 +1,7 @@
 #include <stdlib.h>
 
 #include "common.hip.h"
+#include "march.h"
 #include "samples.h"
 
 namespace nfa {
@@ -103,6 +104,27 @@
     }
 }
 
+template <bool IMPL>
+struct Ends {
+    const float *p;
+    template <bool VEC>
+    __device__ __forceinline__ void fetch(const Pos &q, F4 &b) const { ld4<VEC>(p, q, b); }
+    __device__ __forceinline__ F4 get(const F4 &, const F4 &b) const { return b; }
+};
+template <>
+struct Ends<true> {
+    float step, cone;
+    template <bool VEC>
+    __device__ __forceinline__ void fetch(const Pos &, F4 &) const {}
+    __device__ __forceinline__ F4 get(const F4 &a, const F4 &) const
+    {
+        F4 e;
+#pragma unroll
+        for (int j = 0; j < SE; ++j) e.v[j] = a.v[j] + calc_dt(a.v[j], cone, step);
+        return e;
+    }
+};
+
 struct StepHeads {
     int32_t lh[SE];
     uint32_t acc;
@@ -731,11 +753,12 @@
     __device__ __forceinline__ void store(const Pos &q) { store4<VEC>(galpha, q, res); }
 };
 
-template <bool DENSITY, bool VEC, bool COUNT>
+template <bool DENSITY, bool VEC, bool COUNT, bool IMPL = false>
 struct VisibilityOp : OpBase {
     static constexpr int NCHB = COUNT ? 1 : 0;
     struct Raw { F4 s, pf, a, b; };
-    const float *ts, *te, *val, *prefix;
+    const float *ts, *val, *prefix;
+    Ends<IMPL> te;
     float eps, thre;
     float s_lo, s_hi;
     uint8_t *vis;
@@ -750,17 +773,19 @@
         if (prefix) ld4<VEC>(prefix, q, r.pf);
         if (DENSITY) {
             ld4<VEC>(ts, q, r.a);
-            ld4<VEC>(te, q, r.b);
+            te.template fetch<VEC>(q, r.b);
         }
     }
     __device__ __forceinline__ void load(const Raw &r, const Pos &pos)
     {
         const bool *valid = pos.valid;
+        F4 e;
+        if (DENSITY) e = te.get(r.a, r.b);
 #pragma unroll
         for (int j = 0; j < SE; ++j) {
             pf[j] = prefix ? r.pf.v[j] : 1.0f;
             const float sv = sel(r.s, j, valid, 0.0f);
-            if (DENSITY) { x0[j] = valid[j] ? sv * (r.b.v[j] - r.a.v[j]) : 0.0f; a4[j] = (thre > 0.0f) ? 1.0f - expf(-x0[j]) : 1.0f; }
+            if (DENSITY) { x0[j] = valid[j] ? sv * (e.v[j] - r.a.v[j]) : 0.0f; a4[j] = (thre > 0.0f) ? 1.0f - expf(-x0[j]) : 1.0f; }
             else { a4[j] = sv; x0[j] = 1.0f - sv; }
         }
     }
@@ -829,14 +854,15 @@
     return (valid[j] && ((m.w[j / 4] >> (8 * (j % 4))) & 0xFFu)) ? 1.0f : 0.0f;
 }
 
-template <bool VEC>
+template <bool VEC, bool IMPL = false>
 struct CompactOp : OpBase {
     static constexpr int RAY_CAP = 192;
     static constexpr int RAY_LDS_FLOATS = 3 * SEG_CHUNK + 2 * RAY_CAP;
     struct Raw { U4 m; F4 a, b; };
     const uint8_t *vis;
     int vis_vec;
-    const float *ts, *te;
+    const float *ts;
+    Ends<IMPL> te;
     const int64_t *out_starts;
     int64_t *o_ri;
     float *o_ts, *o_te;
@@ -861,13 +887,14 @@
     {
         load_mask4(vis, vis_vec != 0, q, r.m);
         ld4<VEC>(ts, q, r.a);
-        ld4<VEC>(te, q, r.b);
+        te.template fetch<VEC>(q, r.b);
     }
     __device__ __forceinline__ void load(const Raw &r, const Pos &pos)
     {
         const bool *valid = pos.valid;
-#pragma unroll
-        for (int j = 0; j < SE; ++j) { m[j] = mask_sel(r.m, j, valid); a[j] = r.a.v[j]; b[j] = r.b.v[j]; }
+        const F4 e = te.get(r.a, r.b);
+#pragma unroll
+        for (int j = 0; j < SE; ++j) { m[j] = mask_sel(r.m, j, valid); a[j] = r.a.v[j]; b[j] = e.v[j]; }
     }
     __device__ __forceinline__ float x(int j, int) const { return m[j]; }
     __device__ __forceinline__ void emit(int j, int64_t, bool, bool is_head, int rid, int, const float *, const float prev[1])
@@ -1195,17 +1222,18 @@
     }
 };
 
-template <bool VEC>
+template <bool VEC, bool IMPL = false>
 struct RenderFusedFwdOp : OpBase {
     static constexpr int NCHB = 5;
     struct Raw { F4 a, b, s; float c[3 * SE]; };
-    const float *ts, *te, *sig, *rgb;
+    const float *ts, *sig, *rgb;
+    Ends<IMPL> te;
     float *w, *tr, *al, *colors, *opac, *depth;
     float xs[SE], mid[SE], rw[SE], rt[SE], ra[SE], c[3 * SE];
     __device__ __forceinline__ void fetch(const Pos &q, Raw &r) const
     {
         ld4<VEC>(ts, q, r.a);
-        ld4<VEC>(te, q, r.b);
+        te.template fetch<VEC>(q, r.b);
         ld4<VEC>(sig, q, r.s);
         load_rgb12(rgb, VEC, q, r.c);
     }
@@ -1213,10 +1241,11 @@
     {
         const bool *valid = pos.valid;
         fix_rgb12(rgb, VEC, pos, r.c, c);
+        const F4 e = te.get(r.a, r.b);
 #pragma unroll
         for (int j = 0; j < SE; ++j) {
-            xs[j] = valid[j] ? r.s.v[j] * (r.b.v[j] - r.a.v[j]) : 0.0f;
-            mid[j] = (r.a.v[j] + r.b.v[j]) / 2.0f;
+            xs[j] = valid[j] ? r.s.v[j] * (e.v[j] - r.a.v[j]) : 0.0f;
+            mid[j] = (r.a.v[j] + e.v[j]) / 2.0f;
         }
     }
     __device__ __forceinline__ float x(int j, int) const { return xs[j]; }
@@ -1316,14 +1345,15 @@
     }
 };
 
-template <bool VEC, bool EXTRA >
+template <bool VEC, bool EXTRA , bool IMPL = false>
 struct RenderFusedBwdOp : OpBase {
     static constexpr bool NEEDS_RID = true;
     static constexpr int RAY_CAP = 192;
     static constexpr int RAY_LDS_FLOATS = 8 * RAY_CAP;
     static constexpr bool PIPE = true;
     struct Raw { F4 a, b, T, A, gw, gt, ga; float c[3 * SE]; };
-    const float *ts, *te, *rgb, *tr, *al, *gc, *go, *gd, *gw, *gt, *ga;
+    const float *ts, *rgb, *tr, *al, *gc, *go, *gd, *gw, *gt, *ga;
+    Ends<IMPL> te;
     float *gsig, *grgb;
     const float *g_lds = nullptr;
     int32_t g_lo = 0, g_n = 0;
@@ -1345,7 +1375,7 @@
     __device__ __forceinline__ void fetch(const Pos &q, Raw &r) const
     {
         ld4<VEC>(ts, q, r.a);
-        ld4<VEC>(te, q, r.b);
+        te.template fetch<VEC>(q, r.b);
         ld4<VEC>(tr, q, r.T);
         ld4<VEC>(al, q, r.A);
         if (EXTRA) {
@@ -1359,14 +1389,15 @@
     {
         const bool *valid = pos.valid;
         fix_rgb12(rgb, VEC, pos, r.c, c);
+        const F4 e = te.get(r.a, r.b);
 #pragma unroll
         for (int j = 0; j < SE; ++j) {
             T[j] = sel(r.T, j, valid, 0.0f); A[j] = sel(r.A, j, valid, 0.0f);
             GW[j] = (EXTRA && gw && valid[j]) ? r.gw.v[j] : 0.0f;
             GT[j] = (EXTRA && gt && valid[j]) ? r.gt.v[j] : 0.0f;
             GA[j] = (EXTRA && ga && valid[j]) ? r.ga.v[j] : 0.0f;
-            dlt[j] = r.b.v[j] - r.a.v[j];
-            mid[j] = (r.a.v[j] + r.b.v[j]) / 2.0f;
+            dlt[j] = e.v[j] - r.a.v[j];
+            mid[j] = (r.a.v[j] + e.v[j]) / 2.0f;
         }
     }
     __device__ __forceinline__ void pre(int j, int64_t, bool valid, int rid)
@@ -1690,6 +1721,95 @@
     if (n_elems == 0 && n_rays == 0) return NFA_OK;                                                      \
     NFA_REQUIRE(packed_info && tiles && n_tiles >= 1, name ": packed_info/tiles is null")
 
+#define SEG_IMPLIED_CHECKS(name)                                                                                       \
+    NFA_REQUIRE(isfinite(step_size) && step_size > 0.0f, name ": step_size must be finite and > 0 (got %g)", (double)step_size); \
+    NFA_REQUIRE(isfinite(cone_angle) && cone_angle >= 0.0f, name ": cone_angle must be finite and >= 0 (got %g)", (double)cone_angle)
+
+static inline Ends<false> explicit_ends(const float *t_ends) { return Ends<false>{t_ends}; }
+static inline Ends<true> implied_ends(float step_size, float cone_angle) { return Ends<true>{step_size, cone_angle}; }
+static inline const float *ends_pointer(const Ends<false> &e) { return e.p; }
+static inline const float *ends_pointer(const Ends<true> &) { return nullptr; }
+
+template <bool IMPL>
+static void launch_visibility(const float *t_starts, Ends<IMPL> ends, const float *sigmas_or_alphas, const float *prefix_trans,
+                              float early_stop_eps, float alpha_thre, const int64_t *packed_info, const int64_t *tiles,
+                              int64_t n_tiles, int64_t n_rays, uint8_t *vis, int64_t *vis_cnts, hipStream_t s)
+{
+    const bool density = t_starts != nullptr;
+    float s_lo, s_hi;
+    if (early_stop_eps > 0.0f) {
+        const double L = -log((double)early_stop_eps);
+        const double w = 2e-5 * (L > 1.0 ? L : 1.0);
+        s_lo = (float)(L - w); s_hi = (float)(L + w);
+    } else {
+        s_lo = INFINITY; s_hi = INFINITY;
+    }
+    const bool vec = all_aligned16(t_starts, ends_pointer(ends), sigmas_or_alphas, prefix_trans) &&
+                     (reinterpret_cast<uintptr_t>(vis) & 3) == 0;
+    dispatch_bool(density, [&](auto DN) {
+        dispatch_bool(vec, [&](auto V) {
+            dispatch_bool(vis_cnts != nullptr, [&](auto CN) {
+                VisibilityOp<DN, V, CN, IMPL && DN> op;
+                op.ts = t_starts; op.val = sigmas_or_alphas; op.prefix = prefix_trans;
+                if constexpr (IMPL && DN) op.te = ends;
+                else op.te = explicit_ends(ends_pointer(ends));
+                op.eps = early_stop_eps; op.thre = alpha_thre; op.vis = vis; op.cnts = vis_cnts; op.s_lo = s_lo; op.s_hi = s_hi;
+                launch_seg<1>(op, packed_info, tiles, n_rays, n_tiles, s);
+            });
+        });
+    });
+}
+
+template <bool IMPL>
+static void launch_compact(const uint8_t *vis, const float *t_starts, Ends<IMPL> ends, const int64_t *packed_info,
+                           const int64_t *tiles, int64_t n_tiles, const int64_t *out_starts, int64_t n_rays,
+                           int64_t *out_ray_indices, float *out_t_starts, float *out_t_ends, int64_t capacity, hipStream_t s)
+{
+    const bool vec = all_aligned16(t_starts, ends_pointer(ends));
+    dispatch_bool(vec, [&](auto V) {
+        CompactOp<V, IMPL> op;
+        op.vis = vis; op.vis_vec = (reinterpret_cast<uintptr_t>(vis) & 3) == 0; op.ts = t_starts; op.te = ends;
+        op.out_starts = out_starts; op.o_ri = out_ray_indices; op.o_ts = out_t_starts; op.o_te = out_t_ends; op.cap = capacity;
+        launch_seg<1>(op, packed_info, tiles, n_rays, n_tiles, s);
+    });
+}
+
+template <bool IMPL>
+static void launch_render_fused_fwd(const float *t_starts, Ends<IMPL> ends, const float *sigmas, const float *rgbs,
+                                    const int64_t *packed_info, const int64_t *tiles, int64_t n_tiles, int64_t n_rays,
+                                    float *weights, float *trans, float *alphas, float *colors, float *opacities,
+                                    float *depths, hipStream_t s)
+{
+    const bool vec = all_aligned16(t_starts, ends_pointer(ends), sigmas, rgbs, weights, trans, alphas);
+    dispatch_bool(vec, [&](auto V) {
+        RenderFusedFwdOp<V, IMPL> op;
+        op.ts = t_starts; op.te = ends; op.sig = sigmas; op.rgb = rgbs; op.w = weights; op.tr = trans; op.al = alphas;
+        op.colors = colors; op.opac = opacities; op.depth = depths;
+        launch_seg<1>(op, packed_info, tiles, n_rays, n_tiles, s);
+    });
+}
+
+template <bool IMPL>
+static void launch_render_fused_bwd(const float *t_starts, Ends<IMPL> ends, const float *rgbs, const float *trans,
+                                    const float *alphas, const float *g_colors, const float *g_opacities,
+                                    const float *g_depths, const float *g_weights, const float *g_trans, const float *g_alphas,
+                                    const int64_t *packed_info, const int64_t *tiles, int64_t n_tiles, int64_t n_rays,
+                                    float *grad_sigmas, float *grad_rgbs, hipStream_t s)
+{
+    const bool vec = all_aligned16(t_starts, ends_pointer(ends), rgbs, trans, alphas, g_weights, g_trans, g_alphas, grad_sigmas,
+                                   grad_rgbs);
+    const bool extra = g_weights || g_trans || g_alphas;
+    dispatch_bool(vec, [&](auto V) {
+        dispatch_bool(extra, [&](auto X) {
+            RenderFusedBwdOp<V, X, IMPL> op;
+            op.ts = t_starts; op.te = ends; op.rgb = rgbs; op.tr = trans; op.al = alphas;
+            op.gc = g_colors; op.go = g_opacities; op.gd = g_depths; op.gw = g_weights; op.gt = g_trans; op.ga = g_alphas;
+            op.gsig = grad_sigmas; op.grgb = grad_rgbs;
+            launch_seg<-1>(op, packed_info, tiles, n_rays, n_tiles, s);
+        });
+    });
+}
+
 extern "C" {
 
 void nfa_seg_plan(int64_t n_elems, int64_t n_rays, int64_t *tile_elems, int64_t *n_tiles)
@@ -1907,30 +2027,32 @@
         NFA_REQUIRE(sigmas_or_alphas && vis, "render_visibility: null pointer");
         const bool density = t_starts != nullptr;
         NFA_REQUIRE(!density || t_ends, "render_visibility: t_ends is null");
-        float s_lo, s_hi;
-        if (early_stop_eps > 0.0f) {
-            const double L = -log((double)early_stop_eps);
-            const double w = 2e-5 * (L > 1.0 ? L : 1.0);
-            s_lo = (float)(L - w); s_hi = (float)(L + w);
-        } else {
-            s_lo = INFINITY; s_hi = INFINITY;
-        }
-        const bool vec = all_aligned16(t_starts, t_ends, sigmas_or_alphas, prefix_trans) &&
-                         (reinterpret_cast<uintptr_t>(vis) & 3) == 0;
-        dispatch_bool(density, [&](auto DN) {
-            dispatch_bool(vec, [&](auto V) {
-                dispatch_bool(vis_cnts != nullptr, [&](auto CN) {
-                    VisibilityOp<DN, V, CN> op;
-                    op.ts = t_starts; op.te = t_ends; op.val = sigmas_or_alphas; op.prefix = prefix_trans;
-                    op.eps = early_stop_eps; op.thre = alpha_thre; op.vis = vis; op.cnts = vis_cnts; op.s_lo = s_lo; op.s_hi = s_hi;
-                    launch_seg<1>(op, packed_info, tiles, n_rays, n_tiles, s);
-                });
-            });
-        });
+        launch_visibility(t_starts, explicit_ends(t_ends), sigmas_or_alphas, prefix_trans, early_stop_eps, alpha_thre, packed_info,
+                          tiles, n_tiles, n_rays, vis, vis_cnts, s);
     } else if (vis_cnts && n_rays > 0) {
         if (hipMemsetAsync(vis_cnts, 0, sizeof(int64_t) * n_rays, s) != hipSuccess) { set_error("render_visibility: memset failed"); return NFA_EHIP; }
     }
     NFA_CHECK_LAUNCH("render_visibility");
+    return NFA_OK;
+}
+
+int nfa_render_visibility_implied(const float *t_starts, float step_size, float cone_angle, const float *sigmas,
+                                  const float *prefix_trans, float early_stop_eps, float alpha_thre,
+                                  const int64_t *packed_info, const int64_t *tiles, int64_t n_tiles, int64_t n_rays, int64_t n_elems,
+                                  uint8_t *vis, int64_t *vis_cnts, nfa_stream_t stream)
+{
+    SEG_IMPLIED_CHECKS("render_visibility_implied");
+    SEG_COMMON_CHECKS("render_visibility_implied");
+    hipStream_t s = as_stream(stream);
+    if (n_elems > 0) {
+        NFA_REQUIRE(sigmas && vis, "render_visibility_implied: null pointer");
+        NFA_REQUIRE(t_starts, "render_visibility_implied: t_starts is null (the density form only)");
+        launch_visibility(t_starts, implied_ends(step_size, cone_angle), sigmas, prefix_trans, early_stop_eps, alpha_thre,
+                          packed_info, tiles, n_tiles, n_rays, vis, vis_cnts, s);
+    } else if (vis_cnts && n_rays > 0) {
+        if (hipMemsetAsync(vis_cnts, 0, sizeof(int64_t) * n_rays, s) != hipSuccess) { set_error("render_visibility_implied: memset failed"); return NFA_EHIP; }
+    }
+    NFA_CHECK_LAUNCH("render_visibility_implied");
     return NFA_OK;
 }
 
@@ -1942,15 +2064,25 @@
     if (n_elems == 0) return NFA_OK;
     NFA_REQUIRE(vis && t_starts && t_ends && out_starts, "compact_samples: null input");
     NFA_REQUIRE(capacity >= 0, "compact_samples: negative capacity");
-    hipStream_t s = as_stream(stream);
-    const bool vec = all_aligned16(t_starts, t_ends);
-    dispatch_bool(vec, [&](auto V) {
-        CompactOp<V> op;
-        op.vis = vis; op.vis_vec = (reinterpret_cast<uintptr_t>(vis) & 3) == 0; op.ts = t_starts; op.te = t_ends;
-        op.out_starts = out_starts; op.o_ri = out_ray_indices; op.o_ts = out_t_starts; op.o_te = out_t_ends; op.cap = capacity;
-        launch_seg<1>(op, packed_info, tiles, n_rays, n_tiles, s);
-    });
+    launch_compact(vis, t_starts, explicit_ends(t_ends), packed_info, tiles, n_tiles, out_starts, n_rays, out_ray_indices,
+                   out_t_starts, out_t_ends, capacity, as_stream(stream));
     NFA_CHECK_LAUNCH("compact_samples");
+    return NFA_OK;
+}
+
+int nfa_compact_samples_implied(const uint8_t *vis, const float *t_starts, float step_size, float cone_angle,
+                                const int64_t *packed_info, const int64_t *tiles, int64_t n_tiles, const int64_t *out_starts,
+                                int64_t n_rays, int64_t n_elems, int64_t *out_ray_indices, float *out_t_starts, float *out_t_ends,
+                                int64_t capacity, nfa_stream_t stream)
+{
+    SEG_IMPLIED_CHECKS("compact_samples_implied");
+    SEG_COMMON_CHECKS("compact_samples_implied");
+    if (n_elems == 0) return NFA_OK;
+    NFA_REQUIRE(vis && t_starts && out_starts, "compact_samples_implied: null input");
+    NFA_REQUIRE(capacity >= 0, "compact_samples_implied: negative capacity");
+    launch_compact(vis, t_starts, implied_ends(step_size, cone_angle), packed_info, tiles, n_tiles, out_starts, n_rays,
+                   out_ray_indices, out_t_starts, out_t_ends, capacity, as_stream(stream));
+    NFA_CHECK_LAUNCH("compact_samples_implied");
     return NFA_OK;
 }
 
@@ -2066,15 +2198,25 @@
     if (n_rays == 0) return NFA_OK;
     NFA_REQUIRE(colors && opacities && depths && (n_elems == 0 || (t_starts && t_ends && sigmas && rgbs)),
                 "render_fused_fwd: null pointer");
-    hipStream_t s = as_stream(stream);
-    const bool vec = all_aligned16(t_starts, t_ends, sigmas, rgbs, weights, trans, alphas);
-    dispatch_bool(vec, [&](auto V) {
-        RenderFusedFwdOp<V> op;
-        op.ts = t_starts; op.te = t_ends; op.sig = sigmas; op.rgb = rgbs; op.w = weights; op.tr = trans; op.al = alphas;
-        op.colors = colors; op.opac = opacities; op.depth = depths;
-        launch_seg<1>(op, packed_info, tiles, n_rays, n_tiles, s);
-    });
+    launch_render_fused_fwd(t_starts, explicit_ends(t_ends), sigmas, rgbs, packed_info, tiles, n_tiles, n_rays, weights, trans,
+                            alphas, colors, opacities, depths, as_stream(stream));
     NFA_CHECK_LAUNCH("render_fused_fwd");
+    return NFA_OK;
+}
+
+int nfa_render_fused_fwd_implied(const float *t_starts, float step_size, float cone_angle, const float *sigmas, const float *rgbs,
+                                 const int64_t *packed_info, const int64_t *tiles, int64_t n_tiles, int64_t n_rays, int64_t n_elems,
+                                 float *weights, float *trans, float *alphas, float *colors, float *opacities, float *depths,
+                                 nfa_stream_t stream)
+{
+    SEG_IMPLIED_CHECKS("render_fused_fwd_implied");
+    SEG_COMMON_CHECKS("render_fused_fwd_implied");
+    if (n_rays == 0) return NFA_OK;
+    NFA_REQUIRE(colors && opacities && depths && (n_elems == 0 || (t_starts && sigmas && rgbs)),
+                "render_fused_fwd_implied: null pointer");
+    launch_render_fused_fwd(t_starts, implied_ends(step_size, cone_angle), sigmas, rgbs, packed_info, tiles, n_tiles, n_rays,
+                            weights, trans, alphas, colors, opacities, depths, as_stream(stream));
+    NFA_CHECK_LAUNCH("render_fused_fwd_implied");
     return NFA_OK;
 }
 
@@ -2087,19 +2229,26 @@
     SEG_COMMON_CHECKS("render_fused_bwd");
     if (n_elems == 0) return NFA_OK;
     NFA_REQUIRE(t_starts && t_ends && rgbs && trans && alphas && (grad_sigmas || grad_rgbs), "render_fused_bwd: null pointer");
-    hipStream_t s = as_stream(stream);
-    const bool vec = all_aligned16(t_starts, t_ends, rgbs, trans, alphas, g_weights, g_trans, g_alphas, grad_sigmas, grad_rgbs);
-    const bool extra = g_weights || g_trans || g_alphas;
-    dispatch_bool(vec, [&](auto V) {
-        dispatch_bool(extra, [&](auto X) {
-            RenderFusedBwdOp<V, X> op;
-            op.ts = t_starts; op.te = t_ends; op.rgb = rgbs; op.tr = trans; op.al = alphas;
-            op.gc = g_colors; op.go = g_opacities; op.gd = g_depths; op.gw = g_weights; op.gt = g_trans; op.ga = g_alphas;
-            op.gsig = grad_sigmas; op.grgb = grad_rgbs;
-            launch_seg<-1>(op, packed_info, tiles, n_rays, n_tiles, s);
-        });
-    });
+    launch_render_fused_bwd(t_starts, explicit_ends(t_ends), rgbs, trans, alphas, g_colors, g_opacities, g_depths, g_weights,
+                            g_trans, g_alphas, packed_info, tiles, n_tiles, n_rays, grad_sigmas, grad_rgbs, as_stream(stream));
     NFA_CHECK_LAUNCH("render_fused_bwd");
+    return NFA_OK;
+}
+
+int nfa_render_fused_bwd_implied(const float *t_starts, float step_size, float cone_angle, const float *rgbs, const float *trans,
+                                 const float *alphas, const float *g_colors, const float *g_opacities, const float *g_depths,
+                                 const float *g_weights, const float *g_trans, const float *g_alphas, const int64_t *packed_info,
+                                 const int64_t *tiles, int64_t n_tiles, int64_t n_rays, int64_t n_elems, float *grad_sigmas,
+                                 float *grad_rgbs, nfa_stream_t stream)
+{
+    SEG_IMPLIED_CHECKS("render_fused_bwd_implied");
+    SEG_COMMON_CHECKS("render_fused_bwd_implied");
+    if (n_elems == 0) return NFA_OK;
+    NFA_REQUIRE(t_starts && rgbs && trans && alphas && (grad_sigmas || grad_rgbs), "render_fused_bwd_implied: null pointer");
+    launch_render_fused_bwd(t_starts, implied_ends(step_size, cone_angle), rgbs, trans, alphas, g_colors, g_opacities, g_depths,
+                            g_weights, g_trans, g_alphas, packed_info, tiles, n_tiles, n_rays, grad_sigmas, grad_rgbs,
+                            as_stream(stream));
+    NFA_CHECK_LAUNCH("render_fused_bwd_implied");
     return NFA_OK;
 }
 
diff --git a/nerfacc_amd/estimators/occ_grid.py b/nerfacc_amd/estimators/occ_grid.py
--- a/nerfacc_amd/estimators/occ_grid.py
+++ b/nerfacc_amd/estimators/occ_grid.py
@@ -7,7 +7,7 @@
 from torch import Tensor
 
 from .. import _backend as B
-from .._segments import SegInfo, tag_ray_indices, tag_trusted
+from .._segments import SegInfo, implied_ends, tag_implied_ends, tag_ray_indices, tag_trusted
 from ..grid import _enlarge_aabb, _exclusive_cumsum, _traverse_samples
 from ..volrend import _visibility_native
 from .base import AbstractEstimator
@@ -170,7 +170,8 @@
                 else:
                     sigmas = torch.empty((0,), device=t_starts.device)
                 assert sigmas.shape == t_starts.shape, "sigmas must have shape of (N,)! Got {}".format(sigmas.shape)
-                vis, cnts = _visibility_native(seg, t_starts, t_ends, sigmas, None, early_stop_eps, alpha_thre, True)
+                vis, cnts = _visibility_native(seg, t_starts, t_ends, sigmas, None, early_stop_eps, alpha_thre, True,
+                                               ends=implied_ends(t_starts, t_ends))
             else:
                 if t_starts.shape[0] != 0:
                     alphas = alpha_fn(t_starts, t_ends, ray_indices)
@@ -375,9 +376,10 @@
         host = _pinned_total(dev)
         ri = ts = te = None
         cap = 0
+        ends = implied_ends(t_starts, t_ends)
 
         def run(ri, ts, te, capacity):
-            B.call("nfa_compact_samples", B.ptr(vis), B.ptr(t_starts), B.ptr(t_ends), B.ptr(seg.packed_info),
+            B.call("nfa_compact_samples", B.ptr(vis), B.ptr(t_starts), ends if ends is not None else B.ptr(t_ends), B.ptr(seg.packed_info),
                    B.ptr(seg.tiles), seg.n_tiles, B.ptr(out_starts), seg.n_rays, n, B.ptr(ri), B.ptr(ts), B.ptr(te), capacity, B.stream())
 
         if frac < 1.0 and n > 0:
@@ -418,6 +420,8 @@
         packed = torch.stack([out_starts, cnts], dim=-1)
     info = tag_trusted(packed, m)
     tag_ray_indices(ri, seg.n_rays, info)
+    if ends is not None:
+        tag_implied_ends(ts, te, ends.step, ends.cone)
     return ri, ts, te
 
 
diff --git a/nerfacc_amd/grid.py b/nerfacc_amd/grid.py
--- a/nerfacc_amd/grid.py
+++ b/nerfacc_amd/grid.py
@@ -8,7 +8,7 @@
 from torch import Tensor
 
 from . import _backend as B
-from ._segments import tag_ray_indices, tag_trusted
+from ._segments import tag_implied_ends, tag_ray_indices, tag_trusted
 from .data_specs import RayIntervals, RaySamples
 
 
@@ -495,6 +495,7 @@
                 B.call("nfa_fill_ray_indices", n_rays, B.ptr(packed_info), B.ptr(ray_indices), B.stream())
     info = tag_trusted(packed_info, n_sm)
     tag_ray_indices(ray_indices, n_rays, info)
+    tag_implied_ends(t_starts, t_ends, float(step_size), float(cone_angle))
     out = (ray_indices, t_starts, t_ends, packed_info)
     return (*out, terminate) if return_terminate else out
 
diff --git a/nerfacc_amd/volrend.py b/nerfacc_amd/volrend.py
--- a/nerfacc_amd/volrend.py
+++ b/nerfacc_amd/volrend.py
@@ -7,7 +7,7 @@
 from torch.autograd.function import once_differentiable
 
 from . import _backend as B
-from ._segments import SegInfo, batched_native, resolve, seginfo_from_ray_indices
+from ._segments import SegInfo, batched_native, implied_ends, resolve, seginfo_from_ray_indices
 from .scan import exclusive_prod, exclusive_sum
 
 
@@ -183,7 +183,7 @@
 class _RenderFused(torch.autograd.Function):
 
     @staticmethod
-    def forward(ctx, t_starts, t_ends, sigmas, rgbs, seg: SegInfo):
+    def forward(ctx, t_starts, t_ends, sigmas, rgbs, seg: SegInfo, ends=None):
         ctx.set_materialize_grads(False)
         ts, te, sg, c = _f32c(t_starts), _f32c(t_ends), _f32c(sigmas), _f32c(rgbs)
         dev = B.require_device(ts, te, sg, c)
@@ -194,17 +194,25 @@
         depth = torch.empty((R, 1), dtype=torch.float32, device=dev)
         if R:
             with torch.cuda.device(dev):
-                B.call("nfa_render_fused_fwd", B.ptr(ts), B.ptr(te), B.ptr(sg), B.ptr(c), B.ptr(seg.packed_info),
-                       B.ptr(seg.tiles), seg.n_tiles, R, n, B.ptr(weights), B.ptr(trans), B.ptr(alphas), B.ptr(colors),
-                       B.ptr(opac), B.ptr(depth), B.stream())
-        ctx.seg = seg
-        ctx.save_for_backward(ts, te, c, trans, alphas)
+                B.call("nfa_render_fused_fwd", B.ptr(ts), ends if ends is not None else B.ptr(te), B.ptr(sg), B.ptr(c),
+                       B.ptr(seg.packed_info), B.ptr(seg.tiles), seg.n_tiles, R, n, B.ptr(weights), B.ptr(trans),
+                       B.ptr(alphas), B.ptr(colors), B.ptr(opac), B.ptr(depth), B.stream())
+        ctx.seg, ctx.ends = seg, ends
+        if ends is not None:
+            ctx.save_for_backward(ts, c, trans, alphas)
+        else:
+            ctx.save_for_backward(ts, te, c, trans, alphas)
         return colors, opac, depth, weights, trans, alphas
 
     @staticmethod
     @once_differentiable
     def backward(ctx, g_c, g_o, g_d, g_w, g_t, g_a):
-        ts, te, c, trans, alphas = ctx.saved_tensors
+        ends = ctx.ends
+        if ends is not None:
+            ts, c, trans, alphas = ctx.saved_tensors
+            te = None
+        else:
+            ts, te, c, trans, alphas = ctx.saved_tensors
         seg = ctx.seg
         if ctx.needs_input_grad[0] or ctx.needs_input_grad[1]:
             raise NotImplementedError("nerfacc_amd: rendering is not differentiable w.r.t. t_starts / t_ends "
@@ -214,11 +222,11 @@
         g_rgb = torch.empty_like(c) if need_c else None
         if trans.numel() and (need_sg or need_c):
             with torch.cuda.device(trans.device):
-                B.call("nfa_render_fused_bwd", B.ptr(ts), B.ptr(te), B.ptr(c), B.ptr(trans), B.ptr(alphas),
+                B.call("nfa_render_fused_bwd", B.ptr(ts), ends if ends is not None else B.ptr(te), B.ptr(c), B.ptr(trans), B.ptr(alphas),
                        B.ptr(_f32c(g_c)), B.ptr(_f32c(g_o)), B.ptr(_f32c(g_d)), B.ptr(_f32c(g_w)), B.ptr(_f32c(g_t)),
                        B.ptr(_f32c(g_a)), B.ptr(seg.packed_info), B.ptr(seg.tiles), seg.n_tiles, seg.n_rays,
                        trans.numel(), B.ptr(g_sig), B.ptr(g_rgb), B.stream())
-        return None, None, g_sig, g_rgb, None
+        return None, None, g_sig, g_rgb, None, None
 
 
 def _use_fused(seg: Optional[SegInfo], *tensors: Optional[Tensor]) -> bool:
@@ -263,7 +271,8 @@
         if FUSE_RENDERING and seg is not None and seg.sorted_indices and _use_fused(seg, sigmas, t_starts, t_ends) \
                 and rgbs.dtype == torch.float32 and rgbs.dim() == 2 \
                 and not (t_starts.requires_grad or t_ends.requires_grad):
-            colors, opacities, depths, weights, trans, alphas = _RenderFused.apply(t_starts, t_ends, sigmas, rgbs, seg)
+            colors, opacities, depths, weights, trans, alphas = _RenderFused.apply(
+                t_starts, t_ends, sigmas, rgbs, seg, implied_ends(t_starts, t_ends))
             extras = {"weights": weights, "alphas": alphas, "trans": trans, "sigmas": sigmas, "rgbs": rgbs}
             return _finish_rendering(colors, opacities, depths, extras, rgbs, render_bkgd)
         weights, trans, alphas = render_weight_from_density(
@@ -395,14 +404,15 @@
 
 
 def _visibility_native(seg: SegInfo, t_starts, t_ends, vals, prefix_trans, early_stop_eps, alpha_thre,
-                       want_counts: bool = False):
+                       want_counts: bool = False, ends=None):
     ts, te, v, pf = _f32c(t_starts), _f32c(t_ends), _f32c(vals), _f32c(prefix_trans)
     dev = B.require_device(v, ts, te, pf)
     n = v.numel()
     vis = torch.empty(n, dtype=torch.bool, device=dev)
     cnts = torch.empty(seg.n_rays, dtype=torch.int64, device=dev) if want_counts else None
     with torch.cuda.device(dev):
-        B.call("nfa_render_visibility", B.ptr(ts), B.ptr(te), B.ptr(v), B.ptr(pf), float(early_stop_eps),
+        B.call("nfa_render_visibility", B.ptr(ts), ends if (ends is not None and ts is not None) else B.ptr(te), B.ptr(v), B.ptr(pf),
+               float(early_stop_eps),
                float(alpha_thre), B.ptr(seg.packed_info), B.ptr(seg.tiles), seg.n_tiles, seg.n_rays, n, B.ptr(vis), B.ptr(cnts),
                B.stream())
     return (vis, cnts) if want_counts else vis
```

Result: faster. 764.8 million rays/s (median of 6 runs) (+3.2%).
